# caomw/3DFeatureMatcher

Hardware: AMD Instinct MI355X
Metric: matched+triangulated+normal-optimised keypoints/sec; HBM GB/s vs roofline (higher is better)
Workload: dtype f64

## Files before the change

3dfeaturematcher_amd/csrc/fm3d_ctx.h:

```cpp
#pragma once

#include <hip/hip_runtime.h>

#include <cstdint>
#include <cstdlib>
#include <string>
#include <vector>

#include "fm3d.h"
#include "fm3d_algebra.h"
#include "fm3d_kernels.h"

namespace fm3d_host {

inline bool poison_word(uint32_t* word) {
    const char* e = getenv("FM3D_DEBUG_POISON");
    if (!e || !e[0]) return false;
    *word = (uint32_t)strtoul(e, nullptr, 0);
    return true;
}
inline void poison_host(void* p, size_t n, uint32_t word) {
    uint8_t* b = (uint8_t*)p;
    for (size_t i = 0; i < n; i++) b[i] = (uint8_t)(word >> (8 * (i & 3)));
}
inline hipError_t poison_device(void* p, size_t n) {
    uint32_t word;
    if (!poison_word(&word)) return hipSuccess;
    hipError_t e = hipSuccess;
    if (n / 4) e = hipMemsetD32((hipDeviceptr_t)p, (int)word, n / 4);
    for (size_t i = n & ~(size_t)3; e == hipSuccess && i < n; i++)
        e = hipMemset((uint8_t*)p + i, (int)(uint8_t)(word >> (8 * (i & 3))), 1);
    if (e == hipSuccess) e = hipDeviceSynchronize();
    return e;
}

template <class Mem>
struct Buf {
    void* p = nullptr;
    size_t bytes = 0;
    Buf() = default;
    Buf(const Buf&) = delete;
    Buf& operator=(const Buf&) = delete;
    Buf(Buf&& o) noexcept : p(o.p), bytes(o.bytes) {
        o.p = nullptr;
        o.bytes = 0;
    }
    Buf& operator=(Buf&& o) noexcept {
        if (this != &o) {
            if (p) Mem::free(p);
            p = o.p;
            bytes = o.bytes;
            o.p = nullptr;
            o.bytes = 0;
        }
        return *this;
    }
    ~Buf() {
        if (p) Mem::free(p);
    }
    hipError_t ensure(size_t n) {
        if (n <= bytes) return hipSuccess;
        if (p) Mem::free(p);
        p = nullptr;
        bytes = 0;
        size_t alloc = n < Mem::kMin ? Mem::kMin : n;
        hipError_t e = Mem::alloc(&p, alloc);
        if (e == hipSuccess) e = Mem::poison(p, alloc);
        if (e == hipSuccess) {
            bytes = alloc;
        } else if (p) {
            Mem::free(p);
            p = nullptr;
        }
        return e;
    }
    template <typename T>
    T* as() const {
        return (T*)p;
    }
};

struct DeviceMem {
    static constexpr size_t kMin = 256;
    static hipError_t alloc(void** p, size_t n) { return hipMalloc(p, n); }
    static hipError_t free(void* p) { return hipFree(p); }
    static hipError_t poison(void* p, size_t n) { return poison_device(p, n); }
};
struct PinnedMem {
    static constexpr size_t kMin = 4096;
    static hipError_t alloc(void** p, size_t n) { return hipHostMalloc(p, n, hipHostMallocDefault); }
    static hipError_t free(void* p) { return hipHostFree(p); }
    static hipError_t poison(void* p, size_t n) {
        uint32_t word;
        if (poison_word(&word)) poison_host(p, n, word);
        return hipSuccess;
    }
};
using DevBuf = Buf<DeviceMem>;
using HostBuf = Buf<PinnedMem>;

constexpr size_t kGuard(int w) { return (size_t)4 * w + 64; }

struct PipeSmall {
    int32_t cnt[4];
    unsigned long long prob[2];
    unsigned long long lm[26];
};

struct KnnWork {
    DevBuf cq, ct;
    DevBuf q8, t8;
    DevBuf partIdx, partKey;
    DevBuf pairs;
    DevBuf idx, key, fkey;
};

enum class PairState { Idle, Full, MemberFront, DltFront, Ncc, Verified, DltVerified };

enum class Need { Idle, StagedIdle, Full, Dlt, Ncc, Verified, DltVerified };

enum Ev {
    EV_LM_START,
    EV_END,
    EV_FRONT_START,
    EV_MATCH_DONE,
    EV_DLT_DONE,
    EV_VERIFY_START, EV_VERIFY_END,
    EV_NORMAL_START, EV_NORMAL_END,
    EV_SUBMIT_START,
    EV_TAIL_START,
    EV_COUNT
};

}

using fm3d_host::DevBuf;
using fm3d_host::HostBuf;

struct fm3d_ctx {
    fm3d_settings s;
    int device = 0;
    hipStream_t stream = nullptr;
    bool ownStream = false;
    fm3d::Camera cam{};
    double g12[16];
    double R2[9], t2[3];
    bool haveG12 = false;
    int w = 0, h = 0;
    std::vector<int> lw, lh;
    std::vector<DevBuf> pyr1, pyr2;
    int pyrGuardW = -1, pyrGuardH = -1, pyrGuardLevels = -1;
    DevBuf lvlDesc;
    DevBuf offsets;
    int nOff = 0, nOffPad = 0;
    DevBuf A, B, knnOut, cand, flag, matches, count, scanTmp;
    fm3d_host::KnnWork fwd, rev;
    DevBuf u8Flag;
    DevBuf gLines, gUV;
    bool gateStaged = false;
    bool specU8 = false;
    DevBuf sfImg, sfSum, sfDet, sfTr, sfLayers, sfMids, sfCand, sfCount, sfSortTmp, sfFlag, sfPos, sfKp, sfKin, sfSrc,
        sfDesc, sfDW, sfAng;
    DevBuf orbPyr, orbTab, orbLev, orbMap, orbFlag, orbPos, orbKp, orbR, orbBlur, orbDesc, orbPat;
    std::vector<int> orbUserPattern;
    DevBuf orbOffTab;
    std::vector<int> orbTabPattern;
    int orbTabPatchSize = 0, orbTabReach = 0;
    float orbTabAngle = 0.f;
    DevBuf siftImg, siftBase, siftG, siftD, siftGL, siftDL, siftTaps, siftScan, siftFlag, siftPos, siftCand, siftAng,
        siftNpk, siftKp, siftDesc;
    DevBuf brImg, brSum, brKp, brIdx, brPat, brPairs, brDesc;
    DevBuf frImg, frSum, frKp, frScale, frLut, frOp, frPairs, frAng, frDesc;
    DevBuf msImg, msWork, msHeap, msNode, msHist, msReg, msCnt, msOff, msXY, msScr, msKp, msFlag, msPos, msOut, msRank,
        msPad, msRegC;
    std::vector<int> freakUserPairs;
    DevBuf starImg, starS, starT, starF, starR, starZ, starKp, starFlag, starPos, starOut, starWork;
    DevBuf nccS, nccN, nccB;
    int nccH = 0;
    DevBuf f32Work;
    int nCU = 0;
    DevBuf kp1, kp2, triPts, triMask, triMask8, pts, srcIdx;
    long lmGroups = 0;
    int wallKhz = 0;
    DevBuf lmNormals, lmStatus, lmInfo, lmNfev, lmMdat, lmQueue, lmStat, slab, slabI1;
    DevBuf lbSt, lbCtr;
    unsigned lbEpoch = 0;
    DevBuf records, recTmp, recFlag;
    DevBuf lmProj;
    DevBuf pcnt;
    DevBuf verWork, verMatches;
    DevBuf tailFrames, tailRT, tailDesc, tailPatch;
    DevBuf pdKp, pdGL, pdLvl, pdTaps, pdKept;
    int pdCap = 0, pdSize = 0, pdNTaps = 0;
    float pdAngle = 0.f, pdSigma = 0.f;
    HostBuf hA, hB, hK1, hK2, hImg, hTab, hProj, hSmall, hFlag;
    HostBuf hVer;
    hipEvent_t evStage = nullptr;
    hipEvent_t evProj = nullptr;
    int nccP = 0;
    bool staged = false;
    struct Pipe {
        fm3d_host::PairState state = fm3d_host::PairState::Idle;
        int nA = 0, nB = 0, dim = 0, type = 0, dimPad = 0, queryOffset = 0;
        int K = 0, P = 0;
        bool stageEv = true;
        fm3d_record* subOut = nullptr;
        fm3d_record* pendOut = nullptr;
        fm3d_lm_stats subLm{};
        int nccHPending = 0;
        fm3d_ctx* linkLeader = nullptr;
        std::vector<fm3d_ctx*> linkMembers;
        hipEvent_t evFront = nullptr;
        hipEvent_t evLm = nullptr;
    } pipe;
    hipEvent_t ev[fm3d_host::EV_COUNT] = {};
    std::string err;

    fm3d_ctx() = default;
    fm3d_ctx(const fm3d_ctx&) = delete;
    fm3d_ctx& operator=(const fm3d_ctx&) = delete;
    ~fm3d_ctx() {
        for (hipEvent_t e : {evStage, evProj, pipe.evFront, pipe.evLm})
            if (e) hipEventDestroy(e);
        for (hipEvent_t e : ev)
            if (e) hipEventDestroy(e);
        if (ownStream) hipStreamDestroy(stream);
    }
};

namespace fm3d_host {

inline int fail(fm3d_ctx* c, int code, const std::string& msg) {
    if (c) c->err = msg;
    return code;
}

inline bool env_on(const char* name) {
    const char* e = getenv(name);
    return !(e && e[0] == '0');
}

int ensure_scan_tmp(fm3d_ctx* c, int n);
void install_g12(fm3d_ctx* c, const double g[16]);
bool good_max_px(double v);
int make_gate(fm3d_ctx* c, const fm3d_point2f* kp1, int nA, const fm3d_point2f* kp2, int nB, double maxPx,
              fm3d::EpiGate* g);
int ensure_offsets(fm3d_ctx* c);
int upload(fm3d_ctx* c, DevBuf& b, const void* src, size_t bytes);
int staging_wait(fm3d_ctx* c);
int upload_pinned(fm3d_ctx* c, DevBuf& dst, HostBuf& h, const void* src, size_t bytes);
int make_lookback(fm3d_ctx* c, int nBlocks, fm3d::LookBack* lb);
fm3d::TriParams tri_params(fm3d_ctx* c, int K, int queryOffset);
fm3d::NccParams ncc_params(fm3d_ctx* c, int Hphi, int Htheta, double span);
int set_images_impl(fm3d_ctx* c, const uint8_t* img1, const uint8_t* img2, int width, int height, int stride,
                    bool sync = true, bool waitStaging = true);

int stage_descriptors(fm3d_ctx* c, const void* descA, int nA, const void* descB, int nB, int dim, int type,
                      int* effType, int* dimPad, bool waitStaging = true, bool speculate = false);
struct MatchOpts {
    double eps = 0.0;
    int queryOffset = 0;
    bool wantKnn = false;
    fm3d_dmatch* compactOut = nullptr;
    int* compactCount = nullptr;
    const fm3d::EpiGate* gate = nullptr;
    int crossCheck = 0;
};
int run_match(fm3d_ctx* c, int nA, int nB, int type, int dimPad, const MatchOpts& o);

int describe_chunk();

struct LMSrc {
    fm3d_ctx* c;
    int P;
    const int* Pdev;
};
int lm_groups(fm3d_ctx* c, const void* kptr, int slots, long Ptot, long* out);
int run_lm_multi(fm3d_ctx* c, const LMSrc* src, int nProb, fm3d_lm_stats* stats, hipEvent_t e0, hipEvent_t e1);
int run_lm(fm3d_ctx* c, int P, const int* Pdev, fm3d_lm_stats* stats, hipEvent_t e0, hipEvent_t e1);
void fill_lm_cycles(const fm3d_ctx* c, const unsigned long long* cnt, fm3d_lm_stats* st);
fm3d::Camera lm_camera(const fm3d::Camera& cam);

int verify_staged(fm3d_ctx* c, const fm3d_verify_opts* o, int K, fm3d_verify_report* rep, bool* havePose,
                  double g12[16]);
int verify_staged_queue(fm3d_ctx* c, const fm3d_verify_opts* o);
int verify_report(fm3d_ctx* c, fm3d_verify_report* rep);

}

#define HIPCHK(ctx, expr)                                                                \
    do {                                                                                 \
        hipError_t e_ = (expr);                                                          \
        if (e_ != hipSuccess)                                                            \
            return fm3d_host::fail((ctx), FM3D_ERR_HIP, std::string(#expr ": ") + hipGetErrorString(e_)); \
    } while (0)
```

3dfeaturematcher_amd/csrc/fm3d_host.cpp:

```cpp
#include <hip/hip_runtime.h>

#include <algorithm>
#include <cfloat>
#include <cmath>
#include <cstdlib>
#include <cstring>
#include <string>
#include <vector>

#include "fm3d.h"
#include "fm3d_ctx.h"
#include "fm3d_kernels.h"

using fm3d::LevelDesc;

using namespace fm3d_host;

namespace fm3d_host {

int ensure_scan_tmp(fm3d_ctx* c, int n) {
    HIPCHK(c, c->scanTmp.ensure(fm3d::scan_tmp_bytes(n < 1 ? 1 : n)));
    HIPCHK(c, c->count.ensure(64));
    return FM3D_OK;
}

void install_g12(fm3d_ctx* c, const double g[16]) {
    std::memcpy(c->g12, g, sizeof(c->g12));
    camera2_from_g12(c->g12, c->R2, c->t2);
    c->haveG12 = true;
    c->gateStaged = false;
}

bool good_max_px(double v) { return v > 0. && v <= DBL_MAX; }

int make_gate(fm3d_ctx* c, const fm3d_point2f* kp1, int nA, const fm3d_point2f* kp2, int nB, double maxPx,
              fm3d::EpiGate* g) {
    HIPCHK(c, c->gLines.ensure((size_t)nA * sizeof(float4) + 16));
    HIPCHK(c, c->gUV.ensure((size_t)nB * sizeof(float2) + 16));
    double E[9];
    epipolar_matrix(c->R2, c->t2, E);
    fm3d::launch_epipolar_setup(c->cam, E, kp1, nA, kp2, nB, c->gLines.as<float4>(), c->gUV.as<float2>(), c->stream);
    HIPCHK(c, hipGetLastError());
    g->lines = c->gLines.as<float4>();
    g->uv = c->gUV.as<float2>();
    g->tau = maxPx * 2.0 / (c->cam.fx + c->cam.fy);
    return FM3D_OK;
}

int ensure_offsets(fm3d_ctx* c) {
    if (c->nOff > 0) return FM3D_OK;
    const int R = c->s.pixelsRay;
    std::vector<int2> off;
    for (int i = -R; i <= R; i++)
        for (int j = -R; j <= R; j++)
            if (i * i + j * j <= R * R) off.push_back(make_int2(i, j));
    c->nOff = (int)off.size();
    while (off.size() % 64) off.push_back(make_int2(1 << 20, 1 << 20));
    c->nOffPad = (int)off.size();
    HIPCHK(c, c->offsets.ensure(off.size() * sizeof(int2)));
    HIPCHK(c, hipMemcpy(c->offsets.p, off.data(), off.size() * sizeof(int2), hipMemcpyHostToDevice));
    return FM3D_OK;
}

int upload(fm3d_ctx* c, DevBuf& b, const void* src, size_t bytes) {
    HIPCHK(c, b.ensure(bytes));
    if (bytes) HIPCHK(c, hipMemcpyAsync(b.p, src, bytes, hipMemcpyHostToDevice, c->stream));
    return FM3D_OK;
}

int staging_wait(fm3d_ctx* c) {
    HIPCHK(c, hipEventSynchronize(c->evStage));
    return FM3D_OK;
}

int upload_pinned(fm3d_ctx* c, DevBuf& dst, HostBuf& h, const void* src, size_t bytes) {
    HIPCHK(c, dst.ensure(bytes));
    if (!bytes) return FM3D_OK;
    HIPCHK(c, h.ensure(bytes));
    std::memcpy(h.p, src, bytes);
    HIPCHK(c, hipMemcpyAsync(dst.p, h.p, bytes, hipMemcpyHostToDevice, c->stream));
    return FM3D_OK;
}

int make_lookback(fm3d_ctx* c, int nBlocks, fm3d::LookBack* lb) {
    if (!c->lbCtr.p) {
        HIPCHK(c, c->lbCtr.ensure(64));
        HIPCHK(c, hipMemsetAsync(c->lbCtr.p, 0, 64, c->stream));
    }
    bool zero = false;
    if (c->lbSt.bytes < (size_t)nBlocks * 8) {
        HIPCHK(c, c->lbSt.ensure((size_t)nBlocks * 8 * 2));
        zero = true;
    }
    if (++c->lbEpoch == 0) {
        c->lbEpoch = 1;
        zero = true;
    }
    if (zero) HIPCHK(c, hipMemsetAsync(c->lbSt.p, 0, c->lbSt.bytes, c->stream));
    lb->st = c->lbSt.as<unsigned long long>();
    lb->ctr = c->lbCtr.as<unsigned>();
    lb->epoch = c->lbEpoch;
    return FM3D_OK;
}

int set_images_impl(fm3d_ctx* c, const uint8_t* img1, const uint8_t* img2, int width, int height, int stride,
                    bool sync, bool waitStaging) {
    if (!img1 || !img2 || width <= 0 || height <= 0 || stride < width)
        return fail(c, FM3D_ERR_INVALID, "bad image arguments");
    const int levels = c->s.pyramids;
    if (levels < 0 || levels > 7) return fail(c, FM3D_ERR_UNSUPPORTED, "pyramids must be in [0, 7]");
    int r;
    if (waitStaging && (r = staging_wait(c))) return r;
    c->w = width;
    c->h = height;
    c->lw.assign(levels + 1, 0);
    c->lh.assign(levels + 1, 0);
    c->pyr1.resize(levels + 1);
    c->pyr2.resize(levels + 1);
    c->lw[0] = width;
    c->lh[0] = height;
    for (int L = 1; L <= levels; L++) {
        c->lw[L] = (c->lw[L - 1] + 1) / 2;
        c->lh[L] = (c->lh[L - 1] + 1) / 2;
    }
    bool fresh = c->pyrGuardW != width || c->pyrGuardH != height || c->pyrGuardLevels != levels;
    for (int L = 0; L <= levels; L++) {
        size_t bytes = (size_t)c->lw[L] * c->lh[L] + kGuard(c->lw[L]);
        void* p1 = c->pyr1[L].p;
        void* p2 = c->pyr2[L].p;
        HIPCHK(c, c->pyr1[L].ensure(bytes));
        HIPCHK(c, c->pyr2[L].ensure(bytes));
        fresh |= c->pyr1[L].p != p1 || c->pyr2[L].p != p2;
    }
    for (int L = 0; fresh && L <= levels; L++) {
        const size_t img = (size_t)c->lw[L] * c->lh[L];
        HIPCHK(c, hipMemsetAsync((char*)c->pyr1[L].p + img, 0, c->pyr1[L].bytes - img, c->stream));
        HIPCHK(c, hipMemsetAsync((char*)c->pyr2[L].p + img, 0, c->pyr2[L].bytes - img, c->stream));
    }
    c->pyrGuardW = width;
    c->pyrGuardH = height;
    c->pyrGuardLevels = levels;
    const size_t wh = (size_t)width * height;
    HIPCHK(c, c->hImg.ensure(2 * wh));
    for (int y = 0; y < height; y++) {
        std::memcpy(c->hImg.as<uint8_t>() + (size_t)y * width, img1 + (size_t)y * stride, width);
        std::memcpy(c->hImg.as<uint8_t>() + wh + (size_t)y * width, img2 + (size_t)y * stride, width);
    }
    HIPCHK(c, hipMemcpyAsync(c->pyr1[0].p, c->hImg.p, wh, hipMemcpyHostToDevice, c->stream));
    HIPCHK(c, hipMemcpyAsync(c->pyr2[0].p, c->hImg.as<uint8_t>() + wh, wh, hipMemcpyHostToDevice, c->stream));
    for (int L = 1; L <= levels; L++) {
        fm3d::launch_pyrdown(c->pyr1[L - 1].as<uint8_t>(), c->lw[L - 1], c->lh[L - 1], c->pyr1[L].as<uint8_t>(),
                             c->stream);
        fm3d::launch_pyrdown(c->pyr2[L - 1].as<uint8_t>(), c->lw[L - 1], c->lh[L - 1], c->pyr2[L].as<uint8_t>(),
                             c->stream);
    }
    HIPCHK(c, hipGetLastError());
    HIPCHK(c, c->hTab.ensure((levels + 1) * sizeof(LevelDesc)));
    LevelDesc* d = c->hTab.as<LevelDesc>();
    for (int L = 0; L <= levels; L++) d[L] = LevelDesc{c->pyr1[L].as<uint8_t>(), c->pyr2[L].as<uint8_t>(), c->lw[L], c->lh[L]};
    HIPCHK(c, c->lvlDesc.ensure((levels + 1) * sizeof(LevelDesc)));
    HIPCHK(c, hipMemcpyAsync(c->lvlDesc.p, d, (levels + 1) * sizeof(LevelDesc), hipMemcpyHostToDevice, c->stream));
    HIPCHK(c, hipEventRecord(c->evStage, c->stream));
    if (sync) HIPCHK(c, hipStreamSynchronize(c->stream));
    return FM3D_OK;
}

fm3d::TriParams tri_params(fm3d_ctx* c, int K, int queryOffset) {
    fm3d::TriParams p{};
    p.cam = c->cam;
    std::memcpy(p.g12, c->g12, sizeof(p.g12));
    p.zmin = c->s.zThresholdMin;
    p.zmax = c->s.zThresholdMax;
    p.kp1 = c->kp1.as<fm3d_point2f>();
    p.kp2 = c->kp2.as<fm3d_point2f>();
    p.matches = c->matches.as<fm3d_dmatch>();
    p.K = K;
    p.queryOffset = queryOffset;
    p.pts = c->triPts.as<double>();
    p.mask = c->triMask.as<int>();
    p.dltSolver = c->s.dltSolver;
    return p;
}

fm3d::NccParams ncc_params(fm3d_ctx* c, int Hphi, int Htheta, double span) {
    fm3d::NccParams p{};
    p.cam = lm_camera(c->cam);
    std::memcpy(p.R2, c->R2, sizeof(p.R2));
    std::memcpy(p.t2, c->t2, sizeof(p.t2));
    p.img1 = c->pyr1[0].as<uint8_t>();
    p.img2 = c->pyr2[0].as<uint8_t>();
    p.w = c->lw[0];
    p.h = c->lh[0];
    p.offsets = c->offsets.as<int2>();
    p.nOff = c->nOff;
    p.nOffPad = c->nOffPad;
    p.boundW = c->s.boundWidth;
    p.boundH = c->s.boundHeight;
    p.cmax = (int)(2 * c->s.zThresholdMax);
    p.Hphi = Hphi;
    p.Htheta = Htheta;
    p.span = span;
    return p;
}

}

extern "C" {

const char* fm3d_version(void) { return "fm3d 0.1 (gfx950)"; }

int fm3d_ctx_create(const fm3d_settings* s, int device, fm3d_ctx** out) {
    if (!s || !out) return FM3D_ERR_INVALID;
    *out = nullptr;
    if (s->dltSolver != 0 && s->dltSolver != 1) return FM3D_ERR_INVALID;
    if (!(s->guidedMatchPx >= 0. && s->guidedMatchPx <= DBL_MAX)) return FM3D_ERR_INVALID;
    if (s->crossCheck < 0 || s->crossCheck > 2) return FM3D_ERR_INVALID;
    int n = 0;
    if (hipGetDeviceCount(&n) != hipSuccess || n <= 0) return FM3D_ERR_HIP;
    if (device < 0 || device >= n) return FM3D_ERR_INVALID;
    if (hipSetDevice(device) != hipSuccess) return FM3D_ERR_HIP;
    fm3d_ctx* c = new fm3d_ctx();
    c->s = *s;
    c->device = device;
    if (hipStreamCreateWithFlags(&c->stream, hipStreamNonBlocking) != hipSuccess) {
        delete c;
        return FM3D_ERR_HIP;
    }
    c->ownStream = true;
    if (const char* le = getenv("FM3D_DEBUG_LB_EPOCH")) c->lbEpoch = (unsigned)strtoul(le, nullptr, 0);
    for (auto& e : c->ev) hipEventCreate(&e);
    hipEventCreateWithFlags(&c->evStage, hipEventDisableTiming);
    hipEventCreateWithFlags(&c->evProj, hipEventDisableTiming);
    hipEventCreateWithFlags(&c->pipe.evFront, hipEventDisableTiming);
    hipEventCreateWithFlags(&c->pipe.evLm, hipEventDisableTiming);
    c->cam.fx = s->Fx;
    c->cam.fy = s->Fy;
    c->cam.cx = s->Cx;
    c->cam.cy = s->Cy;
    c->cam.k[0] = s->k0;
    c->cam.k[1] = s->k1;
    c->cam.k[2] = s->p1;
    c->cam.k[3] = s->p2;
    c->cam.k[4] = s->k2;
    *out = c;
    return FM3D_OK;
}

void fm3d_ctx_destroy(fm3d_ctx* c) {
    if (!c) return;
    hipSetDevice(c->device);
    hipStreamSynchronize(c->stream);
    if (c->pipe.linkLeader) {
        auto& v = c->pipe.linkLeader->pipe.linkMembers;
        v.erase(std::remove(v.begin(), v.end(), c), v.end());
    }
    for (fm3d_ctx* m : c->pipe.linkMembers) m->pipe.linkLeader = nullptr;
    delete c;
}

const char* fm3d_last_error(const fm3d_ctx* c) { return c ? c->err.c_str() : "null context"; }

int fm3d_ctx_set_stream(fm3d_ctx* c, void* stream) {
    if (!c) return FM3D_ERR_INVALID;
    hipSetDevice(c->device);
    hipStreamSynchronize(c->stream);
    if (c->ownStream) hipStreamDestroy(c->stream);
    if (stream) {
        c->stream = (hipStream_t)stream;
        c->ownStream = false;
    } else {
        HIPCHK(c, hipStreamCreateWithFlags(&c->stream, hipStreamNonBlocking));
        c->ownStream = true;
    }
    return FM3D_OK;
}

int fm3d_setg12(fm3d_ctx* c, const double T1[3], const double T2[3], const double r1[3], const double r2[3],
                double g12[16]) {
    if (!c || !T1 || !T2 || !r1 || !r2) return fail(c, FM3D_ERR_INVALID, "null argument");
    double g[16];
    fm3d_g12_from_poses(&c->s, T1, T2, r1, r2, g);
    install_g12(c, g);
    if (g12) std::memcpy(g12, g, sizeof(g));
    return FM3D_OK;
}

int fm3d_set_g12(fm3d_ctx* c, const double g12[16]) {
    if (!c || !g12) return fail(c, FM3D_ERR_INVALID, "null argument");
    install_g12(c, g12);
    return FM3D_OK;
}

int fm3d_get_camera2(const fm3d_ctx* c, double R2[9], double t2[3]) {
    if (!c || !c->haveG12) return FM3D_ERR_INVALID;
    std::memcpy(R2, c->R2, sizeof(c->R2));
    std::memcpy(t2, c->t2, sizeof(c->t2));
    return FM3D_OK;
}

int fm3d_triangulate(fm3d_ctx* c, const fm3d_point2f* kpts1, int n1, const fm3d_point2f* kpts2, int n2,
                     const fm3d_dmatch* matches, int K, double* points, uint8_t* inlierMask, int* nPoints) {
    if (!c || !nPoints || K < 0) return fail(c, FM3D_ERR_INVALID, "bad argument");
    if (!c->haveG12) return fail(c, FM3D_ERR_INVALID, "g12 not set (SingleCameraTriangulator::setg12)");
    hipSetDevice(c->device);
    for (int i = 0; i < K; i++)
        if (matches[i].queryIdx < 0 || matches[i].queryIdx >= n1 || matches[i].trainIdx < 0 || matches[i].trainIdx >= n2)
            return fail(c, FM3D_ERR_INVALID, "match index out of range");
    int r;
    if ((r = upload(c, c->kp1, kpts1, (size_t)n1 * sizeof(fm3d_point2f)))) return r;
    if ((r = upload(c, c->kp2, kpts2, (size_t)n2 * sizeof(fm3d_point2f)))) return r;
    if ((r = upload(c, c->matches, matches, (size_t)K * sizeof(fm3d_dmatch)))) return r;
    HIPCHK(c, c->triPts.ensure((size_t)(K + 1) * 3 * sizeof(double)));
    HIPCHK(c, c->triMask.ensure((size_t)(K + 1) * sizeof(int)));
    HIPCHK(c, c->triMask8.ensure((size_t)(K + 1)));
    HIPCHK(c, c->pts.ensure((size_t)(K + 1) * 3 * sizeof(double)));
    HIPCHK(c, c->srcIdx.ensure((size_t)(K + 1) * sizeof(int)));
    if ((r = ensure_scan_tmp(c, K))) return r;
    fm3d::TriParams p = tri_params(c, K, 0);
    p.mask8 = c->triMask8.as<uint8_t>();
    fm3d::launch_triangulate(p, c->stream);
    fm3d::launch_compact_points(c->triPts.as<double>(), c->triMask.as<int>(), K, nullptr, c->pts.as<double>(),
                                c->count.as<int>(), c->srcIdx.as<int>(), c->scanTmp.p, c->stream);
    HIPCHK(c, hipGetLastError());
    int n = 0;
    HIPCHK(c, hipMemcpyAsync(&n, c->count.p, sizeof(int), hipMemcpyDeviceToHost, c->stream));
    if (inlierMask && K) HIPCHK(c, hipMemcpyAsync(inlierMask, c->triMask8.p, K, hipMemcpyDeviceToHost, c->stream));
    HIPCHK(c, hipStreamSynchronize(c->stream));
    if (n && points) HIPCHK(c, hipMemcpy(points, c->pts.p, (size_t)n * 3 * sizeof(double), hipMemcpyDeviceToHost));
    *nPoints = n;
    return FM3D_OK;
}

int fm3d_set_images(fm3d_ctx* c, const uint8_t* img1, const uint8_t* img2, int width, int height, int stride) {
    if (!c) return FM3D_ERR_INVALID;
    hipSetDevice(c->device);
    return set_images_impl(c, img1, img2, width, height, stride);
}

int fm3d_get_pyramid_level(const fm3d_ctx* cc, int which, int level, uint8_t* out, int* w, int* h) {
    fm3d_ctx* c = const_cast<fm3d_ctx*>(cc);
    if (!c || level < 0 || level >= (int)c->pyr1.size() || (which != 1 && which != 2)) return FM3D_ERR_INVALID;
    hipSetDevice(c->device);
    if (w) *w = c->lw[level];
    if (h) *h = c->lh[level];
    if (out) {
        const DevBuf& b = which == 1 ? c->pyr1[level] : c->pyr2[level];
        HIPCHK(c, hipMemcpy(out, b.p, (size_t)c->lw[level] * c->lh[level], hipMemcpyDeviceToHost));
    }
    return FM3D_OK;
}

int fm3d_records_download(fm3d_ctx* c, const fm3d_record* recordsDev, int n, fm3d_record* out) {
    if (!c || n < 0 || (n && !out)) return FM3D_ERR_INVALID;
    hipSetDevice(c->device);
    const void* src = recordsDev ? (const void*)recordsDev : c->records.p;
    if (n) HIPCHK(c, hipMemcpy(out, src, (size_t)n * sizeof(fm3d_record), hipMemcpyDeviceToHost));
    return FM3D_OK;
}

int fm3d_features_frames(fm3d_ctx* c, const double* points, const double* normals, int P, double* frames) {
    if (!c || P < 0 || (P && (!points || !normals || !frames))) return FM3D_ERR_INVALID;
    if (P == 0) return FM3D_OK;
    hipSetDevice(c->device);
    double g[3];
    int r;
    if ((r = fm3d_gravity(&c->s, g))) return fail(c, r, "gravity: singular rodriguesIC rotation");
    DevBuf a, b, f;
    HIPCHK(c, a.ensure((size_t)P * 3 * sizeof(double)));
    HIPCHK(c, b.ensure((size_t)P * 3 * sizeof(double)));
    HIPCHK(c, f.ensure((size_t)P * 16 * sizeof(double)));
    HIPCHK(c, hipMemcpyAsync(a.p, points, (size_t)P * 3 * sizeof(double), hipMemcpyHostToDevice, c->stream));
    HIPCHK(c, hipMemcpyAsync(b.p, normals, (size_t)P * 3 * sizeof(double), hipMemcpyHostToDevice, c->stream));
    fm3d::launch_features_frames(a.as<double>(), b.as<double>(), P, g, f.as<double>(), c->stream);
    HIPCHK(c, hipGetLastError());
    HIPCHK(c, hipMemcpyAsync(frames, f.p, (size_t)P * 16 * sizeof(double), hipMemcpyDeviceToHost, c->stream));
    HIPCHK(c, hipStreamSynchronize(c->stream));
    return FM3D_OK;
}

int fm3d_export_patches(fm3d_ctx* c, const double* frames, int P, uint8_t* patches, double* imagePoints) {
    if (!c || P < 0 || (P && (!frames || !patches))) return FM3D_ERR_INVALID;
    if (c->pyr1.empty()) return fail(c, FM3D_ERR_INVALID, "fm3d_set_images not called");
    const int size = fm3d_patch_size(&c->s);
    if (size <= 0) return fail(c, FM3D_ERR_INVALID, "patch size <= 0 (Neighborhoods.epsilon / cmPerPixel)");
    if (P == 0) return FM3D_OK;
    hipSetDevice(c->device);
    const size_t per = (size_t)size * size;
    DevBuf f, rt, out, pts;
    HIPCHK(c, f.ensure((size_t)P * 16 * sizeof(double)));
    HIPCHK(c, rt.ensure((size_t)P * 12 * sizeof(double)));
    HIPCHK(c, out.ensure((size_t)P * per));
    if (imagePoints) HIPCHK(c, pts.ensure((size_t)P * per * 2 * sizeof(double)));
    HIPCHK(c, hipMemcpyAsync(f.p, frames, (size_t)P * 16 * sizeof(double), hipMemcpyHostToDevice, c->stream));
    fm3d::launch_export_patches(f.as<double>(), P, size, c->s.neighEpsilon, c->s.cmPerPixel * 0.01, c->cam,
                                c->pyr1[0].as<uint8_t>(), c->lw[0], c->lh[0], rt.as<double>(), out.as<uint8_t>(),
                                imagePoints ? pts.as<double>() : nullptr, c->stream);
    HIPCHK(c, hipGetLastError());
    HIPCHK(c, hipMemcpyAsync(patches, out.p, (size_t)P * per, hipMemcpyDeviceToHost, c->stream));
    if (imagePoints)
        HIPCHK(c, hipMemcpyAsync(imagePoints, pts.p, (size_t)P * per * 2 * sizeof(double), hipMemcpyDeviceToHost,
                                 c->stream));
    HIPCHK(c, hipStreamSynchronize(c->stream));
    return FM3D_OK;
}

int fm3d_square_neighborhoods(fm3d_ctx* c, const double* frames, int P, double* out) {
    if (!c || P < 0 || (P && (!frames || !out))) return FM3D_ERR_INVALID;
    const int size = fm3d_patch_size(&c->s);
    if (size <= 0) return fail(c, FM3D_ERR_INVALID, "neighbourhood size <= 0 (Neighborhoods.epsilon / cmPerPixel)");
    if (P == 0) return FM3D_OK;
    hipSetDevice(c->device);
    const size_t perFrame = (size_t)size * size * 3 * sizeof(double);
    const int chunk = (int)std::max<size_t>(1, std::min<size_t>((size_t)P, ((size_t)512 << 20) / perFrame));
    DevBuf f, o;
    HIPCHK(c, f.ensure((size_t)chunk * 16 * sizeof(double)));
    HIPCHK(c, o.ensure((size_t)chunk * perFrame));
    for (int p0 = 0; p0 < P; p0 += chunk) {
        const int n = std::min(chunk, P - p0);
        HIPCHK(c, hipMemcpyAsync(f.p, frames + (size_t)16 * p0, (size_t)n * 16 * sizeof(double),
                                 hipMemcpyHostToDevice, c->stream));
        fm3d::launch_square_neighborhoods(f.as<double>(), n, size, c->s.neighEpsilon, c->s.cmPerPixel * 0.01,
                                          o.as<double>(), c->stream);
        HIPCHK(c, hipGetLastError());
        HIPCHK(c, hipMemcpyAsync(out + (size_t)p0 * size * size * 3, o.p, (size_t)n * perFrame,
                                 hipMemcpyDeviceToHost, c->stream));
        HIPCHK(c, hipStreamSynchronize(c->stream));
    }
    return FM3D_OK;
}

int fm3d_circular_neighborhoods(fm3d_ctx* c, const double* points, const double* normals, int P, double* out) {
    if (!c || P < 0 || (P && (!points || !out))) return FM3D_ERR_INVALID;
    if (c->s.neighMethod != 1) return fail(c, FM3D_ERR_INVALID, "Neighborhoods.method is not circular");
    const int T = c->s.neighThetas, Rn = c->s.neighRays;
    if (T <= 0 || Rn <= 0) return fail(c, FM3D_ERR_INVALID, "Neighborhoods.thetas / rays <= 0");
    if (P == 0) return FM3D_OK;
    hipSetDevice(c->device);
    const double eps = c->s.neighEpsilon;
    const double rayIncrement = eps / Rn, thetaIncrement = 2 * M_PI / T;
    const int S = T * Rn;
    std::vector<double> lut((size_t)S * 3);
    for (int i = 1; i <= Rn; i++)
        for (int j = 0; j < T; j++) {
            const double t = j * thetaIncrement;
            double* e = &lut[3 * ((size_t)(i - 1) * T + j)];
            e[0] = (double)i * rayIncrement;
            e[1] = std::sin(t);
            e[2] = 2 * (std::sin(t / 2)) * (std::sin(t / 2));
        }
    const size_t perPoint = (size_t)S * 3 * sizeof(double);
    const int chunk = (int)std::max<size_t>(1, std::min<size_t>((size_t)P, ((size_t)512 << 20) / perPoint));
    DevBuf L, X, N, O;
    HIPCHK(c, L.ensure(lut.size() * sizeof(double)));
    HIPCHK(c, X.ensure((size_t)chunk * 3 * sizeof(double)));
    if (normals) HIPCHK(c, N.ensure((size_t)chunk * 3 * sizeof(double)));
    HIPCHK(c, O.ensure((size_t)chunk * perPoint));
    HIPCHK(c, hipMemcpyAsync(L.p, lut.data(), lut.size() * sizeof(double), hipMemcpyHostToDevice, c->stream));
    for (int p0 = 0; p0 < P; p0 += chunk) {
        const int n = std::min(chunk, P - p0);
        HIPCHK(c, hipMemcpyAsync(X.p, points + (size_t)3 * p0, (size_t)n * 3 * sizeof(double), hipMemcpyHostToDevice,
                                 c->stream));
        if (normals)
            HIPCHK(c, hipMemcpyAsync(N.p, normals + (size_t)3 * p0, (size_t)n * 3 * sizeof(double),
                                     hipMemcpyHostToDevice, c->stream));
        fm3d::launch_circular_neighborhoods(X.as<double>(), normals ? N.as<double>() : nullptr, n, S, L.as<double>(),
                                            eps, O.as<double>(), c->stream);
        HIPCHK(c, hipGetLastError());
        HIPCHK(c, hipMemcpyAsync(out + (size_t)p0 * S * 3, O.p, (size_t)n * perPoint, hipMemcpyDeviceToHost,
                                 c->stream));
        HIPCHK(c, hipStreamSynchronize(c->stream));
    }
    return FM3D_OK;
}

int fm3d_ncc_hypotheses(fm3d_ctx* c, const double* points, int P, int Hphi, int Htheta, double span, double* scores,
                        double* normals, int32_t* best) {
    if (!c || P < 0 || Hphi <= 0 || Htheta <= 0 || Hphi * Htheta > 32 || (P && (!points || !scores || !normals || !best)))
        return FM3D_ERR_INVALID;
    if (c->pyr1.empty()) return fail(c, FM3D_ERR_INVALID, "fm3d_set_images (NormalOptimizer::setImages) not called");
    if (!c->haveG12) return fail(c, FM3D_ERR_INVALID, "fm3d_set_g12 / fm3d_setg12 not called");
    if (P == 0) return FM3D_OK;
    hipSetDevice(c->device);
    int r;
    if ((r = ensure_offsets(c))) return r;
    const int H = Hphi * Htheta;
    DevBuf X, S, N, B;
    HIPCHK(c, X.ensure((size_t)P * 3 * sizeof(double)));
    HIPCHK(c, S.ensure((size_t)P * H * sizeof(double)));
    HIPCHK(c, N.ensure((size_t)P * 3 * sizeof(double)));
    HIPCHK(c, B.ensure((size_t)P * sizeof(int)));
    HIPCHK(c, hipMemcpyAsync(X.p, points, (size_t)P * 3 * sizeof(double), hipMemcpyHostToDevice, c->stream));
    fm3d::NccParams p = ncc_params(c, Hphi, Htheta, span);
    p.points = X.as<double>();
    p.P = P;
    p.scores = S.as<double>();
    p.normals = N.as<double>();
    p.best = B.as<int>();
    fm3d::launch_ncc_hypotheses(p, c->stream);
    HIPCHK(c, hipGetLastError());
    HIPCHK(c, hipMemcpyAsync(scores, S.p, (size_t)P * H * sizeof(double), hipMemcpyDeviceToHost, c->stream));
    HIPCHK(c, hipMemcpyAsync(normals, N.p, (size_t)P * 3 * sizeof(double), hipMemcpyDeviceToHost, c->stream));
    HIPCHK(c, hipMemcpyAsync(best, B.p, (size_t)P * sizeof(int), hipMemcpyDeviceToHost, c->stream));
    HIPCHK(c, hipStreamSynchronize(c->stream));
// ... 131 lines not shown
```

3dfeaturematcher_amd/csrc/fm3d_internal.h:

```cpp
#pragma once

#include <hip/hip_runtime.h>

#include "fm3d.h"

int fm3d_internal_submit_to(fm3d_ctx* c, const void* descA, int nA, const void* descB, int nB, int dim, int type,
                            const fm3d_point2f* kpts1, const fm3d_point2f* kpts2, const uint8_t* img1,
                            const uint8_t* img2, int width, int height, fm3d_record* recordsDev);
int fm3d_internal_flush(fm3d_ctx* c);
bool fm3d_internal_front_only(const fm3d_ctx* c);
int fm3d_internal_enqueue(fm3d_ctx* c, fm3d_record* recordsDev);
int fm3d_internal_finish(fm3d_ctx* c, int* nKept, fm3d_pipeline_stats* stats);
const int* fm3d_internal_kept_dev(fm3d_ctx* c);
hipStream_t fm3d_internal_stream(fm3d_ctx* c);
int fm3d_internal_prepare(fm3d_ctx* c);
int fm3d_internal_memory_need(fm3d_ctx* c, int64_t nA, int64_t nB, int dim, int type, int width, int height,
                              size_t* bytes);
extern "C" int fm3d_internal_alloc_probe(fm3d_ctx* c, size_t bytes, uint8_t* out);
```

3dfeaturematcher_amd/csrc/fm3d_kernels.h:

```cpp
#pragma once

#include <hip/hip_runtime.h>
#include <stdint.h>

#include "fm3d.h"
#include "fm3d_device.h"

#ifndef FM3D_RAY_AOS
#define FM3D_RAY_AOS 1
#endif

namespace fm3d {

struct LevelDesc {
    const uint8_t* img1;
    const uint8_t* img2;
    int w, h;
};

struct ProjConst {
    double R[9], t[3];
    Camera cam;
    const char *slabRX, *slabRY, *slabI1;
    char *slabDF, *slabDJ0, *slabDJ1;
    double k2d, k3d;
};

struct LMProblem {
    const double* points;
    const int* Pdev;
    const LevelDesc* lvl;
    double* normals;
    int* status;
    int* info;
    int* nfev;
    int* mdat;
    unsigned long long* stat;
    int P;
    unsigned projOff;
};

struct LMParams {
    const double* points_;
    int P_;
    const int* Pdev_;
    Camera cam;
    double R2_[9], t2_[3];
    const ProjConst* proj;
    const LevelDesc* lvl_;
    int levels;
    const int2* offsets;
    int nOff, nOffPad;
    int boundW, boundH;
    double epsfcn;
    int cmax;
    int* queue;
    double* slab;
    float* slabI1;
    long nWaves;
    double* normals_;
    int* status_;
    int* info_;
    int* nfev_;
    int* mdat_;
    unsigned long long* statEval;
    unsigned long long* statPix;
    long long maxIter;
    long long maxTicks;
    int* overflow;
    int coop;
    int safe;
    unsigned long long* statPass;
    int nProb;
    const LMProblem* prob;
};
constexpr int kLMMaxProblems = 4;

constexpr int kLMRunning = 0x100;

constexpr int kLM2Slots = 15;
constexpr int kLM2Ring = 8;
constexpr int kLM2Threads = 64 * (kLM2Slots + 1);
template <bool MULTI, bool TREE>
__global__ void lm2_kernel(LMParams p);

struct KnnOut {
    int* idx;
    int* key;
    float* fkey;
};

struct EpiGate {
    const float4* lines;
    const float2* uv;
    double tau;
    bool transposed = false;
};
void launch_epipolar_setup(const Camera& cam, const double E[9], const fm3d_point2f* kp1, int n1,
                           const fm3d_point2f* kp2, int n2, float4* lines, float2* uv, hipStream_t s);

int knn2_u8_parts(int nA, int nB, int nCU, int qPerBlock, int tileRows);
int knn2_i8_queries_per_block(int dimPad, int bits);
int knn2_i8_tile_rows(int dimPad, int bits);
void launch_knn2_i8(const uint8_t* A, int nA, const uint8_t* B, int nB, int dimPad, int bits, const int* cqA,
                    const int* ctB, int parts, int* partIdx, int* partKey, int* idx, int* key, hipStream_t s,
                    bool deferMerge = false, const EpiGate* gate = nullptr);
void launch_rowconst_u8(const uint8_t* A, int nA, const uint8_t* B, int nB, int dimPad, int* cq, int* ctp,
                        hipStream_t s);
void launch_f32_pack_u8(const float* A, int nA, const float* B, int nB, int dim, int dimPad, uint8_t* Au,
                        uint8_t* Bu, int* notU8, hipStream_t s);
void launch_unpack_bits(const uint8_t* A, int nA, const uint8_t* B, int nB, uint8_t* outA, uint8_t* outB, int* ctp,
                        hipStream_t s);
int knn2_parts(int nA, int nB, int dim, int nCU);
size_t knn2_f32_pairs_bytes(int nB, int dim);
void launch_knn2_f32(const float* A, int nA, const float* B, int nB, int dim, int parts, int* partIdx,
                     float* partKey, float* pairs, int* idx, float* key, hipStream_t s);
void launch_knn2_f32_gated(const float* A, int nA, const float* B, int nB, int dim, int parts, int* partIdx,
                           float* partKey, int* idx, float* key, const EpiGate& gate, hipStream_t s);
size_t knn2_f32_mfma_bytes(int nA, int nB, int dim, int parts);
int knn2_f32_mfma_parts(int nA, int nB, int nCU);
void launch_knn2_f32_mfma(const float* A, int nA, const float* B, int nB, int dim, int parts, bool fused, void* work,
                          int* idx, float* key, hipStream_t s);
int* knn2_f32_mfma_rescan_count(void* work, int nA, int nB, int dim, int parts);
void launch_knn2_f32_mfma_rescan(const float* A, const float* B, int nB, int dim, void* work, int nA, int parts,
                                 int nResc, int* idx, float* key, hipStream_t s);
void launch_knn2_bits(const uint8_t* A, int nA, const uint8_t* B, int nB, int dimBytes, int parts, int* partIdx,
                      int* partKey, int* idx, int* key, hipStream_t s, const EpiGate* gate = nullptr);
void launch_nndr(int type, const int* idx, const int* key, const float* fkey, int nA, int nB, double eps,
                 int queryOffset, fm3d_dmatch* knnOut, fm3d_dmatch* cand, int* flag, hipStream_t s);

struct NccParams {
    const double* points;
    int P;
    const int* Pdev;
    Camera cam;
    double R2[9], t2[3];
    const uint8_t *img1, *img2;
    int w, h;
    const int2* offsets;
    int nOff, nOffPad, boundW, boundH, cmax;
    int Hphi, Htheta;
    double span;
    double* scores;
    double* normals;
    int* best;
};
void launch_ncc_hypotheses(const NccParams& p, hipStream_t s);

struct SurfHF {
    int p0, p1, p2, p3;
    float w;
};
struct SurfLayer {
    long long first;
    size_t off;
    int size, step, margin, si, sj, rows, cols;
    SurfHF hf[10];
};
struct SurfMid {
    long long first;
    int layer, octave, rows, cols, margin;
};
struct SurfCand {
    float x, y, size, response;
    int octave, class_id;
    long long seq;
};
constexpr int kOriMax = 128;
struct SurfOri {
    int n;
    int ax[kOriMax], ay[kOriMax];
    float w[kOriMax];
};
void launch_integral(const uint8_t* img, int w, int h, int* sum, hipStream_t s);
void launch_integral_rows(const uint8_t* img, int w, int h, int* rows, hipStream_t s);
void launch_integral_batch(const uint8_t* img, int w, int h, int nb, int* sum, hipStream_t s);
void launch_surf_orient(const void* kp, size_t kstride, int n, const int* sum, size_t sumStride, int w, int h,
                        const SurfOri& ori, int* flag, float* angle, hipStream_t s);
void launch_surf_hessian(const int* sum, int w, const SurfLayer* layers, int nL, long long total, float* det,
                         float* tr, hipStream_t s);
void launch_surf_maxima(const float* det, const float* tr, const SurfLayer* layers, const SurfMid* mids, int nM,
                        long long total, float thr, SurfCand* cand, int* count, int cap, hipStream_t s);
size_t surf_sort_tmp_bytes(int n);
void launch_surf_sort(SurfCand* cand, int n, void* tmp, size_t tmpBytes, hipStream_t s);
void launch_surf_upright(const SurfCand* cand, const int* count, int n, int w, int h, int* flag, int* pos, int* total,
                         void* scanTmp, fm3d_keypoint* out, int* src, const float* angle, hipStream_t s);
void launch_surf_keep(const fm3d_keypoint* in, int n, int w, int h, int* flag, int* pos, int* total, void* scanTmp,
                      fm3d_keypoint* out, int* src, const float* angle, hipStream_t s);
void launch_surf_describe(const uint8_t* img, size_t imgStride, int w, int h, const fm3d_keypoint* kp, int n,
                          const float* DW, int extended, int upright, float* desc, hipStream_t s);

struct OrbLevel {
    int w, h;
    long long first;
};
struct OrbUmax {
    int u[64];
};
struct OrbBlurK {
    int ik[7];
    float fk[4];
};
void launch_orb_resize(const uint8_t* src, int sw, int sh, uint8_t* dst, int dw, int dh, const int* xofs,
                       const short* alpha, const int* yofs, const short* beta, int xmax, int xs, hipStream_t s);
void launch_orb_fast(const uint8_t* pyr, const OrbLevel* L, int nL, long long total, int thr, int border, int nonmax,
                     uint16_t* map, int* flag, hipStream_t s);
void launch_orb_fast_scatter(const uint16_t* map, const OrbLevel* L, int nL, long long total, const int* flag,
                             const int* pos, fm3d_keypoint* out, hipStream_t s);
void launch_orb_harris(const uint8_t* pyr, const OrbLevel* L, fm3d_keypoint* kp, int n, hipStream_t s);
void launch_orb_angle(const uint8_t* pyr, const OrbLevel* L, fm3d_keypoint* kp, int n, int half, const OrbUmax& um,
                      hipStream_t s);
void launch_orb_blur(const uint8_t* pyr, const OrbLevel* L, int nL, long long total, const OrbBlurK& bk, int* R,
                     uint8_t* out, hipStream_t s);
void launch_orb_desc(const uint8_t* blur, const OrbLevel* L, const fm3d_keypoint* kp, int n, const int* pattern,
                     uint8_t* desc, hipStream_t s);
void launch_orb_offset_table(const int* pattern, float angle, int2* tab, hipStream_t s);
void launch_orb_patch_desc(const uint8_t* patches, int m, int size, const int2* tab, const OrbBlurK& bk, uint8_t* desc,
                           hipStream_t s);

struct SiftLevel {
    int w, h;
    long long first;
};
struct SiftResize {
    int sw, sh, dw, dh, xmax, doubled;
    double scx, scy;
};
struct SiftScan {
    long long first;
    int dog, octave, layer, pad;
};
struct SiftCand {
    float x, y, size, response;
    int koct;
    int octave, layer, r, c, ok;
};
void launch_sift_init(const uint8_t* img, float* dst, const SiftResize& p, int batch, hipStream_t s);
size_t sift_blur_lds(int n);
void launch_sift_blur(const float* src, float* dst, float* dog, int w, int h, const float* taps, int n, int batch,
                      hipStream_t s);
void launch_sift_down(const float* src, int sw, int sh, float* dst, int dw, int dh, double ifx, double ify,
                      hipStream_t s);
void launch_sift_extrema(const float* dog, const SiftLevel* DL, const SiftScan* S, int nS, long long total,
                         int threshold, int* flag, hipStream_t s);
void launch_sift_cand_scatter(const SiftLevel* DL, const SiftScan* S, int nS, long long total, const int* flag,
                              const int* pos, SiftCand* cand, hipStream_t s);
void launch_sift_adjust(const float* dog, const SiftLevel* DL, int L, float contrastThreshold, float edgeThreshold,
                        float sigma, SiftCand* cand, int n, hipStream_t s);
void launch_sift_orient(const float* gp, const SiftLevel* GL, int L, const SiftCand* cand, int n, float* angles,
                        int* npk, hipStream_t s);
void launch_sift_desc(const float* gp, const SiftLevel* GL, int L, int firstOctave, const fm3d_keypoint* kp,
                      const int* lvl, int n, float* desc, hipStream_t s);

size_t scan_tmp_bytes(int n);
void launch_compact_dmatch(const fm3d_dmatch* in, const int* flag, int n, fm3d_dmatch* out, int* count, void* tmp,
                           hipStream_t s, const int* nDev = nullptr);
void launch_compact_points(const double* in, const int* flag, int n, const int* nDev, double* out, int* count,
                           int* srcIndex, void* tmp, hipStream_t s);
void launch_exclusive_scan(const int* flag, int n, int* offsets, int* total, void* tmp, hipStream_t s);

constexpr int kVerifyTile = 1024;
constexpr int kVerifyMaxHyps = 1 << 20;
int verify_pad(int M);
void launch_verify(const Camera& cam, const fm3d_point2f* kp1, const fm3d_point2f* kp2, const fm3d_dmatch* matches,
                   int M, int H, unsigned long long seed, double tau2, int nCU, double* xy, double* models, int* count,
                   int* best, double* E, int* flag, uint8_t* mask, hipStream_t s, bool withMask = true,
                   const int* Mdev = nullptr);
size_t verify_refine_bytes(int M, int rounds);
void launch_verify_refine(int M, int rounds, double tau2, const double* xy, const int* count, const int* best,
                          double* E, void* work, int* flag, uint8_t* mask, int** roundCounts, double** roundModels,
                          int** adopted, hipStream_t s, const int* Mdev = nullptr);
struct VerifySmall {
    int32_t matches, verified, best, adopted;
    double E[9];
};
void launch_verify_report(const int* Mdev, const int* best, const double* E, const int* adopted, const int* verified,
                          VerifySmall* host, hipStream_t s);
size_t verify_pose_bytes();
void launch_verify_pose(int M, const double* xy, const int* flag, const int* best, const double* E, void* work,
                        double** cand, int** valid, int** votes, hipStream_t s);

struct AlignIn {
    const double *ptsA, *nrmA, *ptsB, *nrmB;
    int nA, nB;
};
inline int align_planes(bool normals) { return normals ? 12 : 6; }
void launch_align(const AlignIn& in, const fm3d_dmatch* matches, int M, int H, unsigned long long seed, double tau2,
                  double minCos, int nCU, double* planes, double* models, int* count, int* best, double* model,
                  int* flag, uint8_t* mask, hipStream_t s, bool withMask = true);
size_t align_refine_bytes(int M, int rounds);
void launch_align_refine(int M, bool normals, int rounds, double tau2, double minCos, const double* planes,
                         const int* count, const int* best, double* model, void* work, int* flag, uint8_t* mask,
                         int** roundCounts, double** roundModels, int** adopted, hipStream_t s);

struct LocalizeIn {
    const fm3d_point2f* kpts;
    const double *pts, *nrm;
    int nKpts, nPts;
};
inline int localize_planes(bool normals) { return normals ? 8 : 5; }
void launch_localize(const Camera& cam, const LocalizeIn& in, const fm3d_dmatch* matches, int M, int samples,
                     unsigned long long seed, double tau2, double cos2, int nCU, double* planes, double* models,
                     int* count, int* best, double* model, int* flag, uint8_t* mask, hipStream_t s,
                     bool withMask = true);
size_t localize_refine_bytes(int M, int rounds);
void launch_localize_refine(int M, bool normals, int rounds, double tau2, double cos2, const double* planes,
                            const int* count, const int* best, double* model, void* work, int* flag, uint8_t* mask,
                            int** roundCounts, double** roundModels, int** adopted, hipStream_t s);

struct TriParams {
    Camera cam;
    double g12[16];
    double zmin, zmax;
    const fm3d_point2f* kp1;
    const fm3d_point2f* kp2;
    const fm3d_dmatch* matches;
    int K;
    const int* Kdev;
    int queryOffset;
    double* pts;
    int* mask;
    uint8_t* mask8;
    int dltSolver;
};
void launch_triangulate(const TriParams& p, hipStream_t s);

struct LMReset {
    unsigned long long* stat;
    int* queue;
    int nProb;
    int* pcnt16[kLMMaxProblems];
    int* status[kLMMaxProblems];
    int* info[kLMMaxProblems];
    int* nfev[kLMMaxProblems];
    int P[kLMMaxProblems];
};
void launch_lm_reset(const LMReset& r, hipStream_t s);

struct LookBack {
    unsigned long long* st;
    unsigned* ctr;
    unsigned epoch;
};
__device__ inline int lookback_block_id(const LookBack& lb) {
    const unsigned id = atomicAdd(lb.ctr, 1u);
    if (id == gridDim.x - 1) __hip_atomic_store(lb.ctr, 0u, __ATOMIC_RELAXED, __HIP_MEMORY_SCOPE_AGENT);
    return (int)id;
}
void launch_nndr_compact(int type, const int* idx, const int* key, const float* fkey, const int* partIdx,
                         const int* partKey, int parts, int nA, double eps, int queryOffset, fm3d_dmatch* out,
                         int* count, const LookBack& lb, hipStream_t s);
int nndr_compact_blocks(int nA);
struct MutualCheck {
    const int* rIdx;
    const int* rKey;
    const float* rFkey;
    int mode;
};
void launch_nndr_mutual_compact(int type, const int* idx, const int* key, const float* fkey, const int* partIdx,
                                const int* partKey, int parts, int nA, double eps, int queryOffset,
                                const MutualCheck& mc, fm3d_dmatch* out, int* count, const LookBack& lb,
                                hipStream_t s);
void launch_triangulate_compact(const TriParams& p, double* out, int* srcIdx, int* count, const LookBack& lb,
                                hipStream_t s, int* hostCnt = nullptr);
int triangulate_compact_blocks(int K);

void launch_pyrdown(const uint8_t* src, int w, int h, uint8_t* dst, hipStream_t s);
void launch_undistort(const Camera& cam, const double* xy, int n, double* out, hipStream_t s);

bool math_probe_binary(int fn);
void launch_math_probe(int fn, const double* x, const double* y, int n, double* out, hipStream_t s);

struct PlaneProjParams {
    Camera cam;
    double R2[9], t2[3], X[3], n[3];
    double cmax;
    const int2* offsets;
    int nOff, boundW, boundH, w, h;
    double *xy, *uv;
    int *keep, *status;
};
void launch_plane_project(const PlaneProjParams& p, hipStream_t s);

void launch_features_frames(const double* pts, const double* nrm, int P, const double g[3], double* frames,
                            hipStream_t s);
void launch_circular_neighborhoods(const double* pts, const double* nrm, int P, int S, const double* lut, double eps,
                                   double* out, hipStream_t s);
void launch_square_neighborhoods(const double* frames, int P, int size, double eps, double inc, double* out,
                                 hipStream_t s);
void launch_export_patches(const double* frames, int P, int size, double eps, double inc, const Camera& cam,
                           const uint8_t* img, int w, int h, double* RT, uint8_t* patches, double* imagePoints,
                           hipStream_t s);
void launch_tail_frames(const fm3d_record* rec, const double* pts, const double* nrm, int P, const double g[3],
                        double* frames, double* RT, hipStream_t s);
void launch_patches(const double* RT, int P, int size, double eps, double inc, const Camera& cam, const uint8_t* img,
                    int w, int h, uint8_t* patches, hipStream_t s);
void launch_add_count(const int* count, int* sum, hipStream_t s);

void launch_make_records(const fm3d_dmatch* matches, const int* inlierSrc, int nInl, const int* nDev, const double* pts,
                         const double* normals, const int* status, fm3d_record* rec, int* flag, hipStream_t s);
void launch_compact_records(const fm3d_record* in, const int* flag, int n, const int* nDev, fm3d_record* out,
                            int* count, void* tmp, hipStream_t s);

struct StarPat {
    int np, maxIdx, border, nsimd;
    int sizes1[17];
    int ofs[17 * 8];
    float inv[24];
};
struct StarNms {
    int border, delta, nx, ny, respThr, lineProj, lineBin;
};
size_t star_tilted_lds_bytes(int w);
int star_tilted_max_width();
void launch_star_tilted(const uint8_t* img, int w, int h, int* T, int* F, hipStream_t s);
size_t star_diag_bytes(int w, int h);
void launch_star_tilted_diag(const uint8_t* img, int w, int h, void* work, int* T, int* F, hipStream_t s);
void launch_star_resp(const int* S, const int* T, const int* F, int w, int h, const StarPat& P, float* resp,
                      short* sizes, hipStream_t s);
void launch_star_nms(const float* resp, const short* sizes, int w, int h, const StarNms& N, fm3d_keypoint* kp, int* flag,
                     hipStream_t s);
void launch_star_scatter(const fm3d_keypoint* kp, const int* flag, const int* pos, int n, fm3d_keypoint* out,
                         hipStream_t s);

constexpr int kFreakScales = 64, kFreakOrient = 256, kFreakPoints = 43, kFreakOrientPairs = 45;
void launch_freak_desc(const uint8_t* img, const int* sum, int w, const fm3d_keypoint* kp, const int* scale, int n,
                       const float4* lut, const int4* opairs, const int2* pairs, float* angle, uint8_t* desc,
                       hipStream_t s);

struct MserParams {
    int delta, minArea, maxArea;
    double maxVariation, minDiversity;
};
struct MserHist {
    int shortcut, child, stable, val, size;
};
struct MserLayout {
    int w, h;
    int pw;
    int visInLds;
    long long visWords;
    long long padBytes;
    long long heapEntries;
    long long nodes;
    long long hists;
    long long regCap;
};
constexpr long long kMserLdsBits = 120 * 1024 * 8;
MserLayout mser_layout(int w, int h);
void launch_mser_flood(const uint8_t* img, int count, const MserLayout& L, const MserParams& P, uint8_t* pad,
                       unsigned* vis, int2* heap, int2* node, MserHist* hist, int4* reg, int* nreg, hipStream_t s);
struct MserRank {
    const int *rank, *last, *base, *pts;
};
size_t mser_rank_bytes(long long nodes, int slots);
MserRank launch_mser_rank(const int2* node, long long nodes, int slots, int* work, hipStream_t s);
void launch_mser_fit(const int4* reg, int n, const MserRank& K, long long nodes, const long long* off,
                     const MserLayout& L, int2* xy, double* scratch, fm3d_keypoint* kp, int* flag, float* box,
                     hipStream_t s);

void launch_brisk_desc(const uint8_t* img, const int* II, int w, const fm3d_keypoint* kp, const int* pidx, int n,
                       const float4* pat, const int2* pairs, int npairs, uint8_t* desc, hipStream_t s);

}
```

3dfeaturematcher_amd/csrc/fm3d_lm.cpp:

```cpp
#include <cstdlib>
#include <cstring>
#include <vector>

#include "fm3d_ctx.h"

using fm3d::LevelDesc;

using namespace fm3d_host;

namespace fm3d_host {

void fill_lm_cycles(const fm3d_ctx* c, const unsigned long long* cnt, fm3d_lm_stats* st) {
    st->groups = c->lmGroups;
    st->passes = (int64_t)cnt[3];
    st->cycles_terms = (int64_t)cnt[4];
    st->cycles_chain = (int64_t)cnt[5];
    st->cycles_control = (int64_t)cnt[6];
    st->cycles_total = (int64_t)cnt[7];
    st->wall_ticks_sum = (int64_t)cnt[8];
    st->wall_ticks_max = (int64_t)cnt[9];
    st->wall_clock_khz = c->wallKhz;
    for (int k = 0; k < 4; k++) {
        st->class_passes[k] = (int64_t)cnt[10 + k];
        st->class_cycles[k] = (int64_t)cnt[14 + k];
    }
    st->last_group_start_ticks = (int64_t)(cnt[18] - cnt[20]);
    st->last_group_end_ticks = (int64_t)(cnt[19] - cnt[20]);
    st->cycles_wait = (int64_t)cnt[24];
    st->chain_rounds = (int64_t)cnt[21];
    st->chain_chunks = (int64_t)cnt[22];
    st->queue_empty_ticks = cnt[25] ? (int64_t)(cnt[25] - cnt[20]) : 0;
}

fm3d::Camera lm_camera(const fm3d::Camera& cam) {
    fm3d::Camera k = cam;
    if (k.cx == 0.) k.cx = 0.;
    if (k.cy == 0.) k.cy = 0.;
    return k;
}

int lm_groups(fm3d_ctx* c, const void* kptr, int slots, long Ptot, long* out) {
    long groups = c->s.lmWaves;
    if (groups <= 0) {
        int cus = 0, perCU = 0;
        HIPCHK(c, hipDeviceGetAttribute(&cus, hipDeviceAttributeMultiprocessorCount, c->device));
        HIPCHK(c, hipOccupancyMaxActiveBlocksPerMultiprocessor(&perCU, kptr, fm3d::kLM2Threads, 0));
        if (perCU < 1) perCU = 1;
        groups = (long)cus * perCU;
    }
    if (Ptot >= 0) {
        const long needed = (Ptot + slots - 1) / slots;
        if (groups > needed) groups = needed;
    }
    const size_t ents = (size_t)c->nOffPad * slots;
    const size_t perGroup = ents * (2 * sizeof(double) + 5 * 4);
    const size_t budget = (size_t)48 << 30;
    long cap = (long)(budget / perGroup);
    if (cap < 1) cap = 1;
    if (groups > cap) groups = cap;
    const long cap32 = (long)((((size_t)1 << 32) - ((size_t)1 << 20)) / (ents * sizeof(double) * (FM3D_RAY_AOS ? 2 : 1)));
    if (groups > cap32) groups = cap32;
    if (groups < 1) groups = 1;
    *out = groups;
    return FM3D_OK;
}

int run_lm_multi(fm3d_ctx* c, const LMSrc* src, int nProb, fm3d_lm_stats* stats, hipEvent_t e0, hipEvent_t e1) {
    int r;
    if (nProb < 1 || nProb > fm3d::kLMMaxProblems) return fail(c, FM3D_ERR_INVALID, "bad LM problem count");
    if ((r = ensure_offsets(c))) return r;
    const fm3d::Camera cam = lm_camera(c->cam);
    const int levels = c->s.pyramids;
    long Ptot = 0;
    for (int j = 0; j < nProb; j++) {
        fm3d_ctx* q = src[j].c;
        if (q->pyr1.empty()) return fail(c, FM3D_ERR_INVALID, "fm3d_set_images (NormalOptimizer::setImages) not called");
        if (!q->haveG12) return fail(c, FM3D_ERR_INVALID, "g12 not set (SingleCameraTriangulator::setg12)");
        if (q != c && (q->device != c->device || q->s.pyramids != levels || q->s.pixelsRay != c->s.pixelsRay ||
                       std::memcmp(&q->cam, &c->cam, sizeof(c->cam)) != 0 || q->s.boundWidth != c->s.boundWidth ||
                       q->s.boundHeight != c->s.boundHeight || q->s.zThresholdMax != c->s.zThresholdMax ||
                       q->s.epsilonLMMIN != c->s.epsilonLMMIN || q->s.lmReduction != c->s.lmReduction))
            return fail(c, FM3D_ERR_INVALID, "linked contexts need one device, camera and LM settings");
        const int P = src[j].P;
        HIPCHK(c, q->lmNormals.ensure((size_t)(P + 1) * 3 * sizeof(double)));
        HIPCHK(c, q->lmStatus.ensure((size_t)(P + 1) * sizeof(int)));
        HIPCHK(c, q->lmInfo.ensure((size_t)(P + 1) * 8 * sizeof(int)));
        HIPCHK(c, q->lmNfev.ensure((size_t)(P + 1) * 8 * sizeof(int)));
        HIPCHK(c, q->lmMdat.ensure((size_t)(P + 1) * sizeof(int)));
        HIPCHK(c, q->pcnt.ensure(64));
        Ptot += P;
    }
    HIPCHK(c, c->lmQueue.ensure(64 * sizeof(int)));
    HIPCHK(c, c->lmStat.ensure(256));
    if (c->s.lmReduction != 0 && c->s.lmReduction != 1)
        return fail(c, FM3D_ERR_INVALID, "lmReduction must be 0 (pixel order) or 1 (tree)");
    const bool tree = c->s.lmReduction != 0;
    const int slots = fm3d::kLM2Slots + (tree ? 1 : 0);
    bool multiPose = false;
    for (int j = 1; j < nProb; j++)
        multiPose |= std::memcmp(src[j].c->R2, src[0].c->R2, sizeof(c->R2)) != 0 ||
                     std::memcmp(src[j].c->t2, src[0].c->t2, sizeof(c->t2)) != 0;
    const void* kptr = tree ? (multiPose ? reinterpret_cast<const void*>(fm3d::lm2_kernel<true, true>)
                                         : reinterpret_cast<const void*>(fm3d::lm2_kernel<false, true>))
                            : (multiPose ? reinterpret_cast<const void*>(fm3d::lm2_kernel<true, false>)
                                         : reinterpret_cast<const void*>(fm3d::lm2_kernel<false, false>));
    long groups = 0;
    int r0;
    if ((r0 = lm_groups(c, kptr, slots, Ptot, &groups))) return r0;
    const size_t ents = (size_t)c->nOffPad * slots;
    HIPCHK(c, c->slab.ensure(ents * 2 * sizeof(double) * groups + 16384));
    HIPCHK(c, c->slabI1.ensure(ents * 5 * 4 * groups + 16384));
    fm3d::LMParams p{};
    p.nProb = nProb;
    p.cam = cam;
    {
        HIPCHK(c, hipEventSynchronize(c->evProj));
        const size_t pcBytes = (sizeof(fm3d::ProjConst) + 255) / 256 * 256;
        HIPCHK(c, c->hProj.ensure(pcBytes * nProb + sizeof(fm3d::LMProblem) * nProb));
        char* hp = c->hProj.as<char>();
        fm3d::LMProblem* hpr = (fm3d::LMProblem*)(hp + pcBytes * nProb);
        HIPCHK(c, c->lmProj.ensure(pcBytes * nProb + sizeof(fm3d::LMProblem) * nProb));
        const size_t Gn = (size_t)groups * slots * c->nOffPad;
        for (int j = 0; j < nProb; j++) {
            fm3d_ctx* q = src[j].c;
            fm3d::ProjConst& pc = *(fm3d::ProjConst*)(hp + pcBytes * j);
            std::memcpy(pc.R, q->R2, sizeof(pc.R));
            std::memcpy(pc.t, q->t2, sizeof(pc.t));
            pc.cam = cam;
            pc.k2d = 2. * cam.k[2];
            pc.k3d = 2. * cam.k[3];
            pc.slabRX = (const char*)c->slab.p;
            pc.slabRY = FM3D_RAY_AOS ? pc.slabRX + sizeof(double) : pc.slabRX + Gn * sizeof(double);
            pc.slabI1 = (const char*)c->slabI1.p;
            pc.slabDF = (char*)c->slabI1.p + Gn * 4;
            pc.slabDJ0 = pc.slabDF + Gn * 4;
            pc.slabDJ1 = pc.slabDJ0 + Gn * 4;
            fm3d::LMProblem& pr = hpr[j];
            pr.points = q->pts.as<double>();
            pr.Pdev = src[j].Pdev;
            pr.P = src[j].P;
            pr.lvl = q->lvlDesc.as<LevelDesc>();
            pr.normals = q->lmNormals.as<double>();
            pr.status = q->lmStatus.as<int>();
            pr.info = q->lmInfo.as<int>();
            pr.nfev = q->lmNfev.as<int>();
            pr.mdat = q->lmMdat.as<int>();
            pr.stat = (unsigned long long*)(q->pcnt.as<char>() + 16);
            pr.projOff = (unsigned)(pcBytes * j);
        }
        HIPCHK(c, hipMemcpyAsync(c->lmProj.p, hp, pcBytes * nProb + sizeof(fm3d::LMProblem) * nProb,
                                 hipMemcpyHostToDevice, c->stream));
        HIPCHK(c, hipEventRecord(c->evProj, c->stream));
        p.proj = c->lmProj.as<fm3d::ProjConst>();
        p.prob = (const fm3d::LMProblem*)(c->lmProj.as<char>() + pcBytes * nProb);
    }
    p.levels = levels;
    p.offsets = c->offsets.as<int2>();
    p.nOff = c->nOff;
    p.nOffPad = c->nOffPad;
    p.boundW = c->s.boundWidth;
    p.boundH = c->s.boundHeight;
    p.epsfcn = c->s.epsilonLMMIN;
    p.cmax = (int)(2 * c->s.zThresholdMax);
    p.queue = c->lmQueue.as<int>();
    p.slab = c->slab.as<double>();
    p.slabI1 = c->slabI1.as<float>();
    p.nWaves = groups;
    p.statEval = c->lmStat.as<unsigned long long>();
    p.statPix = c->lmStat.as<unsigned long long>() + 1;
    p.overflow = (int*)(c->lmStat.as<unsigned long long>() + 2);
    p.statPass = c->lmStat.as<unsigned long long>() + 3;
    c->lmGroups = groups;
    {
        const long long perSlot = (Ptot + groups * slots - 1) / (groups * slots) + 1;
        p.maxIter = perSlot * (long long)(levels + 1) * 1600 + 10000;
        int khz = 0;
        if (hipDeviceGetAttribute(&khz, hipDeviceAttributeWallClockRate, c->device) != hipSuccess || khz <= 0) khz = 100000;
        const char* ms = getenv("FM3D_LM_MAX_SECONDS");
        const double secs = ms && atof(ms) > 0 ? atof(ms) : 300.;
        p.maxTicks = (long long)((double)khz * 1000. * secs);
        c->wallKhz = khz;
        const char* co = getenv("FM3D_LM_COOP");
        p.coop = co ? atoi(co) : 1;
        if (tree) p.coop = 0;
        const char* sf = getenv("FM3D_LM_SAFE");
        p.safe = sf ? atoi(sf) : 0;
    }
    {
        fm3d::LMReset rz{};
        rz.stat = c->lmStat.as<unsigned long long>();
        rz.queue = Ptot > 0 ? c->lmQueue.as<int>() : nullptr;
        rz.nProb = nProb;
        for (int j = 0; j < nProb; j++) {
            fm3d_ctx* q = src[j].c;
            rz.pcnt16[j] = q->pcnt.as<int>() + 4;
            rz.status[j] = q->lmStatus.as<int>();
            rz.info[j] = q->lmInfo.as<int>();
            rz.nfev[j] = q->lmNfev.as<int>();
            rz.P[j] = Ptot > 0 && src[j].P > 0 ? src[j].P : 0;
        }
        if (Ptot > 0) HIPCHK(c, hipEventRecord(e0, c->stream));
        fm3d::launch_lm_reset(rz, c->stream);
        HIPCHK(c, hipGetLastError());
    }
    if (Ptot > 0) {
        void* kargs[] = {&p};
        HIPCHK(c, hipLaunchKernel(kptr, dim3((unsigned)groups), dim3(fm3d::kLM2Threads), kargs, 0, c->stream));
        HIPCHK(c, hipEventRecord(e1, c->stream));
    }
    if (stats) {
        std::memset(stats, 0, sizeof(*stats));
        stats->points_in = Ptot;
    }
    return FM3D_OK;
}

int run_lm(fm3d_ctx* c, int P, const int* Pdev, fm3d_lm_stats* stats, hipEvent_t e0, hipEvent_t e1) {
    const LMSrc one{c, P, Pdev};
    return run_lm_multi(c, &one, 1, stats, e0, e1);
}

}

extern "C" {

int fm3d_optimize_normals(fm3d_ctx* c, double* points, int P, double* normals, int32_t* status, int32_t* info,
                          int32_t* nfev, int* nKept, fm3d_lm_stats* stats) {
    if (!c || !nKept || P < 0 || (P && (!points || !normals))) return fail(c, FM3D_ERR_INVALID, "bad argument");
    hipSetDevice(c->device);
    int r;
    if ((r = upload(c, c->pts, points, (size_t)P * 3 * sizeof(double)))) return r;
    if ((r = run_lm(c, P, nullptr, stats, c->ev[EV_LM_START], c->ev[EV_END]))) return r;
    std::vector<double> nrm((size_t)P * 3);
    std::vector<int> st(P), inf((size_t)P * 8), nf((size_t)P * 8);
    unsigned long long cnt[26] = {};
    if (P) {
        HIPCHK(c, hipMemcpyAsync(nrm.data(), c->lmNormals.p, nrm.size() * sizeof(double), hipMemcpyDeviceToHost, c->stream));
        HIPCHK(c, hipMemcpyAsync(st.data(), c->lmStatus.p, st.size() * sizeof(int), hipMemcpyDeviceToHost, c->stream));
        HIPCHK(c, hipMemcpyAsync(inf.data(), c->lmInfo.p, inf.size() * sizeof(int), hipMemcpyDeviceToHost, c->stream));
        HIPCHK(c, hipMemcpyAsync(nf.data(), c->lmNfev.p, nf.size() * sizeof(int), hipMemcpyDeviceToHost, c->stream));
        HIPCHK(c, hipMemcpyAsync(cnt, c->lmStat.p, sizeof(cnt), hipMemcpyDeviceToHost, c->stream));
    }
    HIPCHK(c, hipStreamSynchronize(c->stream));
    int overflow = 0;
    HIPCHK(c, hipMemcpy(&overflow, c->lmStat.as<unsigned long long>() + 2, sizeof(int), hipMemcpyDeviceToHost));
    if (overflow) return fail(c, FM3D_ERR_HIP, "LM kernel iteration guard tripped (internal error)");
    float ms = 0.f;
    if (P) hipEventElapsedTime(&ms, c->ev[EV_LM_START], c->ev[EV_END]);
    int kept = 0;
    bool nanPlane = false;
    for (int i = 0; i < P; i++) {
        if (status) status[i] = st[i];
        if (info) std::memcpy(&info[(size_t)8 * i], &inf[(size_t)8 * i], 8 * sizeof(int));
        if (nfev) std::memcpy(&nfev[(size_t)8 * i], &nf[(size_t)8 * i], 8 * sizeof(int));
        if (st[i] == FM3D_ST_NAN_PLANE) nanPlane = true;
        if (st[i] == FM3D_ST_OK) {
            for (int k = 0; k < 3; k++) {
                points[3 * kept + k] = points[3 * i + k];
// ... 23 lines not shown
```

3dfeaturematcher_amd/csrc/fm3d_lm2.hip:

```cpp
#include <hip/hip_runtime.h>
#include <float.h>
#include <stdint.h>

#include <type_traits>

#include "fm3d_device.h"
#include "fm3d_fastdiv.h"
#include "fm3d_kernels.h"
#include "fm3d_lmdif.h"

namespace fm3d {

namespace {

using namespace lmdif;

constexpr int kW = kLM2Slots;
constexpr int kWA = kW + 1;
constexpr int kE = 64;
constexpr int kR = kLM2Ring;
static_assert((kR & (kR - 1)) == 0, "ring depth: a power of two");
constexpr int kRow = kE + 2;
constexpr int kRS = (2 * kLM2Slots * kRow * 8 + 255) / 256 * 256 / 8;
#ifndef FM3D_EVAL_PIPE
#define FM3D_EVAL_PIPE 1
#endif

enum PassKind2 { Q_IDLE = 0, Q_INIT, Q_LEVEL, Q_EVAL, Q_QR1, Q_QR2, Q_QR3, Q_GRAM, Q_DONE };
enum SumKind { S_NONE = 0, S_ENORM, S_DOT };

typedef __attribute__((address_space(1))) double gdouble;
typedef __attribute__((address_space(1))) float gfloat;
typedef double d2v __attribute__((ext_vector_type(2)));
typedef __attribute__((address_space(1))) d2v gd2v;
typedef __attribute__((address_space(1))) int gint;
typedef __attribute__((address_space(1))) const long long gi64;
typedef __attribute__((address_space(1))) const uint8_t gu8;
typedef __attribute__((address_space(1), aligned(1))) const uint16_t gu16u;


struct SlotP2 {
    int pass, ekind, nev, len, pivot, t0, t1, q0, lw;
    unsigned projOff;
    double n0[2], n1[2], n2[2], mm[2], w[2], hj[2];
    double ta[2], tb[2];
    int tpend;
    double scale, xmax, ymax, ccx, ccy, ajn0s, tq, ajn1s, tq0, agiant, wF;
    const uint8_t* img1;
    const uint8_t* img2;
};

struct SlotS2 {
    LM s;
    double X0, X1, X2, ccx, ccy, nrm0, nrm1, nrm2;
    double apf, aqf, ff, aps, fs, vfirst, r01, tq0, qtf0, wa4s, usecond, ajn0s, tq, ajn1s;
    double wF, wJ[2];
    long long pev, ppix;
    int prob;
    int pidx, m, L, i1ok, ekind, t0, q0, t1, bNaN;
};

struct PassOut2 {
    double nrm[2];
    double sum[2];
    double aqs1;
    double sq[2], g[3];
    int cnt, fail[2], ph3[2], i1fail, slow;
};

struct PassDesc {
    int nChunks, id;
    int kind[2];
    double agiant;
};

struct Slab {
    gdouble* RX;
    gdouble* RY;
    gfloat* I1;
    gfloat* DF;
    gfloat* DJ0;
    gfloat* DJ1;
    gint* KI;
};
template <int NS>
__device__ inline Slab slab_of(const LMParams& p, long gslot) {
    const size_t n = (size_t)p.nOffPad, G = (size_t)p.nWaves * NS;
    Slab s;
#if FM3D_RAY_AOS
    s.RX = (gdouble*)p.slab + gslot * n * 2;
    s.RY = s.RX + 1;
#else
    s.RX = (gdouble*)p.slab + gslot * n;
    s.RY = s.RX + G * n;
#endif
    s.I1 = (gfloat*)p.slabI1 + gslot * n;
    s.DF = s.I1 + G * n;
    s.DJ0 = s.DF + G * n;
    s.DJ1 = s.DJ0 + G * n;
    s.KI = (gint*)(s.DJ1 + G * n);
    return s;
}

struct Ctl2 {
    const LMParams* p;
    Slab sl;
    double eps;
    long long cnt_eval, cnt_pix;
    int tree;

    __device__ void fetch(SlotS2& S, SlotP2& P) {
        int loc = atomicAdd(p->queue, 1), j = 0;
        for (; j < p->nProb; j++) {
            const LMProblem& pr = p->prob[j];
            const int n = pr.Pdev ? *pr.Pdev : pr.P;
            if (loc < n) break;
            loc -= n;
        }
        if (j >= p->nProb) {
            P.pass = Q_DONE;
            return;
        }
        const LMProblem& pr = p->prob[j];
        S.prob = j;
        S.pidx = loc;
        S.pev = 0;
        S.ppix = 0;
        P.projOff = pr.projOff;
        atomicMax(p->statPass + 22, wall_clock64());
        S.X0 = pr.points[3 * loc + 0];
        S.X1 = pr.points[3 * loc + 1];
        S.X2 = pr.points[3 * loc + 2];
        const double Ident[9] = {1, 0, 0, 0, 1, 0, 0, 0, 1};
        const double Zero[3] = {0, 0, 0};
        double cx, cy;
        project1(p->cam, Ident, Zero, S.X0, S.X1, S.X2, cx, cy);
        S.ccx = cx;
        S.ccy = cy;
        P.pass = Q_INIT;
        P.len = p->nOffPad;
        P.ccx = cx;
        P.ccy = cy;
    }
    __device__ void start_level(SlotS2& S, SlotP2& P) {
        const LevelDesc lv = p->prob[S.prob].lvl[S.L];
        P.pass = Q_LEVEL;
        P.len = S.m;
        P.scale = ldexp(1.0, -S.L);
        P.xmax = (1 / P.scale) * lv.w;
        P.ymax = (1 / P.scale) * lv.h;
        P.img1 = lv.img1;
        P.img2 = lv.img2;
        P.lw = lv.w;
        P.ccx = S.ccx;
        P.ccy = S.ccy;
    }
    __device__ void finish_point(SlotS2& S, SlotP2& P, int code) {
        const LMProblem& pr = p->prob[S.prob];
        pr.status[S.pidx] = code;
        pr.normals[3 * S.pidx + 0] = S.nrm0;
        pr.normals[3 * S.pidx + 1] = S.nrm1;
        pr.normals[3 * S.pidx + 2] = S.nrm2;
        pr.mdat[S.pidx] = S.m;
        atomicAdd(pr.stat + 0, (unsigned long long)S.pev);
        atomicAdd(pr.stat + 1, (unsigned long long)S.ppix);
        fetch(S, P);
    }
    __device__ void level_done(SlotS2& S, SlotP2& P, int info) {
        const LMProblem& pr = p->prob[S.prob];
        pr.info[8 * S.pidx + S.L] = info;
        pr.nfev[8 * S.pidx + S.L] = S.s.nfev;
        sph2car_cr(S.s.x[0], S.s.x[1], S.nrm0, S.nrm1, S.nrm2);
        S.L--;
        if (S.L < 0)
            finish_point(S, P, FM3D_ST_OK);
        else
            start_level(S, P);
    }
    __device__ void abort_level(SlotS2& S, SlotP2& P, int code) {
        const LMProblem& pr = p->prob[S.prob];
        pr.info[8 * S.pidx + S.L] = -code;
        pr.nfev[8 * S.pidx + S.L] = S.s.nfev;
        finish_point(S, P, code);
    }
    __device__ bool setup_eval(SlotS2& S, SlotP2& P, int ev, double a, double b, double hj) {
        if (fabs(a) < FM3D_CR_RANGE && fabs(b) < FM3D_CR_RANGE) {
            P.ta[ev] = a;
            P.tb[ev] = b;
            P.tpend |= 1 << ev;
        } else {
            double n0, n1, n2;
            sph2car_cr(a, b, n0, n1, n2);
            if (n2 != n2 || n1 != n1 || n0 != n0) return false;
            P.n0[ev] = n0;
            P.n1[ev] = n1;
            P.n2[ev] = n2;
            P.mm[ev] = n0 * S.X0 + n1 * S.X1 + n2 * S.X2;
            P.tpend &= ~(1 << ev);
        }
        double w_theta = 1.0, w_phi = 1.0;
        if (fabs(b) - M_PI / 2 > 0 || fabs(a) - M_PI > 0) {
            w_theta = fm3d_exp_cr(fabs(b) - M_PI / 2) + 1;
            w_phi = fm3d_exp_cr(fabs(a) - M_PI + 1) + 1;
        }
        P.w[ev] = w_phi * w_theta;
        P.hj[ev] = hj;
        return true;
    }
    __device__ void resolve_trig(const SlotS2& S, SlotP2& P, int lane) {
        __builtin_amdgcn_s_waitcnt(0);
        __builtin_amdgcn_fence(__ATOMIC_ACQ_REL, "wavefront");
        const int pend = __builtin_amdgcn_readfirstlane(P.tpend);
        if (!pend) return;
        const int e = lane >> 2, f = lane & 3;
        double v = 0.;
        if (e < 2 && ((pend >> e) & 1)) v = fm3d_sincos_sel_cr(f < 2 ? P.tb[e] : P.ta[e], (f & 1) == 0);
        for (int k = 0; k < 2; k++) {
            if (!((pend >> k) & 1)) continue;
            const double ct = __shfl(v, 4 * k), st = __shfl(v, 4 * k + 1), cp = __shfl(v, 4 * k + 2),
                         sp = __shfl(v, 4 * k + 3);
            if (lane == 0) {
                const double n0 = ct * cp, n1 = ct * sp, n2 = st;
                P.n0[k] = n0;
                P.n1[k] = n1;
                P.n2[k] = n2;
                P.mm[k] = n0 * S.X0 + n1 * S.X1 + n2 * S.X2;
            }
        }
        if (lane == 0) P.tpend = 0;
        __builtin_amdgcn_s_waitcnt(0);
        __builtin_amdgcn_fence(__ATOMIC_ACQ_REL, "wavefront");
    }
    __device__ void count_eval(SlotS2& S) {
        S.s.nfev++;
        cnt_eval++;
        cnt_pix += S.m;
        S.pev++;
        S.ppix += S.m;
    }
    __device__ void eval_pass(SlotS2& S, SlotP2& P, int kind, double a, double b) {
        count_eval(S);
        if (!setup_eval(S, P, 0, a, b, 1.0)) {
            abort_level(S, P, FM3D_ST_NAN_NORMAL);
            return;
        }
        S.ekind = kind;
        S.wF = P.w[0];
        P.pass = Q_EVAL;
        P.len = S.m;
        P.ekind = kind;
        P.nev = 1;
        P.agiant = 1.304e19 / (double)S.m;
    }
    __device__ void jac_pass(SlotS2& S, SlotP2& P) {
        LM& s = S.s;
        s.h[0] = eps * fabs(s.x[0]);
        if (s.h[0] == 0.) s.h[0] = eps;
        s.h[1] = eps * fabs(s.x[1]);
        if (s.h[1] == 0.) s.h[1] = eps;
        count_eval(S);
        if (!setup_eval(S, P, 0, s.x[0] + s.h[0], s.x[1], s.h[0])) {
            abort_level(S, P, FM3D_ST_NAN_NORMAL);
            return;
        }
        S.bNaN = !setup_eval(S, P, 1, s.x[0], s.x[1] + s.h[1], s.h[1]);
        S.wJ[0] = P.w[0];
        S.wJ[1] = P.w[1];
        S.ekind = E_JAC;
        P.pass = Q_EVAL;
        P.len = S.m;
        P.ekind = E_JAC;
        P.nev = S.bNaN ? 1 : 2;
        P.agiant = 1.304e19 / (double)S.m;
        P.wF = S.wF;
    }
    __device__ double fvec_at(const SlotS2& S, int e) const { return S.wF * (double)sl.DF[e]; }
    __device__ double jcol_at(const SlotS2& S, int j, int e) const {
        const double F = fvec_at(S, e);
        const double r = S.wJ[j] * (double)(j ? sl.DJ1 : sl.DJ0)[e];
        return (r - F) / S.s.h[j];
    }
    __device__ void finalize_qr(SlotS2& S, SlotP2& P, double qtf1) {
        S.s.r[0] = S.t0 ? -S.ajn0s : 0.;
        S.s.r[1] = 0.;
        S.s.r[2] = S.r01;
        S.s.r[3] = S.t1 ? -S.ajn1s : 0.;
        S.s.qtf[0] = S.qtf0;
        S.s.qtf[1] = qtf1;
        after_qr(S, P);
    }
    __device__ void after_qr(SlotS2& S, SlotP2& P) {
        int info = lm_after_qr(S.s);
        if (info) {
            level_done(S, P, info);
        } else {
            lm_inner_step(S.s);
            eval_pass(S, P, E_TRIAL, S.s.wa2[0], S.s.wa2[1]);
        }
    }
    __device__ void start_qr(SlotS2& S, SlotP2& P) {
        LM& s = S.s;
        const int pc = (s.acnorm[1] > s.acnorm[0]) ? 1 : 0;
        s.ipvt[0] = pc;
        s.ipvt[1] = 1 - pc;
        S.apf = jcol_at(S, pc, 0);
        S.aqf = jcol_at(S, 1 - pc, 0);
// ... 237 lines not shown
    return __hip_atomic_load(p, __ATOMIC_ACQUIRE, __HIP_MEMORY_SCOPE_WORKGROUP);
}
__device__ __forceinline__ void lds_store_rel(int* p, int v) {
    __hip_atomic_store(p, v, __ATOMIC_RELEASE, __HIP_MEMORY_SCOPE_WORKGROUP);
}

__device__ __forceinline__ double chain_sum64(double sum, const double* row) {
#if FM3D_ABL_CHAIN
    return sum + row[0];
#endif
    const double2* R = reinterpret_cast<const double2*>(row);
    double2 v0[4], v1[4], v2[4], v3[4];
    auto ld = [&](double2 (&v)[4], int k) {
#pragma unroll
        for (int i = 0; i < 4; i++) v[i] = R[4 * k + i];
        __asm__ __volatile__("" ::: "memory");
        __builtin_amdgcn_sched_barrier(0);
    };
    auto add = [&](const double2 (&v)[4]) {
#pragma unroll
        for (int i = 0; i < 4; i++) {
            sum += v[i].x;
            sum += v[i].y;
        }
        __asm__ __volatile__("" ::: "memory");
        __builtin_amdgcn_sched_barrier(0);
    };
    ld(v0, 0);
    ld(v1, 1);
    ld(v2, 2);
    ld(v3, 3);
    add(v0);
    ld(v0, 4);
    add(v1);
    ld(v1, 5);
    add(v2);
    ld(v2, 6);
    add(v3);
    ld(v3, 7);
    add(v0);
    add(v1);
    add(v2);
    add(v3);
    return sum;
}

__device__ __forceinline__ int rfl(int v) { return __builtin_amdgcn_readfirstlane(v); }
__device__ __forceinline__ unsigned long long rfl_u64(unsigned long long v) {
    return ((unsigned long long)(unsigned)rfl((int)(v >> 32)) << 32) | (unsigned)rfl((int)v);
}
__device__ __forceinline__ const uint8_t* rfl_ptr(const uint8_t* q) {
    const unsigned long long v = (unsigned long long)q;
    return (const uint8_t*)(((unsigned long long)(unsigned)rfl((int)(v >> 32)) << 32) | (unsigned)rfl((int)v));
}

struct Producer {
    Shared* sh;
    int w, lane, me;
    int cmin;
    unsigned long long deadline;

    __device__ __forceinline__ void reserve(int c) {
        if (c >= cmin + kR) {
            cmin = rfl(min(lds_load_acq(&sh->consumed[w][0]), lds_load_acq(&sh->consumed[w][1])));
            if (c >= cmin + kR) {
                const long long c0 = clock64();
                do {
                    __builtin_amdgcn_s_sleep(1);
                    cmin = rfl(min(lds_load_acq(&sh->consumed[w][0]), lds_load_acq(&sh->consumed[w][1])));
                } while (c >= cmin + kR && wall_clock64() < deadline);
                const unsigned long long dt = clock64() - c0;
                if (lane == 0) sh->ws[me].wait += dt;
            }
        }
    }
    template <bool TWO = true>
    __device__ __forceinline__ void write(int c, double t0, double t1, int slowBits) {
        const int pos = c & (kR - 1);
        double* row0 = &sh->ring[pos][2 * w * kRow];
        row0[lane] = t0;
        if (TWO) row0[kRow + lane] = t1;
#if FM3D_TAG_NOWAIT
        __hip_atomic_store(&sh->rowTag[w][pos], (c << 2) | slowBits, __ATOMIC_RELAXED, __HIP_MEMORY_SCOPE_WORKGROUP);
#else
        __builtin_amdgcn_s_waitcnt(0xc07f);
        lds_store_rel(&sh->rowTag[w][pos], (c << 2) | slowBits);
#endif
    }
    template <bool TWO = true>
    __device__ __forceinline__ void put(int c, double t0, double t1, int slowBits) {
        reserve(c);
        write<TWO>(c, t0, t1, slowBits);
    }
#ifndef FM3D_SLOW_BRANCH
#define FM3D_SLOW_BRANCH 1
#endif
    template <bool TWO = true>
    __device__ __forceinline__ void write_terms(int c, double t0, double v0, bool slow0, double t1, double v1,
                                                bool slow1) {
#if FM3D_SLOW_BRANCH
        const int pos = c & (kR - 1);
        double* row0 = &sh->ring[pos][2 * w * kRow];
        row0[lane] = t0;
        if (TWO) row0[kRow + lane] = t1;
        int slowBits = 0;
        if (slow0 || (TWO && slow1)) {
            asm volatile("" ::: "memory");
            if (slow0) row0[lane] = v0;
            if (TWO && slow1) row0[kRow + lane] = v1;
            slowBits = (slow0 ? 1 : 0) | ((TWO && slow1) ? 2 : 0);
        }
        __builtin_amdgcn_s_waitcnt(0xc07f);
        lds_store_rel(&sh->rowTag[w][pos], (c << 2) | slowBits);
#else
        write<TWO>(c, slow0 ? v0 : t0, slow1 ? v1 : t1, (slow0 ? 1 : 0) | (slow1 ? 2 : 0));
#endif
    }
};

typedef __attribute__((address_space(4))) const ProjConst cProjConst;

__device__ __forceinline__ const cProjConst* proj_consts(const ProjConst* p) {
    int z;
    asm volatile("s_mov_b32 %0, 0" : "=s"(z));
    return (const cProjConst*)((const __attribute__((address_space(4))) char*)p + z);
}
__device__ __forceinline__ const cProjConst* proj_consts(const ProjConst* p, unsigned off) {
    unsigned z;
    asm volatile("s_mov_b32 %0, %1" : "=s"(z) : "s"(off));
    return (const cProjConst*)((const __attribute__((address_space(4))) char*)p + z);
}

typedef unsigned long long LaneMask;
__device__ __forceinline__ double sel_mask(double v, LaneMask m) {
    unsigned lo = __double2loint(v), hi = __double2hiint(v);
    asm("v_cndmask_b32_e64 %0, 0, %0, %1" : "+v"(lo) : "s"(m));
    asm("v_cndmask_b32_e64 %0, 0, %0, %1" : "+v"(hi) : "s"(m));
    return __hiloint2double(hi, lo);
}
__device__ __forceinline__ unsigned sel_mask_u32(unsigned v, LaneMask m) {
    asm("v_cndmask_b32_e64 %0, 0, %0, %1" : "+v"(v) : "s"(m));
    return v;
}
__device__ __forceinline__ LaneMask in_mask(int k, int len) {
    const int rem = len - k * kE;
    return rem >= kE ? ~0ull : (rem <= 0 ? 0ull : ((1ull << rem) - 1));
}

struct Geo2 {
    float fx, fy;
    unsigned off;
    LaneMask inbox, good;
};
template <bool MMOK, bool MULTI>
__device__ __forceinline__ Geo2 geometry2(const LMParams& p, unsigned projOff, double ux, double uy, double n0,
                                          double n1, double n2, double mm, double scale,
                                          unsigned long long xmaxb, unsigned long long ymaxb, int lw, double cm) {
    const cProjConst* pc = MULTI ? proj_consts(p.proj, projOff) : proj_consts(p.proj);
    Geo2 r;
    const double nn = n0 * ux + n1 * uy + n2 * 1.;
    const double kk = MMOK ? div_nn(mm, nn, true) : mm / nn;
    const double P0 = kk * ux, P1 = kk * uy, P2 = kk * 1.;
    r.inbox = __ballot(fabs(P0) < cm) & __ballot(fabs(P1) < cm) & __ballot(P2 > 0.) & __ballot(P2 < cm);
    double x = pc->R[0] * P0 + pc->R[1] * P1 + pc->R[2] * P2 + pc->t[0];
    double y = pc->R[3] * P0 + pc->R[4] * P1 + pc->R[5] * P2 + pc->t[1];
    const double z = recip_z_lo(pc->R[6] * P0 + pc->R[7] * P1 + pc->R[8] * P2 + pc->t[2]);
    x *= z;
    y *= z;
    const double xx = x * x, yy = y * y;
    const double r2 = xx + yy;
    const double r4 = r2 * r2;
    const double r6 = r4 * r2;
    const double xy = x * y;
    const double a2 = __builtin_fma(xx, 2., r2);
    const double a3 = __builtin_fma(yy, 2., r2);
    const double cdist = 1 + pc->cam.k[0] * r2 + pc->cam.k[1] * r4 + pc->cam.k[4] * r6;
    const double xd = x * cdist + pc->k2d * xy + pc->cam.k[3] * a2;
    const double yd = y * cdist + pc->cam.k[2] * a3 + pc->k3d * xy;
    const double u = xd * pc->cam.fx + pc->cam.cx;
    const double v = yd * pc->cam.fy + pc->cam.cy;
    r.good = r.inbox & __ballot((unsigned long long)__double_as_longlong(u) <= xmaxb) &
             __ballot((unsigned long long)__double_as_longlong(v) <= ymaxb);
    r.fx = (float)(scale * u);
    r.fy = (float)(scale * v);
    const unsigned o = __umul24((unsigned)(int)floorf(r.fy), (unsigned)lw) + (unsigned)(int)floorf(r.fx);
    r.off = sel_mask_u32(o, r.good);
    return r;
}

__device__ __noinline__ int plane_code(double ux, double uy, double n0, double n1, double n2, double mm) {
    const double nn = n0 * ux + n1 * uy + n2 * 1.;
    const double kk = mm / nn;
    const double P0 = kk * ux, P1 = kk * uy, P2 = kk * 1.;
    return (P0 != P0 || P1 != P1 || P2 != P2) ? 2 : 3;
}

__device__ __forceinline__ float bilinear_w(unsigned lo, unsigned hi, float x, float y) {
    const float x0 = floorf(x), y0 = floorf(y);
    const float b00 = (float)(lo & 0xff), b01 = (float)((lo >> 8) & 0xff);
    const float b10 = (float)(hi & 0xff), b11 = (float)((hi >> 8) & 0xff);
    const float xm0 = 1.0f - (x - x0), xm1 = (x - x0);
    const float ym0 = 1.0f - (y - y0), ym1 = (y - y0);
    return xm0 * (b00 * ym0 + b10 * ym1) + xm1 * (b01 * ym0 + b11 * ym1);
}

typedef float f32x2 __attribute__((ext_vector_type(2)));
__device__ __forceinline__ float bilinear_f(unsigned lo, unsigned hi, float xf, float yf) {
    const f32x2 b0 = {(float)(lo & 0xff), (float)((lo >> 8) & 0xff)};
    const f32x2 b1 = {(float)(hi & 0xff), (float)((hi >> 8) & 0xff)};
    const float ym0 = 1.0f - yf, ym1 = yf;
    const f32x2 sc = b0 * ym0 + b1 * ym1;
    const f32x2 xm = {1.0f - xf, xf};
    const f32x2 q = xm * sc;
    return q.x + q.y;
}

__device__ __forceinline__ double enorm_term2(double x, double agiant, bool& slow) {
    const double xa = fabs(x);
    slow = (__ballot(!(xa < agiant)) | (__ballot(xa <= 3.834e-20) & __ballot(xa != 0.))) != 0;
    return x * x;
}


__device__ __forceinline__ double chain_slow(int lane, double acc0, const double* row) {
    Enorm en = g_sh.chainEn[lane];
    en.s2 = acc0;
    for (int i = 0; i < kE; i++) en.add(row[i]);
    g_sh.chainEn[lane] = en;
    return en.s2;
}
__device__ __forceinline__ double chain_finish(int lane, double acc) {
    Enorm en = g_sh.chainEn[lane];
    en.s2 = acc;
    return en.finish();
}

__device__ __noinline__ void chain_wave(int lane, unsigned long long tStart, long long maxTicks,
                                        unsigned long long* statBusy, unsigned long long* statRounds) {
    __builtin_amdgcn_s_setprio(3);
    const int s = lane >> 1, which = lane & 1;
    bool alive = s < kW;
    const int ss_ = alive ? s : 0;
    int cur = 0, rem = 0, kind = S_NONE, pid = 0;
    bool inPass = false;
    double acc = 0.;
    unsigned long long busy = 0, tLast = 0, rounds = 0, chunks = 0;
    bool wasBusy = false;
    for (;;) {
        if ((long long)(wall_clock64() - tStart) > maxTicks) break;
        if (!__any(alive)) break;
#ifndef FM3D_CHAIN_ONETRIP
#define FM3D_CHAIN_ONETRIP 1
#endif
#if FM3D_CHAIN_ONETRIP
        auto tagRel = [&](int b) {
            return alive ? __hip_atomic_load(&g_sh.rowTag[ss_][(cur + b) & (kR - 1)], __ATOMIC_RELAXED, __HIP_MEMORY_SCOPE_WORKGROUP) : -1;
        };
        const int tag0 = tagRel(0), tg1 = tagRel(1), tg2 = tagRel(2), tg3 = tagRel(3);
        __builtin_amdgcn_fence(__ATOMIC_ACQUIRE, "workgroup");
#else
        const int tag0 = alive ? lds_load_acq(&g_sh.rowTag[ss_][cur & (kR - 1)]) : -1;
#endif
        const bool have = (tag0 >> 2) == cur;
        if (have && !inPass) {
            const PassDesc& d = g_sh.pd[ss_];
            rem = d.nChunks;
            kind = d.kind[which];
            pid = d.id;
            Enorm& en = g_sh.chainEn[lane];
            en.init(1);
            en.agiant = d.agiant;
            acc = 0.;
            inPass = true;
        }
        if (__any(have)) {
            const unsigned long long t = clock64();
            if (wasBusy) busy += t - tLast;
            tLast = t;
            wasBusy = true;
#ifndef FM3D_CHAIN_NB
#define FM3D_CHAIN_NB 4
#endif
#if FM3D_CHAIN_NB == 4
#if FM3D_CHAIN_ONETRIP
            const int tag1 = (have && rem >= 2) ? tg1 : -1, tag2 = (have && rem >= 3) ? tg2 : -1;
            const int tag3 = (have && rem >= 4) ? tg3 : -1;
#else
            const int tag1 = (have && rem >= 2) ? __hip_atomic_load(&g_sh.rowTag[ss_][(cur + 1) & (kR - 1)], __ATOMIC_RELAXED, __HIP_MEMORY_SCOPE_WORKGROUP) : -1;
            const int tag2 = (have && rem >= 3) ? __hip_atomic_load(&g_sh.rowTag[ss_][(cur + 2) & (kR - 1)], __ATOMIC_RELAXED, __HIP_MEMORY_SCOPE_WORKGROUP) : -1;
            const int tag3 = (have && rem >= 4) ? __hip_atomic_load(&g_sh.rowTag[ss_][(cur + 3) & (kR - 1)], __ATOMIC_RELAXED, __HIP_MEMORY_SCOPE_WORKGROUP) : -1;
            __builtin_amdgcn_fence(__ATOMIC_ACQUIRE, "workgroup");
#endif
            int nb = have ? 1 : 0;
            if (nb == 1 && (tag1 >> 2) == cur + 1) nb = 2;
            if (nb == 2 && (tag2 >> 2) == cur + 2) nb = 3;
            if (nb == 3 && (tag3 >> 2) == cur + 3) nb = 4;
            const int slowm = (tag0 & 3) | ((tag1 & 3) << 2) | ((tag2 & 3) << 4) | ((tag3 & 3) << 6);
#else
            const int tag1 = (have && rem >= 2) ? lds_load_acq(&g_sh.rowTag[ss_][(cur + 1) & (kR - 1)]) : -1;
            const int nb = have ? (((tag1 >> 2) == cur + 1) ? 2 : 1) : 0;
#endif
            rounds++;
            chunks += nb;
#pragma nounroll
            for (int b = 0; b < FM3D_CHAIN_NB; b++) {
                if (b < nb) {
                    const double* row = &g_sh.ring[cur & (kR - 1)][lane * kRow];
#if FM3D_CHAIN_NB == 4
                    const bool slow = ((slowm >> (2 * b + which)) & 1) != 0;
#else
                    const bool slow = (((b ? tag1 : tag0) >> which) & 1) != 0;
#endif
                    const double acc0 = acc;
                    acc = chain_sum64(acc, row);
                    if (kind == S_ENORM && slow) acc = chain_slow(lane, acc0, row);
                    cur++;
                    rem--;
                }
            }
            if (nb > 0) lds_store_rel(&g_sh.consumed[ss_][which], cur);
            if (have && rem == 0) {
                g_sh.result[ss_][which] = kind == S_ENORM ? chain_finish(lane, acc) : acc;
                lds_store_rel(&g_sh.resultId[ss_][which], pid);
                inPass = false;
            }
        } else {
            if (wasBusy) {
                busy += clock64() - tLast;
                wasBusy = false;
            }
            if (alive && !inPass && lds_load_acq(&g_sh.done[ss_])) alive = false;
            __builtin_amdgcn_s_sleep(1);
        }
    }
    if (lane == 0) {
        atomicAdd(statBusy, busy);
        atomicAdd(statRounds, rounds);
    }
    for (int o = 32; o > 0; o >>= 1) chunks += __shfl_xor(chunks, o);
    if (lane == 0) atomicAdd(statRounds + 1, chunks);
}

}

template <bool MULTI, bool TREE>
__global__ __launch_bounds__(kLM2Threads, 4) void lm2_kernel(LMParams p) {
    Shared& sh = g_sh;
    constexpr int NS = TREE ? kWA : kW;
    const int tid = threadIdx.x, lane = tid & 63, wave = tid >> 6;
    const unsigned long long tStart = wall_clock64(), cyStart = clock64();
    if (tid == 0) {
        sh.P = p;
        sh.exited = 0;
    }
    if (tid < NS) {
        for (int k = 0; k < kR; k++) sh.rowTag[tid][k] = -1;
        sh.consumed[tid][0] = sh.consumed[tid][1] = 0;
        sh.resultId[tid][0] = sh.resultId[tid][1] = 0;
        sh.done[tid] = 0;
        sh.helper[tid] = sh.annSeq[tid] = sh.helpDone[tid] = 0;
        sh.hAtt[tid] = -2;
        sh.hSeen[tid] = sh.hAnn[tid] = 0;
    }
    __syncthreads();

    if (wave < NS) {
        const int w = rfl(wave);
        const long gslot = (long)blockIdx.x * NS + w;
        Ctl2& ctl = sh.ctl[w];

        if (lane == 0) {
            ctl.p = &sh.P;
            ctl.sl = slab_of<NS>(p, gslot);
            ctl.tree = TREE;
            ctl.eps = sqrt(p.epsfcn > DBL_EPSILON ? p.epsfcn : DBL_EPSILON);
            ctl.cnt_eval = 0;
            ctl.cnt_pix = 0;
        }
        PassOut2& OUT = sh.out[w];
        Producer prod{&sh, w, lane, w, 0, tStart + (unsigned long long)p.maxTicks};
        int chunkSeq = 0;
        const double cm = (double)p.cmax;
        const gi64* __restrict__ offsets = (const gi64*)p.offsets;
        const unsigned long long ltMask = (1ull << lane) - 1;
        int passId = 0;
        Shared::WaveStat& WS = sh.ws[w];
        if (lane == 0) {
            for (int k = 0; k < 4; k++) WS.cnt[k] = WS.cyc[k] = 0;
            WS.terms = WS.ctl = WS.wait = WS.nPass = WS.iter = 0;
            sh.sp[w].tpend = 0;
            ctl.fetch(sh.ss[w], sh.sp[w]);
        }
        ctl.resolve_trig(sh.ss[w], sh.sp[w], lane);
        for (;;) {
            if ((long long)rfl_u64(lane == 0 ? ++WS.iter : 0) > p.maxIter ||
                (long long)(wall_clock64() - tStart) > p.maxTicks) {
                if (lane == 0) atomicExch(p.overflow, 1);
                break;
            }
            __builtin_amdgcn_fence(__ATOMIC_ACQ_REL, "wavefront");
            bool own = true;
            int hBase = 0;
            if (rfl(sh.hAtt[w]) != -2) {
                int go = 0, att = 0;
                if (lane == 0) {
                    att = sh.hAtt[w];
                    int seen = sh.hSeen[w];
                    for (;;) {
                        if (att >= 0) {
                            if (lds_load_acq(&sh.annSeq[att]) > seen) {
                                seen++;
                                hBase = sh.annBase[att];
                                go = 1;
                                break;
                            }
                            if (lds_load_acq(&sh.done[att])) {
                                att = -1;
                                continue;
                            }
                            if ((long long)(wall_clock64() - tStart) > p.maxTicks) break;
                            __builtin_amdgcn_s_sleep(2);
                            continue;
                        }
                        for (int s = 0; s < kW && att < 0; s++)
                            if (s != w && !lds_load_acq(&sh.done[s]) && lds_load_acq(&sh.helper[s]) == 0 &&
                                atomicCAS(&sh.helper[s], 0, 1) == 0) {
                                att = s;
                                seen = 0;
                            }
                        if (att < 0) break;
                    }
                    sh.hAtt[w] = att;
                    sh.hSeen[w] = seen;
                }
                if (!rfl(go)) break;
                att = rfl(att);
                hBase = rfl(hBase);
                own = false;
                if (prod.w != att) {
                    prod.w = att;
                    prod.cmin = 0;
                }
            }
            const int tw = prod.w;
            SlotP2& SP = sh.sp[tw];
            SlotS2& SS = sh.ss[tw];
            const int pass = rfl(SP.pass);
            if (own && pass == Q_DONE) {
                if (!p.coop) break;
                if (lane == 0) {
                    lds_store_rel(&sh.done[w], 1);
                    sh.hAtt[w] = -1;
                }
                continue;
            }
            if (lane == 0) WS.t0 = clock64();
            const int len = rfl(SP.len);
            const int nCh = (len + kE - 1) / kE;
            int cls = 3;
            if (pass == Q_INIT) {
                const Slab sl2 = ctl.sl;
                const double ccx = SP.ccx, ccy = SP.ccy;
                int base = 0;
                for (int k = 0; k < nCh; k++) {
                    const int e = k * kE + lane;
                    const long long o2 = offsets[e];
                    const double px = ccx + (double)(int)o2, py = ccy + (double)(int)(o2 >> 32);
                    const bool v = !(px < 0 || py < 0 || px >= p.boundW || py >= p.boundH);
                    const unsigned long long bm = __ballot(v);
                    if (v) {
                        const int pos = base + __popcll(bm & ltMask);
                        double ux, uy;
                        undistort1(p.cam, px, py, ux, uy);
#if FM3D_RAY_AOS
                        *(gd2v*)(sl2.RX + 2 * pos) = d2v{ux, uy};
#else
                        sl2.RX[pos] = ux;
                        sl2.RY[pos] = uy;
#endif
                        sl2.KI[pos] = e;
                    }
                    base += __popcll(bm);
                }
                if (lane == 0) OUT.cnt = base;
            } else if (pass == Q_LEVEL) {
                const Slab sl2 = ctl.sl;
                const double ccx = SP.ccx, ccy = SP.ccy, scale = SP.scale, xmax = SP.xmax, ymax = SP.ymax;
                const gu8* img1 = (const gu8*)SP.img1;
                const int lw = rfl(SP.lw);
                bool bad = false;
                for (int k = 0; k < nCh; k++) {
                    const int e = k * kE + lane;
                    if (e < len) {
                        const long long o2 = offsets[sl2.KI[e]];
                        const double px = ccx + (double)(int)o2, py = ccy + (double)(int)(o2 >> 32);
                        if (!pixel_good_b(px, py, xmax, ymax)) {
                            bad = true;
                        } else {
                            const float fx = (float)(scale * px), fy = (float)(scale * py);
                            const gu8* g = img1 + (long)(int)floorf(fy) * lw + (int)floorf(fx);
                            sl2.I1[e] = bilinear4(g[0], g[1], g[lw], g[lw + 1], fx, fy);
                        }
                    }
                }
                const bool anyBad = __ballot(bad) != 0;
                if (lane == 0) OUT.i1fail = anyBad ? 1 : 0;
            } else {
                int cbase = hBase, k0 = 1, kS = 2;
                if (own) {
                    passId++;
                    if (lane == 0) WS.nPass++;
                    cbase = chunkSeq;
                    chunkSeq = cbase + nCh;
                    k0 = 0;
                    kS = (p.coop && rfl(lds_load_acq(&sh.helper[w])) != 0) ? 2 : 1;
                }
                cbase = rfl(cbase);
                k0 = rfl(k0);
                kS = rfl(kS);
                const unsigned s8 = (unsigned)(((size_t)blockIdx.x * NS + tw) * p.nOffPad * 8);
                const int ekind = rfl(SP.ekind);
                const int nev = rfl(SP.nev);
                const bool jac = pass == Q_EVAL && ekind == E_JAC;
                cls = jac ? 0 : (pass == Q_EVAL ? 1 : 2);
                const double agiant = SP.agiant;
                if (!TREE && own && lane == 0) {
                    PassDesc& d = sh.pd[w];
                    d.nChunks = nCh;
                    d.id = passId;
                    d.agiant = agiant;
                    d.kind[0] = (pass == Q_QR1 || pass == Q_QR3) ? S_DOT : S_ENORM;
                    d.kind[1] = pass == Q_QR1 ? S_DOT : ((pass == Q_EVAL && nev == 2) ? S_ENORM : S_NONE);
                    if (kS == 2) {
                        sh.annBase[w] = cbase;
                        sh.annId[w] = passId;
                        lds_store_rel(&sh.annSeq[w], ++sh.hAnn[w]);
                    }
                }
                int fail0 = 0x7fffffff, fail1 = 0x7fffffff;
                int ph30 = 0, ph31 = 0;
                double aqs1 = 0.;
                double ta0 = 0., ta1 = 0., ta2 = 0., ta3 = 0., ta4 = 0.;
                bool tslow0 = false, tslow1 = false;
                if (pass == Q_EVAL) {
                    const double n00 = SP.n0[0], n10 = SP.n1[0], n20 = SP.n2[0], mm0 = SP.mm[0], w0 = SP.w[0];
                    const double n01 = SP.n0[1], n11 = SP.n1[1], n21 = SP.n2[1], mm1 = SP.mm[1], w1 = SP.w[1];
                    const double h0 = SP.hj[0], h1 = SP.hj[1], wF = SP.wF;
                    const double y0 = 1. / h0, y1 = 1. / h1;
                    const bool mok0 = mdiv_ok(h0), mok1 = mdiv_ok(h1);
                    const double scale = SP.scale;
                    const unsigned long long xmaxb = (unsigned long long)__double_as_longlong(SP.xmax);
                    const unsigned long long ymaxb = (unsigned long long)__double_as_longlong(SP.ymax);
                    const uint8_t* img2 = SP.img2;
                    const int lw = rfl(SP.lw);
                    const unsigned projOff = MULTI ? (unsigned)rfl((int)SP.projOff) : 0u;
                    const bool i1ok = rfl(SS.i1ok) != 0;
                    const gu8* img2b = (const gu8*)rfl_ptr(img2);
                    const bool fast = !p.safe && div_nn_ok(mm0) && (nev < 2 || div_nn_ok(mm1)) &&
                                      (!jac || (mok0 && 256. * 1.01 * (w0 + wF) < 1e99 &&
                                                (nev < 2 || (mok1 && 256. * 1.01 * (w1 + wF) < 1e99))));
#ifndef FM3D_EVAL_HOIST
#define FM3D_EVAL_HOIST 1
#endif
                    struct SlabB {
                        const char *slabRX, *slabRY, *slabI1;
                        char *slabDF, *slabDJ0, *slabDJ1;
                    };
                    const SlabB sbh = [&] {
                        const cProjConst* q = proj_consts(p.proj);
                        return SlabB{q->slabRX, q->slabRY, q->slabI1, q->slabDF, q->slabDJ0, q->slabDJ1};
                    }();
                    auto run = [&](auto nevc, auto jacc, auto fastc) {
                        constexpr int NEV = decltype(nevc)::value;
                        constexpr bool JAC = decltype(jacc)::value;
                        constexpr bool FAST = decltype(fastc)::value;
                        auto sb = [&]() {
                            if constexpr (FM3D_EVAL_HOIST && !JAC)
                                return &sbh;
                            else
                                return proj_consts(p.proj);
                        };
                        struct Ld {
                            double ux, uy, dF;
                            float i1;
                        };
                        auto geo = [&](double ux, double uy, double n0, double n1, double n2, double mm) {
                            return FAST ? geometry2<true, MULTI>(p, projOff, ux, uy, n0, n1, n2, mm, scale, xmaxb,
                                                                 ymaxb, lw, cm)
                                        : geometry2<false, MULTI>(p, projOff, ux, uy, n0, n1, n2, mm, scale, xmaxb,
                                                                  ymaxb, lw, cm);
                        };
                        auto jdiv = [&](double a, double h, double y, bool mok) {
                            return FAST ? mdiv_fast(a, h, y) : mdiv(a, h, y, mok);
                        };
                        auto load = [&](unsigned o8, unsigned o4) {
                            const auto* pc = sb();
                            Ld L;
#if FM3D_RAY_AOS
                            const d2v r = __builtin_nontemporal_load((const gd2v*)(pc->slabRX + 2 * o8));
                            L.ux = r.x;
                            L.uy = r.y;
#else
                            L.ux = __builtin_nontemporal_load((const gdouble*)(pc->slabRX + o8));
                            L.uy = __builtin_nontemporal_load((const gdouble*)(pc->slabRY + o8));
#endif
                            L.i1 = __builtin_nontemporal_load((const gfloat*)(pc->slabI1 + o4));
                            L.dF = JAC ? (double)__builtin_nontemporal_load((const gfloat*)(pc->slabDF + o4)) : 0.;
                            return L;
                        };
                        auto gather = [&](unsigned off) {
                            return make_uint2(*(const gu16u*)(img2b + off), *(const gu16u*)(img2b + (off + lw)));
                        };
                        auto chunk = [&](const Ld& L, int k, unsigned o4) {
                            if constexpr (!TREE) prod.reserve(cbase + k);
                            const LaneMask in = in_mask(k, len), ok = i1ok ? in : 0ull;
                            const Geo2 g0 = geo(L.ux, L.uy, n00, n10, n20, mm0);
                            Geo2 g1;
                            if (NEV == 2) g1 = geo(L.ux, L.uy, n01, n11, n21, mm1);
                            const uint2 a = gather(g0.off);
                            uint2 c;
                            if (NEV == 2) c = gather(g1.off);
                            {
                                const LaneMask b0 = in & ~g0.inbox;
                                if (b0 && fail0 == 0x7fffffff) {
                                    const int l = __ffsll((long long)b0) - 1;
                                    const int cd = plane_code(L.ux, L.uy, n00, n10, n20, mm0);
                                    fail0 = (k * kE + l) * 4 + __shfl(cd, l);
                                }
                                ph30 |= (in & g0.inbox & ~g0.good) != 0;
                                if (NEV == 2) {
                                    const LaneMask b1 = in & ~g1.inbox;
                                    if (b1 && fail1 == 0x7fffffff) {
                                        const int l = __ffsll((long long)b1) - 1;
                                        const int cd = plane_code(L.ux, L.uy, n01, n11, n21, mm1);
                                        fail1 = (k * kE + l) * 4 + __shfl(cd, l);
                                    }
                                    ph31 |= (in & g1.inbox & ~g1.good) != 0;
                                }
                            }
                            const float dI0 = L.i1 - bilinear_w(a.x, a.y, g0.fx, g0.fy);
                            const double r0 = w0 * (double)dI0;
                            double v0 = JAC ? jdiv(r0 - wF * L.dF, h0, y0, mok0) : r0;
                            v0 = sel_mask(v0, ok & g0.good);
                            {
                                const auto* pc = sb();
                                *(gfloat*)((JAC ? pc->slabDJ0 : pc->slabDF) + o4) = dI0;
                            }
                            bool slow0 = false, slow1 = false;
                            const double t0 = enorm_term2(v0, agiant, slow0);
                            double v1 = 0., t1 = 0.;
                            if (NEV == 2) {
                                const float dI1 = L.i1 - bilinear_w(c.x, c.y, g1.fx, g1.fy);
                                const double r1 = w1 * (double)dI1;
                                v1 = jdiv(r1 - wF * L.dF, h1, y1, mok1);
                                v1 = sel_mask(v1, ok & g1.good);
                                *(gfloat*)(sb()->slabDJ1 + o4) = dI1;
                                t1 = enorm_term2(v1, agiant, slow1);
                            }
                            if constexpr (TREE) {
                                if (!JAC) {
                                    ta0 += t0;
                                    tslow0 |= slow0;
                                }
                            } else {
                                prod.write_terms<NEV == 2>(cbase + k, t0, v0, slow0, t1, v1, slow1);
                            }
                        };
                        unsigned o8 = s8 + lane * 8u + (unsigned)k0 * 512u, o4 = o8 >> 1;
                        const unsigned st8 = (unsigned)kS * 512u, st4 = st8 >> 1;
                        if (NEV == 2 && FM3D_EVAL_PIPE) {
                            struct St2 {
                                float xf0, yf0, xf1, yf1, i1, dF;
                                uint2 a, c;
                                LaneMask ok0, ok1;
                            };
                            auto front2 = [&](const Ld& L, int k) {
                                const LaneMask in = in_mask(k, len), ok = i1ok ? in : 0ull;
                                const Geo2 g0 = geo(L.ux, L.uy, n00, n10, n20, mm0);
                                const Geo2 g1 = geo(L.ux, L.uy, n01, n11, n21, mm1);
                                St2 S;
                                S.a = gather(g0.off);
                                S.c = gather(g1.off);
                                const LaneMask b0 = in & ~g0.inbox;
                                if (b0 && fail0 == 0x7fffffff) {
                                    const int l = __ffsll((long long)b0) - 1;
                                    const int cd = plane_code(L.ux, L.uy, n00, n10, n20, mm0);
                                    fail0 = (k * kE + l) * 4 + __shfl(cd, l);
                                }
                                ph30 |= (in & g0.inbox & ~g0.good) != 0;
                                const LaneMask b1 = in & ~g1.inbox;
                                if (b1 && fail1 == 0x7fffffff) {
                                    const int l = __ffsll((long long)b1) - 1;
                                    const int cd = plane_code(L.ux, L.uy, n01, n11, n21, mm1);
                                    fail1 = (k * kE + l) * 4 + __shfl(cd, l);
                                }
                                ph31 |= (in & g1.inbox & ~g1.good) != 0;
                                S.xf0 = g0.fx - floorf(g0.fx);
                                S.yf0 = g0.fy - floorf(g0.fy);
                                S.xf1 = g1.fx - floorf(g1.fx);
                                S.yf1 = g1.fy - floorf(g1.fy);
                                S.i1 = L.i1;
                                S.dF = (float)L.dF;
                                S.ok0 = ok & g0.good;
                                S.ok1 = ok & g1.good;
                                return S;
                            };
                            auto back2 = [&](const St2& S, int k, unsigned oo) {
                                const float dI0 = S.i1 - bilinear_f(S.a.x, S.a.y, S.xf0, S.yf0);
                                const float dI1 = S.i1 - bilinear_f(S.c.x, S.c.y, S.xf1, S.yf1);
                                if constexpr (TREE) {
                                    const auto* pc = sb();
                                    *(gfloat*)(pc->slabDJ0 + oo) = dI0;
                                    *(gfloat*)(pc->slabDJ1 + oo) = dI1;
                                    return;
                                }
                                const double F = wF * (double)S.dF;
                                double v0 = jdiv(w0 * (double)dI0 - F, h0, y0, mok0);
                                double v1 = jdiv(w1 * (double)dI1 - F, h1, y1, mok1);
                                v0 = sel_mask(v0, S.ok0);
                                v1 = sel_mask(v1, S.ok1);
                                bool slow0, slow1;
                                const double t0 = enorm_term2(v0, agiant, slow0);
                                const double t1 = enorm_term2(v1, agiant, slow1);
                                prod.reserve(cbase + k);
                                {
                                    const auto* pc = sb();
                                    *(gfloat*)(pc->slabDJ0 + oo) = dI0;
                                    *(gfloat*)(pc->slabDJ1 + oo) = dI1;
                                }
                                prod.write_terms<true>(cbase + k, t0, v0, slow0, t1, v1, slow1);
                            };
                            Ld A = load(o8, o4), B = load(o8 + st8, o4 + st4);
                            St2 S = front2(A, k0), N;
                            A = load(o8 + 2 * st8, o4 + 2 * st4);
                            for (int k = k0; k < nCh; k += 2 * kS) {
                                N = front2(B, k + kS);
                                B = load(o8 + 3 * st8, o4 + 3 * st4);
                                back2(S, k, o4);
                                if (k + kS >= nCh) break;
                                S = front2(A, k + 2 * kS);
                                A = load(o8 + 4 * st8, o4 + 4 * st4);
                                back2(N, k + kS, o4 + st4);
                                o8 += 2 * st8;
                                o4 += 2 * st4;
                            }
                        } else if (NEV == 2) {
                            Ld A = load(o8, o4), B = load(o8 + st8, o4 + st4);
                            for (int k = k0; k < nCh; k += 2 * kS) {
                                const Ld C = load(o8 + 2 * st8, o4 + 2 * st4);
                                chunk(A, k, o4);
                                A = C;
                                if (k + kS < nCh) {
                                    const Ld D = load(o8 + 3 * st8, o4 + 3 * st4);
                                    chunk(B, k + kS, o4 + st4);
                                    B = D;
                                }
                                o8 += 2 * st8;
                                o4 += 2 * st4;
                            }
                        } else if (FM3D_EVAL_PIPE) {
                            struct St {
                                float fxA, fyA, fxB, fyB, i1A, i1B, dFA, dFB;
                                uint2 a, b;
                                LaneMask okA, okB;
                            };
                            auto front = [&](const Ld& A, const Ld& B, int k) {
                                const int kB = k + kS;
                                const LaneMask inA = in_mask(k, len), inB = in_mask(kB, len);
                                const Geo2 gA = geo(A.ux, A.uy, n00, n10, n20, mm0);
                                const Geo2 gB = geo(B.ux, B.uy, n00, n10, n20, mm0);
                                St S;
                                S.a = gather(gA.off);
                                S.b = gather(gB.off);
                                const LaneMask bA = inA & ~gA.inbox;
                                const LaneMask bB = inB & ~gB.inbox;
                                if ((bA | bB) && fail0 == 0x7fffffff) {
                                    const bool first = bA != 0;
                                    const int l = __ffsll((long long)(first ? bA : bB)) - 1;
                                    const int cd = first ? plane_code(A.ux, A.uy, n00, n10, n20, mm0)
                                                         : plane_code(B.ux, B.uy, n00, n10, n20, mm0);
                                    fail0 = ((first ? k : kB) * kE + l) * 4 + __shfl(cd, l);
                                }
                                ph30 |= ((inA & gA.inbox & ~gA.good) | (inB & gB.inbox & ~gB.good)) != 0;
                                S.fxA = gA.fx - floorf(gA.fx);
                                S.fyA = gA.fy - floorf(gA.fy);
                                S.fxB = gB.fx - floorf(gB.fx);
                                S.fyB = gB.fy - floorf(gB.fy);
                                S.i1A = A.i1;
                                S.i1B = B.i1;
                                S.dFA = (float)A.dF;
                                S.dFB = (float)B.dF;
                                S.okA = (i1ok ? inA : 0ull) & gA.good;
                                S.okB = (i1ok ? inB : 0ull) & gB.good;
                                return S;
                            };
                            auto value = [&](float xf, float yf, uint2 w, float i1, float dF, LaneMask ok, float& dI) {
                                dI = i1 - bilinear_f(w.x, w.y, xf, yf);
                                const double r = w0 * (double)dI;
                                const double v = JAC ? jdiv(r - wF * (double)dF, h0, y0, mok0) : r;
                                return sel_mask(v, ok);
                            };
                            auto publish = [&](double v, float dI, unsigned oo, int kk) {
                                {
                                    const auto* pc = sb();
                                    *(gfloat*)((JAC ? pc->slabDJ0 : pc->slabDF) + oo) = dI;
                                }
                                bool slow;
                                const double t = enorm_term2(v, agiant, slow);
                                if constexpr (TREE) {
                                    ta0 += t;
                                    tslow0 |= slow;
                                } else {
                                    prod.write_terms<false>(cbase + kk, t, v, slow, 0., 0., false);
                                }
                            };
                            auto back = [&](const St& S, int k, unsigned oo) {
                                const int kB = k + kS;
                                const bool two = kB < nCh;
                                float dIA, dIB;
                                const double vA = value(S.fxA, S.fyA, S.a, S.i1A, S.dFA, S.okA, dIA);
                                const double vB = value(S.fxB, S.fyB, S.b, S.i1B, S.dFB, S.okB, dIB);
                                if constexpr (!TREE) prod.reserve(cbase + (two ? kB : k));
                                publish(vA, dIA, oo, k);
                                if (two) publish(vB, dIB, oo + st4, kB);
                            };
                            Ld A = load(o8, o4), B = load(o8 + st8, o4 + st4);
                            St S = front(A, B, k0), N;
                            A = load(o8 + 2 * st8, o4 + 2 * st4);
                            B = load(o8 + 3 * st8, o4 + 3 * st4);
                            for (int k = k0; k < nCh; k += 4 * kS) {
                                N = front(A, B, k + 2 * kS);
                                A = load(o8 + 4 * st8, o4 + 4 * st4);
                                B = load(o8 + 5 * st8, o4 + 5 * st4);
                                back(S, k, o4);
                                if (k + 2 * kS >= nCh) break;
                                S = front(A, B, k + 4 * kS);
                                A = load(o8 + 6 * st8, o4 + 6 * st4);
                                B = load(o8 + 7 * st8, o4 + 7 * st4);
                                back(N, k + 2 * kS, o4 + 2 * st4);
                                o8 += 4 * st8;
                                o4 += 4 * st4;
                            }
                        } else {
                            Ld A = load(o8, o4), B = load(o8 + st8, o4 + st4);
                            for (int k = k0; k < nCh; k += 2 * kS) {
                                const int kB = k + kS;
                                const bool two = kB < nCh;
                                if constexpr (!TREE) prod.reserve(cbase + (two ? kB : k));
                                const LaneMask inA = in_mask(k, len), inB = in_mask(kB, len);
                                const Geo2 gA = geo(A.ux, A.uy, n00, n10, n20, mm0);
                                const Geo2 gB = geo(B.ux, B.uy, n00, n10, n20, mm0);
                                const uint2 a = gather(gA.off), b = gather(gB.off);
                                const float i1A = A.i1, i1B = B.i1;
                                const double dFA = A.dF, dFB = B.dF;
                                const LaneMask bA = inA & ~gA.inbox;
                                const LaneMask bB = inB & ~gB.inbox;
                                if ((bA | bB) && fail0 == 0x7fffffff) {
                                    const bool first = bA != 0;
                                    const int l = __ffsll((long long)(first ? bA : bB)) - 1;
                                    const int cd = first ? plane_code(A.ux, A.uy, n00, n10, n20, mm0)
                                                         : plane_code(B.ux, B.uy, n00, n10, n20, mm0);
                                    fail0 = ((first ? k : kB) * kE + l) * 4 + __shfl(cd, l);
                                }
                                ph30 |= ((inA & gA.inbox & ~gA.good) | (inB & gB.inbox & ~gB.good)) != 0;
                                A = load(o8 + 2 * st8, o4 + 2 * st4);
                                B = load(o8 + 3 * st8, o4 + 3 * st4);
                                auto back1 = [&](const Geo2& g, uint2 w, float i1, double dF, LaneMask in, unsigned oo, int kk) {
                                    const float dI = i1 - bilinear_w(w.x, w.y, g.fx, g.fy);
                                    const double r = w0 * (double)dI;
                                    double v = JAC ? jdiv(r - wF * dF, h0, y0, mok0) : r;
                                    v = sel_mask(v, (i1ok ? in : 0ull) & g.good);
                                    {
                                        const auto* pc = sb();
                                        *(gfloat*)((JAC ? pc->slabDJ0 : pc->slabDF) + oo) = dI;
                                    }
                                    bool slow;
                                    const double t = enorm_term2(v, agiant, slow);
                                    if constexpr (TREE) {
                                        ta0 += t;
                                        tslow0 |= slow;
                                    } else {
                                        prod.write_terms<false>(cbase + kk, t, v, slow, 0., 0., false);
                                    }
                                };
                                back1(gA, a, i1A, dFA, inA, o4, k);
                                if (two) back1(gB, b, i1B, dFB, inB, o4 + st4, kB);
                                o8 += 2 * st8;
                                o4 += 2 * st4;
                            }
                        }
                    };
                    using I1 = std::integral_constant<int, 1>;
                    using I2 = std::integral_constant<int, 2>;
                    using T = std::true_type;
                    using F = std::false_type;
                    if (fast) {
                        if (nev == 2)
                            run(I2(), T(), T());
                        else if (jac)
                            run(I1(), T(), T());
                        else
                            run(I1(), F(), T());
                    } else {
                        if (nev == 2)
                            run(I2(), T(), F());
                        else if (jac)
                            run(I1(), T(), F());
                        else
                            run(I1(), F(), F());
                    }
                } else {
                    const int pc = rfl(SP.pivot), t0f = rfl(SP.t0), t1f = rfl(SP.t1), q0f = rfl(SP.q0);
                    const double wF = SP.wF, wp = SP.w[pc], wq = SP.w[1 - pc], hp = SP.hj[pc], hq = SP.hj[1 - pc];
                    const double yp = 1. / hp, yq = 1. / hq;
                    const bool mokp = mdiv_ok(hp), mokq = mdiv_ok(hq);
                    const double ajn0s = SP.ajn0s, ya0 = 1. / ajn0s, tq = SP.tq;
                    const bool moka0 = mdiv_ok(ajn0s);
                    const double ajn1s = SP.ajn1s, ya1 = 1. / ajn1s, tq0 = SP.tq0;
                    const bool moka1 = mdiv_ok(ajn1s);
                    const double bnum = 256. * 1.01 * (wp + wq + 2. * wF);
                    const double bap = bnum / fabs(hp), baq = bnum / fabs(hq);
                    bool fast = !p.safe && t0f && q0f && mokp && mokq && moka0 && bnum < 1e99 && bap < 1e99 &&
                                baq < 1e99 && (pass != Q_QR3 || (t1f && moka1 &&
                                baq + fabs(tq) * (bap / fabs(ajn0s) + 1.) < 1e99));
                    if constexpr (TREE)
                        if (pass == Q_GRAM) fast = !p.safe && mokp && mokq && bnum < 1e99 && bap < 1e99 && baq < 1e99;
                    auto run = [&](auto kindc, auto fastc) {
                        constexpr int KIND = decltype(kindc)::value;
                        constexpr bool FAST = decltype(fastc)::value;
                        struct Ld {
                            float p, q, f;
                        };
#ifndef FM3D_QR_HOIST
#define FM3D_QR_HOIST 1
#endif
#if FM3D_QR_HOIST
                        const cProjConst* pcs0 = proj_consts(p.proj);
                        const char* const Dp0 = pc ? pcs0->slabDJ1 : pcs0->slabDJ0;
                        const char* const Dq0 = pc ? pcs0->slabDJ0 : pcs0->slabDJ1;
                        const char* const Df0 = pcs0->slabDF;
#endif
                        auto load = [&](unsigned o4) {
#if FM3D_QR_HOIST
                            const char* Dp = Dp0;
                            const char* Dq = Dq0;
                            struct {
                                const char* slabDF;
                            } s0{Df0}, *pcs = &s0;
#else
                            const cProjConst* pcs = proj_consts(p.proj);
                            const char* Dp = pc ? pcs->slabDJ1 : pcs->slabDJ0;
                            const char* Dq = pc ? pcs->slabDJ0 : pcs->slabDJ1;
#endif
                            Ld L;
                            L.p = __builtin_nontemporal_load((const gfloat*)(Dp + o4));
                            L.q = __builtin_nontemporal_load((const gfloat*)(Dq + o4));
                            L.f = __builtin_nontemporal_load((const gfloat*)(pcs->slabDF + o4));
                            return L;
                        };
                        auto dv = [&](double a, double d, double y, bool mok) {
                            return FAST ? mdiv_fast(a, d, y) : mdiv(a, d, y, mok);
                        };
                        struct Terms {
                            double t0, t1, a;
                            bool slow;
                            double g0, g1, g2;
                            bool slow1;
                        };
                        auto chunk = [&](const Ld& L, int k, auto edgec) {
                            constexpr bool EDGE = decltype(edgec)::value;
                            const int e = k * kE + lane;
                            const bool in = e < len;
                            const double F = wF * (double)L.f;
                            const double ap = dv(wp * (double)L.p - F, hp, yp, mokp);
                            const double aq = dv(wq * (double)L.q - F, hq, yq, mokq);
                            double t0 = 0., t1 = 0., a = 0., g0 = 0., g1 = 0., g2 = 0.;
                            bool slow = false, slow1 = false;
                            if constexpr (KIND == Q_GRAM) {
                                const double a0 = (EDGE && !in) ? 0. : ap, a1 = (EDGE && !in) ? 0. : aq;
                                const double f = (EDGE && !in) ? 0. : F;
                                t0 = enorm_term2(a0, agiant, slow);
                                t1 = enorm_term2(a1, agiant, slow1);
                                g0 = a0 * a1;
                                g1 = a0 * f;
                                g2 = a1 * f;
                            } else if constexpr (KIND == Q_QR1) {
                                double v = dv(ap, ajn0s, ya0, moka0);
                                if (EDGE && e == 0) v = v + 1.;
                                t0 = v * aq;
                                t1 = v * F;
                                if (EDGE && !in) t0 = t1 = 0.;
                            } else if constexpr (KIND == Q_QR2) {
                                a = aq;
                                if (FAST || t0f) a = a - tq * dv(ap, ajn0s, ya0, moka0);
                                if (EDGE) {
                                    a = (in && e > 0) ? a : 0.;
                                    if (e == 1) aqs1 = a;
                                }
                                t0 = enorm_term2(a, agiant, slow);
                            } else {
                                const double v = (FAST || t0f) ? dv(ap, ajn0s, ya0, moka0) : 0.;
                                double b = aq;
                                if (FAST || t0f) b = b - tq * v;
                                double u = (FAST || t1f) ? dv(b, ajn1s, ya1, moka1) : b;
                                if (EDGE && (FAST || t1f) && e == 1) u = u + 1.;
                                double wa = F;
                                if (FAST || q0f) wa = wa + v * tq0;
                                t0 = u * wa;
                                if (EDGE && !(in && e > 0)) t0 = 0.;
                            }
                            return Terms{t0, t1, a, slow, g0, g1, g2, slow1};
                        };
#ifndef FM3D_QR_DEPTH
#define FM3D_QR_DEPTH 8
#endif
                        constexpr int kQD = FM3D_QR_DEPTH;
                        unsigned o4 = (s8 >> 1) + lane * 4u + (unsigned)k0 * 256u;
                        const unsigned st4 = (unsigned)kS * 256u;
                        Ld buf[kQD];
#pragma unroll
                        for (int j = 0; j < kQD; j++) {
// ... 12 lines not shown
                                        if (KIND == Q_QR1 || KIND == Q_GRAM) ta1 += T.t1;
                                        if (KIND == Q_GRAM) {
                                            ta2 += T.g0;
                                            ta3 += T.g1;
                                            ta4 += T.g2;
                                            tslow1 |= T.slow1;
                                        }
                                        tslow0 |= T.slow;
                                    } else {
                                        prod.reserve(cbase + kc);
                                        prod.write_terms<KIND == Q_QR1>(cbase + kc, T.t0, T.a, T.slow, T.t1, 0., false);
                                    }
                                    buf[j] = load(o4);
                                }
                                o4 += st4;
                            }
                        }
                    };
                    if (TREE && pass == Q_GRAM) {
                        if constexpr (TREE) {
                            if (fast)
                                run(std::integral_constant<int, Q_GRAM>(), std::true_type());
                            else
                                run(std::integral_constant<int, Q_GRAM>(), std::false_type());
                        }
                    } else if (fast) {
                        if (pass == Q_QR1)
                            run(std::integral_constant<int, Q_QR1>(), std::true_type());
                        else if (pass == Q_QR2)
                            run(std::integral_constant<int, Q_QR2>(), std::true_type());
                        else
                            run(std::integral_constant<int, Q_QR3>(), std::true_type());
                    } else {
                        if (pass == Q_QR1)
                            run(std::integral_constant<int, Q_QR1>(), std::false_type());
                        else if (pass == Q_QR2)
                            run(std::integral_constant<int, Q_QR2>(), std::false_type());
                        else
                            run(std::integral_constant<int, Q_QR3>(), std::false_type());
                    }
                    aqs1 = __shfl(aqs1, 1);
                }
                if (!own) {
                    __builtin_amdgcn_s_waitcnt(0);
                    if (lane == 0) {
                        sh.hfail[tw][0] = fail0;
                        sh.hfail[tw][1] = fail1;
                        sh.hph3[tw][0] = ph30 != 0;
                        sh.hph3[tw][1] = ph31 != 0;
                        lds_store_rel(&sh.helpDone[tw], sh.annId[tw]);
                    }
                } else if constexpr (TREE) {
                    const bool two = pass == Q_QR1 || pass == Q_GRAM;
                    const bool gram = pass == Q_GRAM;
                    for (int o = 32; o > 0; o >>= 1) {
                        ta0 += __shfl_xor(ta0, o);
                        if (two) ta1 += __shfl_xor(ta1, o);
                        if (gram) {
                            ta2 += __shfl_xor(ta2, o);
                            ta3 += __shfl_xor(ta3, o);
                            ta4 += __shfl_xor(ta4, o);
                        }
                    }
                    const bool en = (pass == Q_EVAL && !jac) || pass == Q_QR2 || pass == Q_GRAM;
                    if (lane == 0) {
                        double r0 = ta0, r1 = ta1;
                        if (en) {
                            r0 = tslow0 ? ctl.seq_enorm(SP, pass == Q_QR2 ? 3 : (pass == Q_GRAM ? 1 : 0), len) : sqrt(ta0);
                            if (two) r1 = tslow1 ? ctl.seq_enorm(SP, 2, len) : sqrt(ta1);
                        }
                        OUT.nrm[0] = OUT.sum[0] = r0;
                        OUT.nrm[1] = OUT.sum[1] = r1;
                        OUT.sq[0] = ta0;
                        OUT.sq[1] = ta1;
                        OUT.g[0] = ta2;
                        OUT.g[1] = ta3;
                        OUT.g[2] = ta4;
                        OUT.slow = (tslow0 ? 1 : 0) | (tslow1 ? 2 : 0);
                        OUT.fail[0] = fail0;
                        OUT.fail[1] = fail1;
                        OUT.ph3[0] = ph30 != 0;
                        OUT.ph3[1] = ph31 != 0;
                        OUT.aqs1 = aqs1;
                    }
                } else {
                    const long long c0 = clock64();
                    while ((lds_load_acq(&sh.resultId[w][0]) != passId || lds_load_acq(&sh.resultId[w][1]) != passId) &&
                           wall_clock64() < prod.deadline)
                        __builtin_amdgcn_s_sleep(1);
                    bool hp0 = false, hp1 = false;
                    if (kS == 2) {
                        while (lds_load_acq(&sh.helpDone[w]) != passId && wall_clock64() < prod.deadline)
                            __builtin_amdgcn_s_sleep(1);
                        fail0 = min(fail0, sh.hfail[w][0]);
                        fail1 = min(fail1, sh.hfail[w][1]);
                        hp0 = sh.hph3[w][0] != 0;
                        hp1 = sh.hph3[w][1] != 0;
                    }
                    if (lane == 0) {
                        WS.wait += clock64() - c0;
                        OUT.nrm[0] = OUT.sum[0] = sh.result[w][0];
                        OUT.nrm[1] = OUT.sum[1] = sh.result[w][1];
                        OUT.fail[0] = fail0;
                        OUT.fail[1] = fail1;
                        OUT.ph3[0] = ph30 != 0 || hp0;
                        OUT.ph3[1] = ph31 != 0 || hp1;
                        OUT.aqs1 = aqs1;
                    }
                }
            }
            __builtin_amdgcn_s_waitcnt(0);
            __builtin_amdgcn_fence(__ATOMIC_ACQ_REL, "wavefront");
            if (lane == 0) {
                const unsigned long long tp1 = clock64();
                if (own) ctl.after_pass(SS, SP, OUT);
                const unsigned long long tp2 = clock64();
                WS.terms += tp1 - WS.t0;
                WS.ctl += tp2 - tp1;
                WS.cnt[cls]++;
                WS.cyc[cls] += tp2 - WS.t0;
            }
            if (own) ctl.resolve_trig(SS, SP, lane);
            __builtin_amdgcn_s_waitcnt(0);
        }
        if (lane == 0) {
            lds_store_rel(&sh.done[w], 1);
            atomicAdd(p.statEval, (unsigned long long)ctl.cnt_eval);
            atomicAdd(p.statPix, (unsigned long long)ctl.cnt_pix);
            atomicAdd(p.statPass + 0, WS.nPass);
            atomicAdd(p.statPass + 1, WS.terms);
            atomicAdd(p.statPass + 3, WS.ctl);
            for (int k = 0; k < 4; k++) {
                atomicAdd(p.statPass + 7 + k, WS.cnt[k]);
                atomicAdd(p.statPass + 11 + k, WS.cyc[k]);
            }
            atomicAdd(p.statPass + 21, WS.wait);
        }
    } else {
        chain_wave(lane, tStart, p.maxTicks, p.statPass + 2, p.statPass + 18);
    }
    bool lastWave = false;
    if (lane == 0) lastWave = TREE ? atomicAdd(&sh.exited, 1) == NS - 1 : wave == kW;
    if (lastWave) {
        atomicAdd(p.statPass + 4, clock64() - cyStart);
        const unsigned long long wt = wall_clock64() - tStart;
        atomicAdd(p.statPass + 5, wt);
        atomicMax(p.statPass + 6, wt);
        atomicMax(p.statPass + 15, tStart);
        atomicMax(p.statPass + 16, wall_clock64());
        atomicMin(p.statPass + 17, tStart);
    }
}

template __global__ void lm2_kernel<false, false>(LMParams p);
template __global__ void lm2_kernel<true, false>(LMParams p);
template __global__ void lm2_kernel<false, true>(LMParams p);
template __global__ void lm2_kernel<true, true>(LMParams p);

}
```

3dfeaturematcher_amd/csrc/fm3d_misc.hip:

```cpp
#include <hip/hip_runtime.h>
#include <stdint.h>

#include "fm3d_kernels.h"

namespace fm3d {

namespace {

template <int P, int Q>
__device__ __forceinline__ bool jacobi_pair(double* A, double* V) {
    double alpha = 0, beta = 0, gamma = 0;
#pragma unroll
    for (int i = 0; i < 4; i++) {
        double ap = A[i * 4 + P], aq = A[i * 4 + Q];
        alpha += ap * ap;
        beta += aq * aq;
        gamma += ap * aq;
    }
    if (gamma != 0. && fabs(gamma) > 1e-15 * sqrt(alpha * beta)) {
        double zeta = (beta - alpha) / (2. * gamma);
        double t = (zeta >= 0. ? 1. : -1.) / (fabs(zeta) + sqrt(1. + zeta * zeta));
        double cs = 1. / sqrt(1. + t * t);
        double sn = cs * t;
#pragma unroll
        for (int i = 0; i < 4; i++) {
            double ap = A[i * 4 + P], aq = A[i * 4 + Q];
            A[i * 4 + P] = cs * ap - sn * aq;
            A[i * 4 + Q] = sn * ap + cs * aq;
            ap = V[i * 4 + P];
            aq = V[i * 4 + Q];
            V[i * 4 + P] = cs * ap - sn * aq;
            V[i * 4 + Q] = sn * ap + cs * aq;
        }
        return true;
    }
    return false;
}
__device__ inline void dlt_nullvec(double* A, double* v) {
    double V[16];
#pragma unroll
    for (int i = 0; i < 16; i++) V[i] = (i % 5 == 0) ? 1. : 0.;
    for (int sweep = 0; sweep < 30; sweep++) {
        bool rotated = jacobi_pair<0, 1>(A, V);
        rotated |= jacobi_pair<2, 3>(A, V);
        rotated |= jacobi_pair<0, 2>(A, V);
        rotated |= jacobi_pair<1, 3>(A, V);
        rotated |= jacobi_pair<0, 3>(A, V);
        rotated |= jacobi_pair<1, 2>(A, V);
        if (!rotated) break;
    }
    double nrm[4];
#pragma unroll
    for (int p = 0; p < 4; p++) {
        double s = 0;
#pragma unroll
        for (int i = 0; i < 4; i++) s += A[i * 4 + p] * A[i * 4 + p];
        nrm[p] = s;
    }
    int best = 0;
#pragma unroll
    for (int p = 1; p < 4; p++)
        if (nrm[p] < nrm[best]) best = p;
#pragma unroll
    for (int i = 0; i < 4; i++) v[i] = best == 0 ? V[i * 4] : best == 1 ? V[i * 4 + 1] : best == 2 ? V[i * 4 + 2] : V[i * 4 + 3];
}

constexpr int kTriThreads = 64;
__device__ __forceinline__ bool tri_one(const TriParams& p, int i, double* X) {
    const fm3d_dmatch mt = p.matches[i];
    const fm3d_point2f k1 = p.kp1[mt.queryIdx - p.queryOffset];
    const fm3d_point2f k2 = p.kp2[mt.trainIdx];
    double u1x, u1y, u2x, u2y;
    undistort1(p.cam, (double)k1.x, (double)k1.y, u1x, u1y);
    undistort1(p.cam, (double)k2.x, (double)k2.y, u2x, u2y);
    if (p.dltSolver == 0) {
        fm3d_cv::triangulate_point(p.g12, u1x, u1y, u2x, u2y, X);
    } else {
        double A[16];
        const double P1[12] = {1, 0, 0, 0, 0, 1, 0, 0, 0, 0, 1, 0};
        for (int k = 0; k < 4; k++) {
            A[0 * 4 + k] = u1x * P1[8 + k] - P1[0 + k];
            A[1 * 4 + k] = u1y * P1[8 + k] - P1[4 + k];
            A[2 * 4 + k] = u2x * p.g12[8 + k] - p.g12[0 + k];
            A[3 * 4 + k] = u2y * p.g12[8 + k] - p.g12[4 + k];
        }
        dlt_nullvec(A, X);
    }
    const bool out = (X[2] / X[3] < p.zmin || X[2] / X[3] >= p.zmax);
    p.mask[i] = out ? 0 : 1;
    if (p.mask8) p.mask8[i] = out ? 0 : 1;
    return !out;
}
__global__ __launch_bounds__(kTriThreads) void triangulate_kernel(TriParams p) {
    const int i = blockIdx.x * blockDim.x + threadIdx.x;
    if (i >= (p.Kdev ? *p.Kdev : p.K)) return;
    double X[4];
    tri_one(p, i, X);
    p.pts[3 * i + 0] = X[0] / X[3];
    p.pts[3 * i + 1] = X[1] / X[3];
    p.pts[3 * i + 2] = X[2] / X[3];
}
__global__ __launch_bounds__(kTriThreads) void triangulate_compact_kernel(TriParams p, double* __restrict__ out,
                                                                          int* __restrict__ srcIdx,
                                                                          int* __restrict__ count, LookBack lb,
                                                                          int* hostCnt) {
    __shared__ int sBid;
    const int lane = threadIdx.x;
    if (lane == 0) sBid = lookback_block_id(lb);
    __syncthreads();
    const int bid = sBid;
    const int i = bid * kTriThreads + lane;
    double X[4];
    const bool inl = i < (p.Kdev ? *p.Kdev : p.K) && tri_one(p, i, X);
    const unsigned long long bal = __ballot(inl);
    const int ex = lookback_exclusive(lb.st, lb.epoch, bid, __popcll(bal));
    const int o = ex + __popcll(bal & ((1ull << lane) - 1));
    if (inl) {
        out[3 * o + 0] = X[0] / X[3];
        out[3 * o + 1] = X[1] / X[3];
        out[3 * o + 2] = X[2] / X[3];
        srcIdx[o] = i;
    }
    if (lane == 0 && bid == (int)gridDim.x - 1) {
        const int total = ex + __popcll(bal);
        *count = total;
        if (hostCnt) {
            __hip_atomic_store(&hostCnt[0], p.Kdev ? *p.Kdev : p.K, __ATOMIC_RELAXED, __HIP_MEMORY_SCOPE_SYSTEM);
            __hip_atomic_store(&hostCnt[1], total, __ATOMIC_RELAXED, __HIP_MEMORY_SCOPE_SYSTEM);
        }
    }
}

__global__ void lm_reset_kernel(LMReset r, int maxP) {
    const int t = blockIdx.x * blockDim.x + threadIdx.x;
    if (t < 32) r.stat[t] = t == 20 ? ~0ull : 0ull;
    if (r.queue && t < 64) r.queue[t] = 0;
    for (int j = 0; j < r.nProb; j++) {
        if (t < 4) r.pcnt16[j][t] = 0;
        if (t < r.P[j]) r.status[j][t] = kLMRunning;
        if (t < 8 * r.P[j]) {
            r.info[j][t] = 0;
            r.nfev[j][t] = 0;
        }
    }
    (void)maxP;
}

__device__ inline int reflect101(int q, int len) {
    if (len == 1) return 0;
    while (q < 0 || q >= len) q = q < 0 ? -q : 2 * len - q - 2;
    return q;
}

__global__ void pyrdown_kernel(const uint8_t* __restrict__ src, int w, int h, uint8_t* __restrict__ dst) {
    const int dw = (w + 1) / 2, dh = (h + 1) / 2;
    const int x = blockIdx.x * blockDim.x + threadIdx.x;
    const int y = blockIdx.y * blockDim.y + threadIdx.y;
    if (x >= dw || y >= dh) return;
    const int wt[5] = {1, 4, 6, 4, 1};
    int sx[5];
    for (int j = 0; j < 5; j++) sx[j] = reflect101(2 * x + j - 2, w);
    int s = 0;
    for (int i = 0; i < 5; i++) {
        const uint8_t* row = src + (size_t)reflect101(2 * y + i - 2, h) * w;
        int rs = 0;
        for (int j = 0; j < 5; j++) rs += wt[j] * row[sx[j]];
        s += wt[i] * rs;
    }
    dst[(size_t)y * dw + x] = (uint8_t)((s + 128) >> 8);
}

__global__ void undistort_kernel(Camera cam, const double* __restrict__ xy, int n, double* __restrict__ out) {
    const int i = blockIdx.x * blockDim.x + threadIdx.x;
    if (i >= n) return;
    undistort1(cam, xy[2 * i], xy[2 * i + 1], out[2 * i], out[2 * i + 1]);
}

struct EpiMat {
    double e[9];
};
__global__ void epipolar_lines_kernel(Camera cam, EpiMat E, const fm3d_point2f* __restrict__ kp1, int n1,
                                      const fm3d_point2f* __restrict__ kp2, int n2, float4* __restrict__ lines,
                                      float2* __restrict__ uv) {
    const int i = blockIdx.x * blockDim.x + threadIdx.x;
    if (i >= n1 + n2) return;
    const fm3d_point2f k = i < n1 ? kp1[i] : kp2[i - n1];
    double x, y;
    undistort1(cam, (double)k.x, (double)k.y, x, y);
    if (i >= n1) {
        uv[i - n1] = make_float2((float)x, (float)y);
        return;
    }
    const double l0 = (E.e[0] * x + E.e[1] * y) + E.e[2];
    const double l1 = (E.e[3] * x + E.e[4] * y) + E.e[5];
    const double l2 = (E.e[6] * x + E.e[7] * y) + E.e[8];
    const double n = sqrt(l0 * l0 + l1 * l1);
    const float a = (float)(l0 / n), b = (float)(l1 / n), c = (float)(l2 / n);
    const float inf = __builtin_inff();
    const bool ok = n != 0. && fabsf(a) < inf && fabsf(b) < inf && fabsf(c) < inf;
    lines[i] = ok ? make_float4(a, b, c, 0.f) : make_float4(0.f, 0.f, inf, 0.f);
}

__global__ void plane_project_kernel(PlaneProjParams p) {
    const int t = blockIdx.x * blockDim.x + threadIdx.x;
    if (t >= p.nOff) return;
    const double I[9] = {1, 0, 0, 0, 1, 0, 0, 0, 1}, Z[3] = {0, 0, 0};
    double cx, cy;
    project1(p.cam, I, Z, p.X[0], p.X[1], p.X[2], cx, cy);
    const int2 o = p.offsets[t];
    const double px = cx + o.x, py = cy + o.y;
    const int keep = !(px < 0 || py < 0 || px >= p.boundW || py >= p.boundH);
    p.keep[t] = keep;
    p.xy[2 * t] = px;
    p.xy[2 * t + 1] = py;
    if (!keep) return;
    double ux, uy;
    undistort1(p.cam, px, py, ux, uy);
    const double mm = p.n[0] * p.X[0] + p.n[1] * p.X[1] + p.n[2] * p.X[2];
    const double nn = p.n[0] * ux + p.n[1] * uy + p.n[2] * 1.;
    const double k = mm / nn;
    const double P0 = k * ux, P1 = k * uy, P2 = k * 1.;
    const double cm = p.cmax;
    int st = 0;
    if (P0 != P0 || P1 != P1 || P2 != P2) st = 5;
    else if (!((P0 > -cm && P0 < cm) && (P1 > -cm && P1 < cm) && (P2 > 0. && P2 < cm))) st = 2;
    double u, v;
    project1(p.cam, p.R2, p.t2, P0, P1, P2, u, v);
    if (!st && p.w > 0 && !pixel_good(u, v, 1.0, p.w, p.h)) st = 4;
    p.uv[2 * t] = u;
    p.uv[2 * t + 1] = v;
    p.status[t] = st;
}

constexpr int kScanBlock = 1024;

__device__ __forceinline__ int dev_count(const int* nDev, int n) {
    if (!nDev) return n;
    const int d = *nDev;
    return d < n ? d : n;
}

__global__ void scan_count_kernel(const int* __restrict__ flag, int n, const int* __restrict__ nDev,
                                  int* __restrict__ blockSums) {
    __shared__ int red[256];
    n = dev_count(nDev, n);
    const int base = blockIdx.x * kScanBlock;
    int c = 0;
    for (int k = 0; k < 4; k++) {
        int i = base + threadIdx.x * 4 + k;
        c += (i < n && flag[i]) ? 1 : 0;
    }
    red[threadIdx.x] = c;
    __syncthreads();
    for (int s = 128; s > 0; s >>= 1) {
        if ((int)threadIdx.x < s) red[threadIdx.x] += red[threadIdx.x + s];
        __syncthreads();
    }
    if (threadIdx.x == 0) blockSums[blockIdx.x] = red[0];
}

__global__ void scan_blocks_kernel(int* __restrict__ blockSums, int nb, int* __restrict__ total) {
    __shared__ int buf[1024];
    __shared__ int carry;
    if (threadIdx.x == 0) carry = 0;
    __syncthreads();
    for (int c0 = 0; c0 < nb; c0 += 1024) {
        const int i = c0 + threadIdx.x;
        int v = (i < nb) ? blockSums[i] : 0;
        buf[threadIdx.x] = v;
        __syncthreads();
        for (int off = 1; off < 1024; off <<= 1) {
            int t = (int)threadIdx.x >= off ? buf[threadIdx.x - off] : 0;
            __syncthreads();
            buf[threadIdx.x] += t;
            __syncthreads();
        }
        const int incl = buf[threadIdx.x];
        if (i < nb) blockSums[i] = carry + incl - v;
        __syncthreads();
        if (threadIdx.x == 1023) carry += incl;
        __syncthreads();
    }
    if (threadIdx.x == 0 && total) *total = carry;
}

__device__ inline int block_local_offset(const int* flag, int n, int base, int* sh, int& c4, int f[4]) {
    c4 = 0;
    for (int k = 0; k < 4; k++) {
        int i = base + threadIdx.x * 4 + k;
        f[k] = (i < n && flag[i]) ? 1 : 0;
        c4 += f[k];
    }
    sh[threadIdx.x] = c4;
    __syncthreads();
    for (int off = 1; off < 256; off <<= 1) {
        int t = (int)threadIdx.x >= off ? sh[threadIdx.x - off] : 0;
        __syncthreads();
        sh[threadIdx.x] += t;
        __syncthreads();
    }
    return sh[threadIdx.x] - c4;
}

template <typename T>
__global__ void scatter_kernel(const T* __restrict__ in, const int* __restrict__ flag, int n,
                               const int* __restrict__ nDev, const int* __restrict__ blockOff, T* __restrict__ out,
                               int* __restrict__ srcIndex) {
    __shared__ int sh[256];
    n = dev_count(nDev, n);
    const int base = blockIdx.x * kScanBlock;
    int c4, f[4];
    int o = blockOff[blockIdx.x] + block_local_offset(flag, n, base, sh, c4, f);
    for (int k = 0; k < 4; k++) {
        int i = base + threadIdx.x * 4 + k;
        if (f[k]) {
            out[o] = in[i];
            if (srcIndex) srcIndex[o] = i;
            o++;
        }
    }
}

struct Point3 {
    double v[3];
};

__global__ void offsets_kernel(const int* __restrict__ flag, int n, const int* __restrict__ blockOff,
                               int* __restrict__ offsets) {
    __shared__ int sh[256];
    const int base = blockIdx.x * kScanBlock;
    int c4, f[4];
    int o = blockOff[blockIdx.x] + block_local_offset(flag, n, base, sh, c4, f);
    for (int k = 0; k < 4; k++) {
        int i = base + threadIdx.x * 4 + k;
        if (i < n) offsets[i] = o;
        o += f[k];
    }
}

constexpr int kSmallCompact = 16384;

template <typename T>
__global__ __launch_bounds__(1024) void compact_small_kernel(const T* __restrict__ in, const int* __restrict__ flag,
                                                             int n, const int* __restrict__ nDev, T* __restrict__ out,
                                                             int* __restrict__ count, int* __restrict__ srcIndex,
                                                             int* __restrict__ offsets) {
    __shared__ int wt[256];
    __shared__ int ws4[4];
    __shared__ int totS;
    n = dev_count(nDev, n);
    const int tid = threadIdx.x, lane = tid & 63, wid = tid >> 6;
    const int ipt = (n + 1023) >> 10;
    bool f[16];
#pragma unroll
    for (int it = 0; it < 16; it++) {
        const int i = it * 1024 + tid;
        f[it] = it < ipt && i < n && flag[i] != 0;
    }
    const unsigned long long below = (1ull << lane) - 1ull;
    int pre[16];
#pragma unroll
    for (int it = 0; it < 16; it++) {
        const unsigned long long b = __ballot(f[it]);
        pre[it] = __popcll(b & below);
        if (lane == 0) wt[it * 16 + wid] = __popcll(b);
    }
    __syncthreads();
    int v = 0, x = 0;
    if (tid < 256) {
        v = wt[tid];
        x = v;
        for (int o = 1; o < 64; o <<= 1) {
            const int y = __shfl_up(x, o);
            if (lane >= o) x += y;
        }
        if (lane == 63) ws4[wid] = x;
    }
    __syncthreads();
    if (tid < 256) {
        int add = 0;
        for (int w = 0; w < wid; w++) add += ws4[w];
        wt[tid] = add + x - v;
        if (tid == 255) totS = add + x;
    }
    __syncthreads();
#pragma unroll
    for (int it = 0; it < 16; it++) {
        const int i = it * 1024 + tid;
        if (it < ipt && i < n) {
            const int o = wt[it * 16 + wid] + pre[it];
            if (offsets) offsets[i] = o;
            if (f[it]) {
                if (out) out[o] = in[i];
                if (srcIndex) srcIndex[o] = i;
            }
        }
    }
    if (tid == 0 && count) *count = totS;
}

template <typename T>
void compact(const T* in, const int* flag, int n, const int* nDev, T* out, int* count, int* srcIndex, void* tmp,
             hipStream_t s) {
    const int nb = (n + kScanBlock - 1) / kScanBlock;
    int* blockSums = (int*)tmp;
    if (n <= 0) {
        hipMemsetAsync(count, 0, sizeof(int), s);
        return;
    }
    if (n <= kSmallCompact) {
        compact_small_kernel<T><<<1, 1024, 0, s>>>(in, flag, n, nDev, out, count, srcIndex, nullptr);
        return;
    }
    scan_count_kernel<<<nb, 256, 0, s>>>(flag, n, nDev, blockSums);
    scan_blocks_kernel<<<1, 1024, 0, s>>>(blockSums, nb, count);
    scatter_kernel<T><<<nb, 256, 0, s>>>(in, flag, n, nDev, blockSums, out, srcIndex);
}

__global__ void make_records_kernel(const fm3d_dmatch* __restrict__ matches, const int* __restrict__ inlierSrc,
                                    int nInl, const int* __restrict__ nDev, const double* __restrict__ pts,
                                    const double* __restrict__ normals, const int* __restrict__ status,
                                    fm3d_record* __restrict__ rec, int* __restrict__ flag) {
    const int i = blockIdx.x * blockDim.x + threadIdx.x;
    if (i >= dev_count(nDev, nInl)) return;
    const fm3d_dmatch m = matches[inlierSrc[i]];
    fm3d_record r;
    r.queryIdx = m.queryIdx;
    r.trainIdx = m.trainIdx;
    r.distance = m.distance;
    r.status = status[i];
    for (int k = 0; k < 3; k++) {
        r.point[k] = pts[3 * i + k];
        r.normal[k] = normals[3 * i + k];
    }
    rec[i] = r;
    flag[i] = status[i] == FM3D_ST_OK ? 1 : 0;
}

}

void launch_triangulate(const TriParams& p, hipStream_t s) {
    if (p.K <= 0) return;
    triangulate_kernel<<<(p.K + kTriThreads - 1) / kTriThreads, kTriThreads, 0, s>>>(p);
}

int triangulate_compact_blocks(int K) { return K > 0 ? (K + kTriThreads - 1) / kTriThreads : 1; }

void launch_triangulate_compact(const TriParams& p, double* out, int* srcIdx, int* count, const LookBack& lb,
                                hipStream_t s, int* hostCnt) {
    triangulate_compact_kernel<<<triangulate_compact_blocks(p.K), kTriThreads, 0, s>>>(p, out, srcIdx, count, lb,
                                                                                      hostCnt);
}

void launch_lm_reset(const LMReset& r, hipStream_t s) {
    int maxP = 0;
    for (int j = 0; j < r.nProb; j++) maxP = r.P[j] > maxP ? r.P[j] : maxP;
    const long n = 8L * maxP > 64 ? 8L * maxP : 64;
    lm_reset_kernel<<<(unsigned)((n + 255) / 256), 256, 0, s>>>(r, maxP);
}

void launch_pyrdown(const uint8_t* src, int w, int h, uint8_t* dst, hipStream_t s) {
    const int dw = (w + 1) / 2, dh = (h + 1) / 2;
    dim3 blk(32, 8), grd((dw + 31) / 32, (dh + 7) / 8);
    pyrdown_kernel<<<grd, blk, 0, s>>>(src, w, h, dst);
}

void launch_plane_project(const PlaneProjParams& p, hipStream_t s) {
    if (p.nOff > 0) plane_project_kernel<<<(p.nOff + 255) / 256, 256, 0, s>>>(p);
}

void launch_undistort(const Camera& cam, const double* xy, int n, double* out, hipStream_t s) {
    if (n <= 0) return;
    undistort_kernel<<<(n + 255) / 256, 256, 0, s>>>(cam, xy, n, out);
}

void launch_epipolar_setup(const Camera& cam, const double E[9], const fm3d_point2f* kp1, int n1,
                           const fm3d_point2f* kp2, int n2, float4* lines, float2* uv, hipStream_t s) {
    if (n1 + n2 <= 0) return;
    EpiMat m;
    for (int k = 0; k < 9; k++) m.e[k] = E[k];
    epipolar_lines_kernel<<<(n1 + n2 + 255) / 256, 256, 0, s>>>(cam, m, kp1, n1, kp2, n2, lines, uv);
}

size_t scan_tmp_bytes(int n) { return sizeof(int) * ((size_t)(n + kScanBlock - 1) / kScanBlock + 16); }

void launch_compact_dmatch(const fm3d_dmatch* in, const int* flag, int n, fm3d_dmatch* out, int* count, void* tmp,
                           hipStream_t s, const int* nDev) {
    compact<fm3d_dmatch>(in, flag, n, nDev, out, count, nullptr, tmp, s);
}

void launch_compact_points(const double* in, const int* flag, int n, const int* nDev, double* out, int* count,
                           int* srcIndex, void* tmp, hipStream_t s) {
    compact<Point3>((const Point3*)in, flag, n, nDev, (Point3*)out, count, srcIndex, tmp, s);
}

void launch_exclusive_scan(const int* flag, int n, int* offsets, int* total, void* tmp, hipStream_t s) {
    const int nb = (n + kScanBlock - 1) / kScanBlock;
    int* blockSums = (int*)tmp;
    if (n <= 0) {
        hipMemsetAsync(total, 0, sizeof(int), s);
        return;
    }
    if (n <= kSmallCompact) {
        compact_small_kernel<int><<<1, 1024, 0, s>>>(nullptr, flag, n, nullptr, nullptr, total, nullptr, offsets);
        return;
    }
    scan_count_kernel<<<nb, 256, 0, s>>>(flag, n, nullptr, blockSums);
    scan_blocks_kernel<<<1, 1024, 0, s>>>(blockSums, nb, total);
    offsets_kernel<<<nb, 256, 0, s>>>(flag, n, blockSums, offsets);
}

void launch_make_records(const fm3d_dmatch* matches, const int* inlierSrc, int nInl, const int* nDev, const double* pts,
                         const double* normals, const int* status, fm3d_record* rec, int* flag, hipStream_t s) {
    if (nInl <= 0) return;
    make_records_kernel<<<(nInl + 255) / 256, 256, 0, s>>>(matches, inlierSrc, nInl, nDev, pts, normals, status, rec,
                                                            flag);
}

void launch_compact_records(const fm3d_record* in, const int* flag, int n, const int* nDev, fm3d_record* out,
                            int* count, void* tmp, hipStream_t s) {
    compact<fm3d_record>(in, flag, n, nDev, out, count, nullptr, tmp, s);
}

}
```

3dfeaturematcher_amd/csrc/fm3d_pipeline.cpp:

```cpp
#include <cstdlib>
#include <cstring>
#include <vector>

#include "fm3d_ctx.h"
#include "fm3d_internal.h"

using namespace fm3d_host;

namespace {

int require(fm3d_ctx* c, Need need) {
    if (need == Need::StagedIdle && (!c || !c->staged)) return fail(c, FM3D_ERR_INVALID, "fm3d_pipeline_upload not called");
    if (!c) return FM3D_ERR_INVALID;
    const PairState s = c->pipe.state;
    if (need != Need::StagedIdle && need != Need::Idle) {
        if (s == PairState::Verified && need != Need::Verified)
            return fail(c, FM3D_ERR_INVALID, "a verified frame pair is pending: fm3d_pipeline_wait_verified");
        if (s == PairState::DltVerified && need != Need::DltVerified)
            return fail(c, FM3D_ERR_INVALID, "a verified front half is pending: fm3d_pipeline_wait_dlt_verified");
    }
    if (need == Need::Verified && s != PairState::Verified)
        return fail(c, FM3D_ERR_INVALID, "no verified frame pair submitted (fm3d_pipeline_submit_verified)");
    if (need == Need::DltVerified && s != PairState::DltVerified)
        return fail(c, FM3D_ERR_INVALID, "no verified front half submitted (fm3d_pipeline_submit_dlt_verified)");
// ... 519 lines not shown
    if ((r = verify_report(c, rep))) return r;
    if (out && kept > cap) return fail(c, FM3D_ERR_INVALID, "record buffer too small");
    if (out && kept)
        HIPCHK(c, hipMemcpy(out, c->pipe.pendOut, (size_t)kept * sizeof(fm3d_record), hipMemcpyDeviceToHost));
    if (nKept) *nKept = kept;
    return FM3D_OK;
}

int fm3d_pipeline_submit_dlt_verified(fm3d_ctx* c, const fm3d_verify_opts* o) {
    int r;
    if ((r = check_verified_submit(c, o, Need::StagedIdle))) return r;
    hipSetDevice(c->device);
    if ((r = enqueue_verified(c, o, true))) return r;
    c->pipe.state = PairState::DltVerified;
    return FM3D_OK;
}

int fm3d_pipeline_wait_dlt_verified(fm3d_ctx* c, int* nInliers, fm3d_pipeline_stats* stats, fm3d_verify_report* rep) {
    int r;
    if (!c || !rep) return fail(c, FM3D_ERR_INVALID, "null argument");
    if ((r = require(c, Need::DltVerified))) return r;
    hipSetDevice(c->device);
    c->pipe.state = PairState::Idle;
    HIPCHK(c, hipEventSynchronize(c->ev[EV_END]));
    if ((r = verify_report(c, rep))) return r;
    report_front_counts(c, nInliers, stats);
    return FM3D_OK;
}

int fm3d_pipeline_submit_ncc(fm3d_ctx* c, int Hphi, int Htheta, double span) {
    int r;
    if ((r = require(c, Need::StagedIdle))) return r;
    if (Hphi <= 0 || Htheta <= 0 || Hphi * Htheta > 32) return fail(c, FM3D_ERR_INVALID, "1 <= Hphi * Htheta <= 32");
    if (!c->haveG12) return fail(c, FM3D_ERR_INVALID, "fm3d_set_g12 / fm3d_setg12 not called");
    hipSetDevice(c->device);
    c->nccP = 0;
    if ((r = pipeline_front(c))) return r;
    const int nA = c->pipe.nA;
    const int H = Hphi * Htheta;
    HIPCHK(c, hipEventRecord(c->ev[EV_NORMAL_START], c->stream));
    if (nA > 0) {
        if ((r = ensure_offsets(c))) return r;
        HIPCHK(c, c->nccS.ensure((size_t)nA * H * sizeof(double)));
        HIPCHK(c, c->nccN.ensure((size_t)nA * 3 * sizeof(double)));
        HIPCHK(c, c->nccB.ensure((size_t)nA * sizeof(int)));
        fm3d::NccParams p = ncc_params(c, Hphi, Htheta, span);
        p.points = c->pts.as<double>();
        p.P = nA;
        p.Pdev = c->pcnt.as<int>() + 1;
        p.scores = c->nccS.as<double>();
        p.normals = c->nccN.as<double>();
        p.best = c->nccB.as<int>();
        fm3d::launch_ncc_hypotheses(p, c->stream);
        HIPCHK(c, hipGetLastError());
    }
    HIPCHK(c, hipEventRecord(c->ev[EV_NORMAL_END], c->stream));
    HIPCHK(c, c->hSmall.ensure(sizeof(PipeSmall)));
    PipeSmall* hs = c->hSmall.as<PipeSmall>();
    HIPCHK(c, hipMemcpyAsync(hs->cnt, c->pcnt.p, sizeof(hs->cnt), hipMemcpyDeviceToHost, c->stream));
    HIPCHK(c, hipEventRecord(c->ev[EV_END], c->stream));
    c->pipe.state = PairState::Ncc;
    c->pipe.nccHPending = H;
    return FM3D_OK;
}

int fm3d_pipeline_wait_ncc(fm3d_ctx* c, int* nPoints, fm3d_pipeline_stats* stats) {
    if (int r = require(c, Need::Ncc)) return r;
    hipSetDevice(c->device);
    c->pipe.state = PairState::Idle;
    HIPCHK(c, hipEventSynchronize(c->ev[EV_END]));
    const PipeSmall* hs = c->hSmall.as<PipeSmall>();
    const int K = hs->cnt[0], P = hs->cnt[1];
    c->pipe.K = K;
    c->pipe.P = P;
    c->nccH = c->pipe.nccHPending;
    c->nccP = P;
    if (nPoints) *nPoints = P;
    if (stats) {
        stats_head(c, K, P, true, stats);
        stats->kept = P;
        float ms;
        hipEventElapsedTime(&ms, c->ev[EV_NORMAL_START], c->ev[EV_NORMAL_END]);
        stats->lm_ms = ms;
        hipEventElapsedTime(&ms, c->ev[EV_FRONT_START], c->ev[EV_END]);
        stats->total_ms = ms;
    }
    return FM3D_OK;
}

int fm3d_pipeline_run_ncc(fm3d_ctx* c, int Hphi, int Htheta, double span, int* nPoints, fm3d_pipeline_stats* stats) {
    if (int r = fm3d_pipeline_submit_ncc(c, Hphi, Htheta, span)) return r;
    return fm3d_pipeline_wait_ncc(c, nPoints, stats);
}

int fm3d_pipeline_ncc_download(fm3d_ctx* c, double* scores, double* normals, int32_t* best) {
    if (!c || !c->staged) return FM3D_ERR_INVALID;
    if (int r = require(c, Need::Idle)) return r;
    hipSetDevice(c->device);
    const size_t P = (size_t)c->nccP;
    if (P && scores) HIPCHK(c, hipMemcpy(scores, c->nccS.p, P * c->nccH * sizeof(double), hipMemcpyDeviceToHost));
    if (P && normals) HIPCHK(c, hipMemcpy(normals, c->nccN.p, P * 3 * sizeof(double), hipMemcpyDeviceToHost));
    if (P && best) HIPCHK(c, hipMemcpy(best, c->nccB.p, P * sizeof(int), hipMemcpyDeviceToHost));
    return FM3D_OK;
}

int fm3d_pipeline_dlt_download(fm3d_ctx* c, fm3d_dmatch* matches, double* points, int32_t* matchIdx) {
    if (!c || !c->staged) return FM3D_ERR_INVALID;
    if (int r = require(c, Need::Idle)) return r;
    hipSetDevice(c->device);
    if (matches && c->pipe.K) HIPCHK(c, hipMemcpy(matches, c->matches.p, (size_t)c->pipe.K * sizeof(fm3d_dmatch), hipMemcpyDeviceToHost));
    if (points && c->pipe.P) HIPCHK(c, hipMemcpy(points, c->pts.p, (size_t)c->pipe.P * 3 * sizeof(double), hipMemcpyDeviceToHost));
    if (matchIdx && c->pipe.P) HIPCHK(c, hipMemcpy(matchIdx, c->srcIdx.p, (size_t)c->pipe.P * sizeof(int), hipMemcpyDeviceToHost));
    return FM3D_OK;
}

}

int fm3d_internal_submit_to(fm3d_ctx* c, const void* descA, int nA, const void* descB, int nB, int dim, int type,
                            const fm3d_point2f* kpts1, const fm3d_point2f* kpts2, const uint8_t* img1,
                            const uint8_t* img2, int width, int height, fm3d_record* recordsDev) {
    return submit_impl(c, {descA, nA, descB, nB, dim, type, kpts1, kpts2, img1, img2, width, height, 0}, recordsDev);
}

int fm3d_internal_flush(fm3d_ctx* c) { return c ? flush_member(c) : FM3D_ERR_INVALID; }
bool fm3d_internal_front_only(const fm3d_ctx* c) { return c && c->pipe.state == PairState::MemberFront; }

int fm3d_internal_enqueue(fm3d_ctx* c, fm3d_record* recordsDev) {
    int r;
    if ((r = require(c, Need::StagedIdle))) return r;
    hipSetDevice(c->device);
    HIPCHK(c, hipEventRecord(c->ev[EV_SUBMIT_START], c->stream));
    c->pipe.subLm = fm3d_lm_stats{};
    if ((r = enqueue_full(c, recordsDev, &c->pipe.subLm))) return r;
    c->pipe.state = PairState::Full;
    return FM3D_OK;
}

int fm3d_internal_finish(fm3d_ctx* c, int* nKept, fm3d_pipeline_stats* stats) {
    if (!c || c->pipe.state == PairState::Idle) return fail(c, FM3D_ERR_INVALID, "nothing pending");
    hipSetDevice(c->device);
    c->pipe.state = PairState::Idle;
    return finalize_full(c, c->pipe.subLm, c->ev[EV_SUBMIT_START], true, nKept, stats);
}

const int* fm3d_internal_kept_dev(fm3d_ctx* c) { return c->pcnt.as<int>() + 2; }
hipStream_t fm3d_internal_stream(fm3d_ctx* c) { return c->stream; }
int fm3d_internal_memory_need(fm3d_ctx* c, int64_t nA, int64_t nB, int dim, int type, int width, int height,
                              size_t* bytes) {
    hipSetDevice(c->device);
    int r;
    if ((r = ensure_offsets(c))) return r;
    const bool tree = c->s.lmReduction != 0;
    const int slots = fm3d::kLM2Slots + (tree ? 1 : 0);
    const void* kptr = tree ? reinterpret_cast<const void*>(fm3d::lm2_kernel<true, true>)
                            : reinterpret_cast<const void*>(fm3d::lm2_kernel<true, false>);
    long groups = 0;
    if ((r = lm_groups(c, kptr, slots, -1, &groups))) return r;
    const size_t ents = (size_t)c->nOffPad * slots;
    size_t need = ents * (2 * sizeof(double) + 5 * 4) * groups + 32768;
    const size_t rowIn = type == FM3D_DESC_F32 ? (size_t)dim * 4 : (size_t)dim;
    const size_t rowWork = 256 + (type == FM3D_DESC_F32 ? (size_t)dim * 4 : 0);
    need += (size_t)(nA + nB) * (rowIn + rowWork) + (size_t)nB * 64;
    if (c->s.guidedMatchPx > 0.) need += (size_t)nA * 16 + (size_t)nB * 8;
    if (c->s.crossCheck != 0) need += (size_t)(nA + nB) * (rowWork + 8) + (size_t)nB * (24 + 16 * 16);
    need += (size_t)nA * 1536;
    need += (size_t)width * height * 4 + ((size_t)16 << 20);
    *bytes = need;
    return FM3D_OK;
}

int fm3d_internal_alloc_probe(fm3d_ctx* c, size_t bytes, uint8_t* out) {
    if (!c || !bytes || !out) return fail(c, FM3D_ERR_INVALID, "alloc_probe: null context, no bytes or null out");
    hipSetDevice(c->device);
    DevBuf b;
    HIPCHK(c, b.ensure(bytes));
    HIPCHK(c, hipMemcpy(out, b.p, bytes, hipMemcpyDeviceToHost));
    return FM3D_OK;
}

int fm3d_internal_prepare(fm3d_ctx* c) {
    hipSetDevice(c->device);
    HIPCHK(c, c->pcnt.ensure(64));
    return FM3D_OK;
}
```

Before: 33940.

## Add column-major img2 pyramid and select LM sampling layout by epipolar direction

Builds a transposed, column-major copy of every image-2 pyramid level, through a tiled transpose for level 0 and a second store inside pyrdown for the other levels. The LM kernel gets a COLS template variant that gathers bilinear samples from this copy. The host turns that variant on when the projected epipolar direction is mostly vertical. This is meant to make neighbouring lanes' image gathers fall in contiguous memory and cut scattered HBM traffic, at the cost of extra memory, transpose work on every image upload, and twice as many kernel instantiations.

```diff
diff --git a/3dfeaturematcher_amd/csrc/fm3d_ctx.h b/3dfeaturematcher_amd/csrc/fm3d_ctx.h
--- a/3dfeaturematcher_amd/csrc/fm3d_ctx.h
+++ b/3dfeaturematcher_amd/csrc/fm3d_ctx.h
@@ -100,6 +100,8 @@
 using HostBuf = Buf<PinnedMem>;
 
 constexpr size_t kGuard(int w) { return (size_t)4 * w + 64; }
+constexpr int kColStride(int h) { return (h + 2 + 63) / 64 * 64; }
+constexpr size_t kColBytes(int w, int h) { return (size_t)(w + 2) * kColStride(h) + 64; }
 
 struct PipeSmall {
     int32_t cnt[4];
@@ -149,6 +151,8 @@
     int w = 0, h = 0;
     std::vector<int> lw, lh;
     std::vector<DevBuf> pyr1, pyr2;
+    std::vector<DevBuf> pyr2t;
+    int lmCols = -1;
     int pyrGuardW = -1, pyrGuardH = -1, pyrGuardLevels = -1;
     DevBuf lvlDesc;
     DevBuf offsets;
diff --git a/3dfeaturematcher_amd/csrc/fm3d_host.cpp b/3dfeaturematcher_amd/csrc/fm3d_host.cpp
--- a/3dfeaturematcher_amd/csrc/fm3d_host.cpp
+++ b/3dfeaturematcher_amd/csrc/fm3d_host.cpp
@@ -10,6 +10,7 @@
 
 #include "fm3d.h"
 #include "fm3d_ctx.h"
+#include "fm3d_internal.h"
 #include "fm3d_kernels.h"
 
 using fm3d::LevelDesc;
@@ -117,6 +118,7 @@
     c->lh.assign(levels + 1, 0);
     c->pyr1.resize(levels + 1);
     c->pyr2.resize(levels + 1);
+    c->pyr2t.resize(levels + 1);
     c->lw[0] = width;
     c->lh[0] = height;
     for (int L = 1; L <= levels; L++) {
@@ -128,14 +130,17 @@
         size_t bytes = (size_t)c->lw[L] * c->lh[L] + kGuard(c->lw[L]);
         void* p1 = c->pyr1[L].p;
         void* p2 = c->pyr2[L].p;
+        void* pt = c->pyr2t[L].p;
         HIPCHK(c, c->pyr1[L].ensure(bytes));
         HIPCHK(c, c->pyr2[L].ensure(bytes));
-        fresh |= c->pyr1[L].p != p1 || c->pyr2[L].p != p2;
+        HIPCHK(c, c->pyr2t[L].ensure(kColBytes(c->lw[L], c->lh[L])));
+        fresh |= c->pyr1[L].p != p1 || c->pyr2[L].p != p2 || c->pyr2t[L].p != pt;
     }
     for (int L = 0; fresh && L <= levels; L++) {
         const size_t img = (size_t)c->lw[L] * c->lh[L];
         HIPCHK(c, hipMemsetAsync((char*)c->pyr1[L].p + img, 0, c->pyr1[L].bytes - img, c->stream));
         HIPCHK(c, hipMemsetAsync((char*)c->pyr2[L].p + img, 0, c->pyr2[L].bytes - img, c->stream));
+        HIPCHK(c, hipMemsetAsync(c->pyr2t[L].p, 0, c->pyr2t[L].bytes, c->stream));
     }
     c->pyrGuardW = width;
     c->pyrGuardH = height;
@@ -148,16 +153,20 @@
     }
     HIPCHK(c, hipMemcpyAsync(c->pyr1[0].p, c->hImg.p, wh, hipMemcpyHostToDevice, c->stream));
     HIPCHK(c, hipMemcpyAsync(c->pyr2[0].p, c->hImg.as<uint8_t>() + wh, wh, hipMemcpyHostToDevice, c->stream));
+    fm3d::launch_level_transpose(c->pyr2[0].as<uint8_t>(), width, height, c->pyr2t[0].as<uint8_t>(), kColStride(height),
+                                 c->stream);
     for (int L = 1; L <= levels; L++) {
         fm3d::launch_pyrdown(c->pyr1[L - 1].as<uint8_t>(), c->lw[L - 1], c->lh[L - 1], c->pyr1[L].as<uint8_t>(),
                              c->stream);
         fm3d::launch_pyrdown(c->pyr2[L - 1].as<uint8_t>(), c->lw[L - 1], c->lh[L - 1], c->pyr2[L].as<uint8_t>(),
-                             c->stream);
+                             c->stream, c->pyr2t[L].as<uint8_t>(), kColStride(c->lh[L]));
     }
     HIPCHK(c, hipGetLastError());
     HIPCHK(c, c->hTab.ensure((levels + 1) * sizeof(LevelDesc)));
     LevelDesc* d = c->hTab.as<LevelDesc>();
-    for (int L = 0; L <= levels; L++) d[L] = LevelDesc{c->pyr1[L].as<uint8_t>(), c->pyr2[L].as<uint8_t>(), c->lw[L], c->lh[L]};
+    for (int L = 0; L <= levels; L++)
+        d[L] = LevelDesc{c->pyr1[L].as<uint8_t>(), c->pyr2[L].as<uint8_t>(), c->lw[L], c->lh[L],
+                         c->pyr2t[L].as<uint8_t>(), kColStride(c->lh[L])};
     HIPCHK(c, c->lvlDesc.ensure((levels + 1) * sizeof(LevelDesc)));
     HIPCHK(c, hipMemcpyAsync(c->lvlDesc.p, d, (levels + 1) * sizeof(LevelDesc), hipMemcpyHostToDevice, c->stream));
     HIPCHK(c, hipEventRecord(c->evStage, c->stream));
@@ -349,6 +358,20 @@
     }
     return FM3D_OK;
 }
+
+int fm3d_internal_level_cols(fm3d_ctx* c, int level, uint8_t* out, int* w, int* h, int* hs, size_t* bytes) {
+    if (!c || level < 0 || level >= (int)c->pyr2t.size()) return FM3D_ERR_INVALID;
+    hipSetDevice(c->device);
+    const size_t n = kColBytes(c->lw[level], c->lh[level]);
+    if (w) *w = c->lw[level];
+    if (h) *h = c->lh[level];
+    if (hs) *hs = kColStride(c->lh[level]);
+    if (bytes) *bytes = n;
+    if (out) HIPCHK(c, hipMemcpy(out, c->pyr2t[level].p, n, hipMemcpyDeviceToHost));
+    return FM3D_OK;
+}
+
+int fm3d_internal_lm_img2_cols(const fm3d_ctx* c) { return c ? c->lmCols : -1; }
 
 int fm3d_records_download(fm3d_ctx* c, const fm3d_record* recordsDev, int n, fm3d_record* out) {
     if (!c || n < 0 || (n && !out)) return FM3D_ERR_INVALID;
diff --git a/3dfeaturematcher_amd/csrc/fm3d_internal.h b/3dfeaturematcher_amd/csrc/fm3d_internal.h
--- a/3dfeaturematcher_amd/csrc/fm3d_internal.h
+++ b/3dfeaturematcher_amd/csrc/fm3d_internal.h
@@ -17,3 +17,6 @@
 int fm3d_internal_memory_need(fm3d_ctx* c, int64_t nA, int64_t nB, int dim, int type, int width, int height,
                               size_t* bytes);
 extern "C" int fm3d_internal_alloc_probe(fm3d_ctx* c, size_t bytes, uint8_t* out);
+extern "C" int fm3d_internal_level_cols(fm3d_ctx* c, int level, uint8_t* out, int* w, int* h, int* hs,
+                                        size_t* bytes);
+extern "C" int fm3d_internal_lm_img2_cols(const fm3d_ctx* c);
diff --git a/3dfeaturematcher_amd/csrc/fm3d_kernels.h b/3dfeaturematcher_amd/csrc/fm3d_kernels.h
--- a/3dfeaturematcher_amd/csrc/fm3d_kernels.h
+++ b/3dfeaturematcher_amd/csrc/fm3d_kernels.h
@@ -16,6 +16,8 @@
     const uint8_t* img1;
     const uint8_t* img2;
     int w, h;
+    const uint8_t* img2t;
+    int hs;
 };
 
 struct ProjConst {
@@ -81,7 +83,7 @@
 constexpr int kLM2Slots = 15;
 constexpr int kLM2Ring = 8;
 constexpr int kLM2Threads = 64 * (kLM2Slots + 1);
-template <bool MULTI, bool TREE>
+template <bool MULTI, bool TREE, bool COLS>
 __global__ void lm2_kernel(LMParams p);
 
 struct KnnOut {
@@ -365,7 +367,8 @@
                                 hipStream_t s, int* hostCnt = nullptr);
 int triangulate_compact_blocks(int K);
 
-void launch_pyrdown(const uint8_t* src, int w, int h, uint8_t* dst, hipStream_t s);
+void launch_pyrdown(const uint8_t* src, int w, int h, uint8_t* dst, hipStream_t s, uint8_t* dstT = nullptr, int hs = 0);
+void launch_level_transpose(const uint8_t* src, int w, int h, uint8_t* dstT, int hs, hipStream_t s);
 void launch_undistort(const Camera& cam, const double* xy, int n, double* out, hipStream_t s);
 
 bool math_probe_binary(int fn);
diff --git a/3dfeaturematcher_amd/csrc/fm3d_lm.cpp b/3dfeaturematcher_amd/csrc/fm3d_lm.cpp
--- a/3dfeaturematcher_amd/csrc/fm3d_lm.cpp
+++ b/3dfeaturematcher_amd/csrc/fm3d_lm.cpp
@@ -1,3 +1,4 @@
+#include <cmath>
 #include <cstdlib>
 #include <cstring>
 #include <vector>
@@ -63,6 +64,23 @@
     if (groups < 1) groups = 1;
     *out = groups;
     return FM3D_OK;
+}
+
+bool lm_prefers_cols(const fm3d_ctx* q) {
+    const fm3d::Camera& k = q->cam;
+    const double z = 0.5 * (q->s.zThresholdMin + q->s.zThresholdMax);
+    const double X[2][3] = {{0., 0., z}, {0., z / k.fy, z}};
+    double u[2], v[2];
+    for (int i = 0; i < 2; i++) {
+        const double* R = q->R2;
+        const double x = R[0] * X[i][0] + R[1] * X[i][1] + R[2] * X[i][2] + q->t2[0];
+        const double y = R[3] * X[i][0] + R[4] * X[i][1] + R[5] * X[i][2] + q->t2[1];
+        const double w = R[6] * X[i][0] + R[7] * X[i][1] + R[8] * X[i][2] + q->t2[2];
+        if (!(w > 0.)) return false;
+        u[i] = k.fx * x / w;
+        v[i] = k.fy * y / w;
+    }
+    return std::fabs(v[1] - v[0]) > std::fabs(u[1] - u[0]);
 }
 
 int run_lm_multi(fm3d_ctx* c, const LMSrc* src, int nProb, fm3d_lm_stats* stats, hipEvent_t e0, hipEvent_t e1) {
@@ -100,10 +118,25 @@
     for (int j = 1; j < nProb; j++)
         multiPose |= std::memcmp(src[j].c->R2, src[0].c->R2, sizeof(c->R2)) != 0 ||
                      std::memcmp(src[j].c->t2, src[0].c->t2, sizeof(c->t2)) != 0;
-    const void* kptr = tree ? (multiPose ? reinterpret_cast<const void*>(fm3d::lm2_kernel<true, true>)
-                                         : reinterpret_cast<const void*>(fm3d::lm2_kernel<false, true>))
-                            : (multiPose ? reinterpret_cast<const void*>(fm3d::lm2_kernel<true, false>)
-                                         : reinterpret_cast<const void*>(fm3d::lm2_kernel<false, false>));
+    bool cols = true;
+    for (int j = 0; j < nProb; j++) cols &= lm_prefers_cols(src[j].c);
+    if (const char* lay = getenv("FM3D_LM_IMG2")) {
+        if (!std::strcmp(lay, "rows")) cols = false;
+        else if (!std::strcmp(lay, "cols")) cols = true;
+        else if (std::strcmp(lay, "auto")) return fail(c, FM3D_ERR_INVALID, "FM3D_LM_IMG2 must be rows, cols or auto");
+    }
+    for (int j = 0; j < nProb; j++) src[j].c->lmCols = cols;
+    c->lmCols = cols;
+    const void* const kptrs[2][2][2] = {
+        {{reinterpret_cast<const void*>(fm3d::lm2_kernel<false, false, false>),
+          reinterpret_cast<const void*>(fm3d::lm2_kernel<false, false, true>)},
+         {reinterpret_cast<const void*>(fm3d::lm2_kernel<true, false, false>),
+          reinterpret_cast<const void*>(fm3d::lm2_kernel<true, false, true>)}},
+        {{reinterpret_cast<const void*>(fm3d::lm2_kernel<false, true, false>),
+          reinterpret_cast<const void*>(fm3d::lm2_kernel<false, true, true>)},
+         {reinterpret_cast<const void*>(fm3d::lm2_kernel<true, true, false>),
+          reinterpret_cast<const void*>(fm3d::lm2_kernel<true, true, true>)}}};
+    const void* kptr = kptrs[tree][multiPose][cols];
     long groups = 0;
     int r0;
     if ((r0 = lm_groups(c, kptr, slots, Ptot, &groups))) return r0;
diff --git a/3dfeaturematcher_amd/csrc/fm3d_lm2.hip b/3dfeaturematcher_amd/csrc/fm3d_lm2.hip
--- a/3dfeaturematcher_amd/csrc/fm3d_lm2.hip
+++ b/3dfeaturematcher_amd/csrc/fm3d_lm2.hip
@@ -48,6 +48,8 @@
     double scale, xmax, ymax, ccx, ccy, ajn0s, tq, ajn1s, tq0, agiant, wF;
     const uint8_t* img1;
     const uint8_t* img2;
+    const uint8_t* img2t;
+    int s2;
 };
 
 struct SlotS2 {
@@ -152,6 +154,8 @@
         P.img1 = lv.img1;
         P.img2 = lv.img2;
         P.lw = lv.w;
+        P.img2t = lv.img2t;
+        P.s2 = lv.hs;
         P.ccx = S.ccx;
         P.ccy = S.ccy;
     }
@@ -695,7 +699,7 @@
     unsigned off;
     LaneMask inbox, good;
 };
-template <bool MMOK, bool MULTI>
+template <bool MMOK, bool MULTI, bool COLS>
 __device__ __forceinline__ Geo2 geometry2(const LMParams& p, unsigned projOff, double ux, double uy, double n0,
                                           double n1, double n2, double mm, double scale,
                                           unsigned long long xmaxb, unsigned long long ymaxb, int lw, double cm) {
@@ -726,7 +730,8 @@
              __ballot((unsigned long long)__double_as_longlong(v) <= ymaxb);
     r.fx = (float)(scale * u);
     r.fy = (float)(scale * v);
-    const unsigned o = __umul24((unsigned)(int)floorf(r.fy), (unsigned)lw) + (unsigned)(int)floorf(r.fx);
+    const unsigned o = COLS ? __umul24((unsigned)(int)floorf(r.fx), (unsigned)lw) + (unsigned)(int)floorf(r.fy)
+                            : __umul24((unsigned)(int)floorf(r.fy), (unsigned)lw) + (unsigned)(int)floorf(r.fx);
     r.off = sel_mask_u32(o, r.good);
     return r;
 }
@@ -738,19 +743,21 @@
     return (P0 != P0 || P1 != P1 || P2 != P2) ? 2 : 3;
 }
 
+template <bool COLS>
 __device__ __forceinline__ float bilinear_w(unsigned lo, unsigned hi, float x, float y) {
     const float x0 = floorf(x), y0 = floorf(y);
-    const float b00 = (float)(lo & 0xff), b01 = (float)((lo >> 8) & 0xff);
-    const float b10 = (float)(hi & 0xff), b11 = (float)((hi >> 8) & 0xff);
+    const float b00 = (float)(lo & 0xff), b01 = COLS ? (float)(hi & 0xff) : (float)((lo >> 8) & 0xff);
+    const float b10 = COLS ? (float)((lo >> 8) & 0xff) : (float)(hi & 0xff), b11 = (float)((hi >> 8) & 0xff);
     const float xm0 = 1.0f - (x - x0), xm1 = (x - x0);
     const float ym0 = 1.0f - (y - y0), ym1 = (y - y0);
     return xm0 * (b00 * ym0 + b10 * ym1) + xm1 * (b01 * ym0 + b11 * ym1);
 }
 
 typedef float f32x2 __attribute__((ext_vector_type(2)));
+template <bool COLS>
 __device__ __forceinline__ float bilinear_f(unsigned lo, unsigned hi, float xf, float yf) {
-    const f32x2 b0 = {(float)(lo & 0xff), (float)((lo >> 8) & 0xff)};
-    const f32x2 b1 = {(float)(hi & 0xff), (float)((hi >> 8) & 0xff)};
+    const f32x2 b0 = {(float)(lo & 0xff), COLS ? (float)(hi & 0xff) : (float)((lo >> 8) & 0xff)};
+    const f32x2 b1 = {COLS ? (float)((lo >> 8) & 0xff) : (float)(hi & 0xff), (float)((hi >> 8) & 0xff)};
     const float ym0 = 1.0f - yf, ym1 = yf;
     const f32x2 sc = b0 * ym0 + b1 * ym1;
     const f32x2 xm = {1.0f - xf, xf};
@@ -886,7 +893,7 @@
 
 }
 
-template <bool MULTI, bool TREE>
+template <bool MULTI, bool TREE, bool COLS>
 __global__ __launch_bounds__(kLM2Threads, 4) void lm2_kernel(LMParams p) {
     Shared& sh = g_sh;
     constexpr int NS = TREE ? kWA : kW;
@@ -1094,8 +1101,8 @@
                     const double scale = SP.scale;
                     const unsigned long long xmaxb = (unsigned long long)__double_as_longlong(SP.xmax);
                     const unsigned long long ymaxb = (unsigned long long)__double_as_longlong(SP.ymax);
-                    const uint8_t* img2 = SP.img2;
-                    const int lw = rfl(SP.lw);
+                    const uint8_t* img2 = COLS ? SP.img2t : SP.img2;
+                    const int lw = rfl(COLS ? SP.s2 : SP.lw);
                     const unsigned projOff = MULTI ? (unsigned)rfl((int)SP.projOff) : 0u;
                     const bool i1ok = rfl(SS.i1ok) != 0;
                     const gu8* img2b = (const gu8*)rfl_ptr(img2);
@@ -1128,9 +1135,9 @@
                             float i1;
                         };
                         auto geo = [&](double ux, double uy, double n0, double n1, double n2, double mm) {
-                            return FAST ? geometry2<true, MULTI>(p, projOff, ux, uy, n0, n1, n2, mm, scale, xmaxb,
+                            return FAST ? geometry2<true, MULTI, COLS>(p, projOff, ux, uy, n0, n1, n2, mm, scale, xmaxb,
                                                                  ymaxb, lw, cm)
-                                        : geometry2<false, MULTI>(p, projOff, ux, uy, n0, n1, n2, mm, scale, xmaxb,
+                                        : geometry2<false, MULTI, COLS>(p, projOff, ux, uy, n0, n1, n2, mm, scale, xmaxb,
                                                                   ymaxb, lw, cm);
                         };
                         auto jdiv = [&](double a, double h, double y, bool mok) {
@@ -1181,7 +1188,7 @@
                                     ph31 |= (in & g1.inbox & ~g1.good) != 0;
                                 }
                             }
-                            const float dI0 = L.i1 - bilinear_w(a.x, a.y, g0.fx, g0.fy);
+                            const float dI0 = L.i1 - bilinear_w<COLS>(a.x, a.y, g0.fx, g0.fy);
                             const double r0 = w0 * (double)dI0;
                             double v0 = JAC ? jdiv(r0 - wF * L.dF, h0, y0, mok0) : r0;
                             v0 = sel_mask(v0, ok & g0.good);
@@ -1193,7 +1200,7 @@
                             const double t0 = enorm_term2(v0, agiant, slow0);
                             double v1 = 0., t1 = 0.;
                             if (NEV == 2) {
-                                const float dI1 = L.i1 - bilinear_w(c.x, c.y, g1.fx, g1.fy);
+                                const float dI1 = L.i1 - bilinear_w<COLS>(c.x, c.y, g1.fx, g1.fy);
                                 const double r1 = w1 * (double)dI1;
                                 v1 = jdiv(r1 - wF * L.dF, h1, y1, mok1);
                                 v1 = sel_mask(v1, ok & g1.good);
@@ -1249,8 +1256,8 @@
                                 return S;
                             };
                             auto back2 = [&](const St2& S, int k, unsigned oo) {
-                                const float dI0 = S.i1 - bilinear_f(S.a.x, S.a.y, S.xf0, S.yf0);
-                                const float dI1 = S.i1 - bilinear_f(S.c.x, S.c.y, S.xf1, S.yf1);
+                                const float dI0 = S.i1 - bilinear_f<COLS>(S.a.x, S.a.y, S.xf0, S.yf0);
+                                const float dI1 = S.i1 - bilinear_f<COLS>(S.c.x, S.c.y, S.xf1, S.yf1);
                                 if constexpr (TREE) {
                                     const auto* pc = sb();
                                     *(gfloat*)(pc->slabDJ0 + oo) = dI0;
@@ -1338,7 +1345,7 @@
                                 return S;
                             };
                             auto value = [&](float xf, float yf, uint2 w, float i1, float dF, LaneMask ok, float& dI) {
-                                dI = i1 - bilinear_f(w.x, w.y, xf, yf);
+                                dI = i1 - bilinear_f<COLS>(w.x, w.y, xf, yf);
                                 const double r = w0 * (double)dI;
                                 const double v = JAC ? jdiv(r - wF * (double)dF, h0, y0, mok0) : r;
                                 return sel_mask(v, ok);
@@ -1409,7 +1416,7 @@
                                 A = load(o8 + 2 * st8, o4 + 2 * st4);
                                 B = load(o8 + 3 * st8, o4 + 3 * st4);
                                 auto back1 = [&](const Geo2& g, uint2 w, float i1, double dF, LaneMask in, unsigned oo, int kk) {
-                                    const float dI = i1 - bilinear_w(w.x, w.y, g.fx, g.fy);
+                                    const float dI = i1 - bilinear_w<COLS>(w.x, w.y, g.fx, g.fy);
                                     const double r = w0 * (double)dI;
                                     double v = JAC ? jdiv(r - wF * dF, h0, y0, mok0) : r;
                                     v = sel_mask(v, (i1ok ? in : 0ull) & g.good);
@@ -1728,9 +1735,13 @@
     }
 }
 
-template __global__ void lm2_kernel<false, false>(LMParams p);
-template __global__ void lm2_kernel<true, false>(LMParams p);
-template __global__ void lm2_kernel<false, true>(LMParams p);
-template __global__ void lm2_kernel<true, true>(LMParams p);
-
-}
+template __global__ void lm2_kernel<false, false, false>(LMParams p);
+template __global__ void lm2_kernel<true, false, false>(LMParams p);
+template __global__ void lm2_kernel<false, true, false>(LMParams p);
+template __global__ void lm2_kernel<true, true, false>(LMParams p);
+template __global__ void lm2_kernel<false, false, true>(LMParams p);
+template __global__ void lm2_kernel<true, false, true>(LMParams p);
+template __global__ void lm2_kernel<false, true, true>(LMParams p);
+template __global__ void lm2_kernel<true, true, true>(LMParams p);
+
+}
diff --git a/3dfeaturematcher_amd/csrc/fm3d_misc.hip b/3dfeaturematcher_amd/csrc/fm3d_misc.hip
--- a/3dfeaturematcher_amd/csrc/fm3d_misc.hip
+++ b/3dfeaturematcher_amd/csrc/fm3d_misc.hip
@@ -152,7 +152,24 @@
     return q;
 }
 
-__global__ void pyrdown_kernel(const uint8_t* __restrict__ src, int w, int h, uint8_t* __restrict__ dst) {
+__device__ inline void store_colmajor(uint8_t* __restrict__ T, int hs, int w, int x, int y, uint8_t v) {
+    T[(size_t)x * hs + y] = v;
+    for (int xx = x + w, yy = y - 1; xx <= w + 1 && yy >= 0; xx += w, yy--) T[(size_t)xx * hs + yy] = v;
+}
+
+__global__ void level_transpose_kernel(const uint8_t* __restrict__ src, int w, int h, uint8_t* __restrict__ dstT,
+                                       int hs) {
+    __shared__ uint8_t tile[32][33];
+    const int tx = threadIdx.x, ty = threadIdx.y;
+    const int sx = blockIdx.x * 32 + tx, sy = blockIdx.y * 32 + ty;
+    if (sx < w && sy < h) tile[ty][tx] = src[(size_t)sy * w + sx];
+    __syncthreads();
+    const int x = blockIdx.x * 32 + ty, y = blockIdx.y * 32 + tx;
+    if (x < w && y < h) store_colmajor(dstT, hs, w, x, y, tile[tx][ty]);
+}
+
+__global__ void pyrdown_kernel(const uint8_t* __restrict__ src, int w, int h, uint8_t* __restrict__ dst,
+                               uint8_t* __restrict__ dstT, int hs) {
     const int dw = (w + 1) / 2, dh = (h + 1) / 2;
     const int x = blockIdx.x * blockDim.x + threadIdx.x;
     const int y = blockIdx.y * blockDim.y + threadIdx.y;
@@ -167,7 +184,9 @@
         for (int j = 0; j < 5; j++) rs += wt[j] * row[sx[j]];
         s += wt[i] * rs;
     }
-    dst[(size_t)y * dw + x] = (uint8_t)((s + 128) >> 8);
+    const uint8_t v = (uint8_t)((s + 128) >> 8);
+    dst[(size_t)y * dw + x] = v;
+    if (dstT) store_colmajor(dstT, hs, dw, x, y, v);
 }
 
 __global__ void undistort_kernel(Camera cam, const double* __restrict__ xy, int n, double* __restrict__ out) {
@@ -459,10 +478,15 @@
     lm_reset_kernel<<<(unsigned)((n + 255) / 256), 256, 0, s>>>(r, maxP);
 }
 
-void launch_pyrdown(const uint8_t* src, int w, int h, uint8_t* dst, hipStream_t s) {
+void launch_pyrdown(const uint8_t* src, int w, int h, uint8_t* dst, hipStream_t s, uint8_t* dstT, int hs) {
     const int dw = (w + 1) / 2, dh = (h + 1) / 2;
     dim3 blk(32, 8), grd((dw + 31) / 32, (dh + 7) / 8);
-    pyrdown_kernel<<<grd, blk, 0, s>>>(src, w, h, dst);
+    pyrdown_kernel<<<grd, blk, 0, s>>>(src, w, h, dst, dstT, hs);
+}
+
+void launch_level_transpose(const uint8_t* src, int w, int h, uint8_t* dstT, int hs, hipStream_t s) {
+    dim3 blk(32, 32), grd((w + 31) / 32, (h + 31) / 32);
+    level_transpose_kernel<<<grd, blk, 0, s>>>(src, w, h, dstT, hs);
 }
 
 void launch_plane_project(const PlaneProjParams& p, hipStream_t s) {
diff --git a/3dfeaturematcher_amd/csrc/fm3d_pipeline.cpp b/3dfeaturematcher_amd/csrc/fm3d_pipeline.cpp
--- a/3dfeaturematcher_amd/csrc/fm3d_pipeline.cpp
+++ b/3dfeaturematcher_amd/csrc/fm3d_pipeline.cpp
@@ -695,8 +695,8 @@
     if ((r = ensure_offsets(c))) return r;
     const bool tree = c->s.lmReduction != 0;
     const int slots = fm3d::kLM2Slots + (tree ? 1 : 0);
-    const void* kptr = tree ? reinterpret_cast<const void*>(fm3d::lm2_kernel<true, true>)
-                            : reinterpret_cast<const void*>(fm3d::lm2_kernel<true, false>);
+    const void* kptr = tree ? reinterpret_cast<const void*>(fm3d::lm2_kernel<true, true, false>)
+                            : reinterpret_cast<const void*>(fm3d::lm2_kernel<true, false, false>);
     long groups = 0;
     if ((r = lm_groups(c, kptr, slots, -1, &groups))) return r;
     const size_t ents = (size_t)c->nOffPad * slots;
@@ -708,6 +708,7 @@
     if (c->s.crossCheck != 0) need += (size_t)(nA + nB) * (rowWork + 8) + (size_t)nB * (24 + 16 * 16);
     need += (size_t)nA * 1536;
     need += (size_t)width * height * 4 + ((size_t)16 << 20);
+    need += (size_t)(width + 2) * (height + 65) * 2;
     *bytes = need;
     return FM3D_OK;
 }
```

Result: faster. 36430, median of 6 (+7.3%).
